# zhangkao/IIP_UAVSal_Saliency

Hardware: AMD Instinct MI355X
Metric: saliency frames/sec at 360x640 (higher is better)
Workload: dtype f32; 1 GPU; 360x640 batch=1 clip(s)/GPU seq=8, UAVSal.forward_clips, prec=f32, launch loop; requests_in_flight=1, clips_per_gpu=1, seq_len=8, height=360, width=640, precision=f32, persistent_state=False, parallelism=single GPU, fused_dw=10

## Files before the change

iip_uavsal_saliency_amd/_lib.py:

```python
from __future__ import annotations

import collections
import ctypes as C
import os

PKG = os.path.dirname(os.path.abspath(__file__))
LIB_PATH = os.environ.get("UAVSAL_HIP_LIB") or os.path.join(PKG, "libuavsal_hip.so")

PREC = {"f32": 0, "bf16x3": 1, "bf16": 2, "f16x3": 3}
ACT_NONE, ACT_RELU6, ACT_SIGMOID = 0, 1, 2
EPI_AFFINE, EPI_TWA, EPI_LSTM = 0, 1, 2
SK_TICKET_BASE = 4096

_ERR = {-1: "UAVSAL_EINVAL (null pointer / non-positive size)",
        -2: "UAVSAL_EALIGN (channel count / ld / pointer not 16-byte aligned)",
        -3: "UAVSAL_ESHAPE (shape not supported by the kernel)",
        -4: "UAVSAL_ESTATE (plan used in the wrong state)",
        -5: "UAVSAL_EDEVICE (a kernel reported a device-side error; the run's outputs are invalid)"}
ERR_STREAMK = 1
DW_KERNEL = {1: "dw3x3_kernel<1, 4, 4>", 2: "dw3x3_kernel<1, 2, 2>", 3: "dw3x3_kernel<2, 2, 2>", 4: "dw3x3_dilated_kernel",
             16: "dw3x3_map_lds_kernel<16, 256>", 32: "dw3x3_map_lds_kernel<32, 256>",
             528: "dw3x3_map_lds_kernel<16, 512>", 544: "dw3x3_map_lds_kernel<32, 512>",
             2048: "dw3x3_rowclass_kernel<256>"}

# ... 418 lines not shown

DESC_TYPES = [ConvDesc, DwDesc, StemDesc, BilinearDesc, TdiffDesc, TsumDesc, LayoutDesc, PostDesc, GuardDesc, CopyDesc,
              FusedIrDesc, WinoDesc, DwDotDesc, FillDesc, ScoreDesc, LetterboxDesc, OverlayDesc, GazeDesc, LossDesc, ConvRoute]

SYMBOLS = [
    ("uavsal_conv_gemm", C.c_int, [C.POINTER(ConvDesc), C.c_void_p]),
    ("uavsal_conv_route_of", C.c_int, [C.POINTER(ConvDesc), C.POINTER(ConvRoute)]),
    ("uavsal_conv_tile", C.c_int, [C.POINTER(ConvDesc)]),
    ("uavsal_conv_uses_split", C.c_int, [C.POINTER(ConvDesc)]),
    ("uavsal_conv_dwproj", C.c_int, [C.POINTER(ConvDesc)]),
    ("uavsal_streamk_workspace_bytes", C.c_longlong, []),
    ("uavsal_conv_streamk_grid", C.c_int, [C.POINTER(ConvDesc)]),
    ("uavsal_dw3x3", C.c_int, [C.POINTER(DwDesc), C.c_void_p]),
    ("uavsal_dw3x3_dot", C.c_int, [C.POINTER(DwDotDesc), C.c_void_p]),
    ("uavsal_dw_variant", C.c_int, [C.POINTER(DwDesc)]),
    ("uavsal_stem_conv", C.c_int, [C.POINTER(StemDesc), C.c_void_p]),
    ("uavsal_bilinear_ac", C.c_int, [C.POINTER(BilinearDesc), C.c_void_p]),
    ("uavsal_tdiff", C.c_int, [C.POINTER(TdiffDesc), C.c_void_p]),
    ("uavsal_tsum", C.c_int, [C.POINTER(TsumDesc), C.c_void_p]),
    ("uavsal_layout", C.c_int, [C.POINTER(LayoutDesc), C.c_void_p]),
    ("uavsal_postprocess", C.c_int, [C.POINTER(PostDesc), C.c_void_p]),
    ("uavsal_letterbox_u8", C.c_int, [C.POINTER(LetterboxDesc), C.c_void_p]),
    ("uavsal_overlay_workspace_bytes", C.c_int64, [C.POINTER(OverlayDesc)]),
    ("uavsal_overlay_u8", C.c_int, [C.POINTER(OverlayDesc), C.c_void_p]),
    ("uavsal_gaze_prepare", C.c_int, [C.POINTER(GazeDesc), C.c_void_p]),
    ("uavsal_loss_fu", C.c_int, [C.POINTER(LossDesc), C.c_void_p]),
    ("uavsal_loss_fu_grad", C.c_int, [C.POINTER(LossDesc), C.c_void_p]),
    ("uavsal_prior_accumulate", C.c_int, [C.POINTER(PriorAccDesc), C.c_void_p]),
    ("uavsal_prior_finish", C.c_int, [C.POINTER(PriorFinishDesc), C.c_void_p]),
    ("uavsal_prior_slab_frames", C.c_int, [C.c_int64, C.c_int32]),
    ("uavsal_prior_sizeof_desc", C.c_int, [C.c_int]),
    ("uavsal_twa_gate_bwd", C.c_int, [C.POINTER(TwaGateDesc), C.c_void_p]),
    ("uavsal_twa_wgrad_workspace_bytes", C.c_int64, [C.POINTER(TwaWgradDesc)]),
    ("uavsal_twa_wgrad_shares", C.c_int, [C.POINTER(TwaWgradDesc)]),
    ("uavsal_twa_wgrad", C.c_int, [C.POINTER(TwaWgradDesc), C.c_void_p]),
    ("uavsal_dec_bwd", C.c_int, [C.POINTER(DecBwdDesc), C.c_void_p]),
    ("uavsal_train_sizeof_desc", C.c_int, [C.c_int]),
    ("uavsal_lstm_scan", C.c_int, [C.POINTER(LstmScanDesc), C.c_void_p]),
    ("uavsal_lstm_gate_bwd", C.c_int, [C.POINTER(LstmGateDesc), C.c_void_p]),
    ("uavsal_lstm_sizeof_desc", C.c_int, [C.c_int]),
    ("uavsal_pix_gemm_workspace_bytes", C.c_int64, [C.POINTER(PixGemmDesc)]),
    ("uavsal_pix_gemm_shares", C.c_int, [C.POINTER(PixGemmDesc)]),
    ("uavsal_pix_gemm", C.c_int, [C.POINTER(PixGemmDesc), C.c_void_p]),
    ("uavsal_dec_sums_workspace_bytes", C.c_int64, [C.POINTER(DecSumsDesc)]),
    ("uavsal_dec_sums_slabs", C.c_int, [C.POINTER(DecSumsDesc)]),
    ("uavsal_dec_sums_slab_rows", C.c_int, [C.POINTER(DecSumsDesc)]),
    ("uavsal_dec_sums", C.c_int, [C.POINTER(DecSumsDesc), C.c_void_p]),
    ("uavsal_dec_finish", C.c_int, [C.POINTER(DecFinishDesc), C.c_void_p]),
    ("uavsal_train_decoder_sizeof_desc", C.c_int, [C.c_int]),
    ("uavsal_ir_bwd", C.c_int, [C.POINTER(IrBwdDesc), C.c_void_p]),
    ("uavsal_ir_sums_workspace_bytes", C.c_int64, [C.POINTER(IrSumsDesc)]),
    ("uavsal_ir_sums_slabs", C.c_int, [C.POINTER(IrSumsDesc)]),
    ("uavsal_ir_sums_slab_rows", C.c_int, [C.POINTER(IrSumsDesc)]),
    ("uavsal_ir_sums", C.c_int, [C.POINTER(IrSumsDesc), C.c_void_p]),
    ("uavsal_ir_finish", C.c_int, [C.POINTER(IrFinishDesc), C.c_void_p]),
    ("uavsal_ir_finish_c16", C.c_int, [C.POINTER(IrFinishDesc), C.c_void_p]),
    ("uavsal_block_sizeof_desc", C.c_int, [C.c_int]),
    ("uavsal_ir_bwd_s2", C.c_int, [C.POINTER(IrBwdS2Desc), C.c_void_p]),
    ("uavsal_bilinear_ac_bwd", C.c_int, [C.POINTER(BilinearBwdDesc), C.c_void_p]),
    ("uavsal_tsum_bwd", C.c_int, [C.POINTER(TsumBwdDesc), C.c_void_p]),
    ("uavsal_ctx_sizeof_desc", C.c_int, [C.c_int]),
    ("uavsal_ir_sums_s2_workspace_bytes", C.c_int64, [C.POINTER(IrSumsS2Desc)]),
    ("uavsal_ir_sums_s2_slabs", C.c_int, [C.POINTER(IrSumsS2Desc)]),
    ("uavsal_ir_sums_s2_slab_rows", C.c_int, [C.POINTER(IrSumsS2Desc)]),
    ("uavsal_ir_sums_s2", C.c_int, [C.POINTER(IrSumsS2Desc), C.c_void_p]),
    ("uavsal_mp_sizeof_desc", C.c_int, [C.c_int]),
    ("uavsal_ir_narrow_workspace_bytes", C.c_int64, [C.POINTER(IrNarrowDesc)]),
    ("uavsal_ir_narrow_slabs", C.c_int, [C.POINTER(IrNarrowDesc)]),
    ("uavsal_ir_narrow_slab_rows", C.c_int, [C.POINTER(IrNarrowDesc)]),
    ("uavsal_ir_narrow_grads", C.c_int, [C.POINTER(IrNarrowDesc), C.c_void_p]),
    ("uavsal_ir_narrow_finish", C.c_int, [C.POINTER(IrNarrowFinishDesc), C.c_void_p]),
    ("uavsal_frame_sum", C.c_int, [C.POINTER(FrameSumDesc), C.c_void_p]),
    ("uavsal_nets_sizeof_desc", C.c_int, [C.c_int]),
    ("uavsal_cbr_sums_workspace_bytes", C.c_int64, [C.POINTER(CbrSumsDesc)]),
    ("uavsal_cbr_sums_slabs", C.c_int, [C.POINTER(CbrSumsDesc)]),
    ("uavsal_cbr_sums_slab_rows", C.c_int, [C.POINTER(CbrSumsDesc)]),
    ("uavsal_cbr_sums", C.c_int, [C.POINTER(CbrSumsDesc), C.c_void_p]),
    ("uavsal_cbr_finish", C.c_int, [C.POINTER(CbrFinishDesc), C.c_void_p]),
    ("uavsal_tdiff_bwd", C.c_int, [C.POINTER(TdiffBwdDesc), C.c_void_p]),
    ("uavsal_st_sizeof_desc", C.c_int, [C.c_int]),
    ("uavsal_conv3_wgrad_workspace_bytes", C.c_int64, [C.POINTER(Conv3WgradDesc)]),
    ("uavsal_conv3_wgrad_shares", C.c_int, [C.POINTER(Conv3WgradDesc)]),
    ("uavsal_conv3_wgrad", C.c_int, [C.POINTER(Conv3WgradDesc), C.c_void_p]),
    ("uavsal_ir_bwd_dil", C.c_int, [C.POINTER(IrBwdDilDesc), C.c_void_p]),
    ("uavsal_ir_sums_dil_workspace_bytes", C.c_int64, [C.POINTER(IrSumsDilDesc)]),
    ("uavsal_ir_sums_dil_slabs", C.c_int, [C.POINTER(IrSumsDilDesc)]),
    ("uavsal_ir_sums_dil_slab_rows", C.c_int, [C.POINTER(IrSumsDilDesc)]),
    ("uavsal_ir_sums_dil", C.c_int, [C.POINTER(IrSumsDilDesc), C.c_void_p]),
    ("uavsal_srf_sizeof_desc", C.c_int, [C.c_int]),
    ("uavsal_skinny_wgrad_workspace_bytes", C.c_int64, [C.POINTER(SkinnyWgradDesc)]),
    ("uavsal_skinny_wgrad_shares", C.c_int, [C.POINTER(SkinnyWgradDesc)]),
    ("uavsal_skinny_wgrad", C.c_int, [C.POINTER(SkinnyWgradDesc), C.c_void_p]),
    ("uavsal_shallow_sizeof_desc", C.c_int, [C.c_int]),
    ("uavsal_bn_slabs", C.c_int, [C.c_int, C.c_int, C.c_int]),
    ("uavsal_bn_slab_rows", C.c_int, [C.c_int, C.c_int, C.c_int]),
    ("uavsal_bn_stats_workspace_bytes", C.c_int64, [C.POINTER(BnStatsDesc)]),
    ("uavsal_bn_stats", C.c_int, [C.POINTER(BnStatsDesc), C.c_void_p]),
    ("uavsal_bn_apply", C.c_int, [C.POINTER(BnApplyDesc), C.c_void_p]),
    ("uavsal_bn_bwd_workspace_bytes", C.c_int64, [C.POINTER(BnBwdDesc)]),
    ("uavsal_bn_bwd_sums", C.c_int, [C.POINTER(BnBwdDesc), C.c_void_p]),
    ("uavsal_bn_bwd_apply", C.c_int, [C.POINTER(BnBwdDesc), C.c_void_p]),
    ("uavsal_dw_wgrad_workspace_bytes", C.c_int64, [C.POINTER(DwWgradDesc)]),
    ("uavsal_dw_wgrad", C.c_int, [C.POINTER(DwWgradDesc), C.c_void_p]),
    ("uavsal_bn_sizeof_desc", C.c_int, [C.c_int]),
    ("uavsal_bn_apply_res", C.c_int, [C.POINTER(BnApplyResDesc), C.c_void_p]),
    ("uavsal_block_bn_sizeof_desc", C.c_int, [C.c_int]),
    ("uavsal_repack", C.c_int, [C.c_void_p, C.c_int, C.c_int, C.c_void_p]),
    ("uavsal_repack_sizeof_desc", C.c_int, []),
    ("uavsal_guard", C.c_int, [C.POINTER(GuardDesc), C.c_void_p]),
    ("uavsal_copy_rows", C.c_int, [C.POINTER(CopyDesc), C.c_void_p]),
    ("uavsal_fill", C.c_int, [C.POINTER(FillDesc), C.c_void_p]),
    ("uavsal_plan_add_fill", C.c_int, [C.c_void_p, C.POINTER(FillDesc)]),
    ("uavsal_fused_ir", C.c_int, [C.POINTER(FusedIrDesc), C.c_void_p]),
    ("uavsal_fused_ir_supported", C.c_int, [C.POINTER(FusedIrDesc)]),
    ("uavsal_plan_add_fused_ir", C.c_int, [C.c_void_p, C.POINTER(FusedIrDesc)]),
    ("uavsal_wino_input", C.c_int, [C.POINTER(WinoDesc), C.c_void_p]),
    ("uavsal_wino_output", C.c_int, [C.POINTER(WinoDesc), C.c_void_p]),
    ("uavsal_wino_output_zero_h", C.c_int, [C.POINTER(WinoDesc), C.c_void_p]),
    ("uavsal_wino_seam", C.c_int, [C.POINTER(WinoDesc), C.POINTER(WinoDesc), C.c_void_p]),
    ("uavsal_wino_seam_zero_h", C.c_int, [C.POINTER(WinoDesc), C.POINTER(WinoDesc), C.c_void_p]),
    ("uavsal_wino_seam_check", C.c_int, [C.POINTER(WinoDesc), C.POINTER(WinoDesc)]),
    ("uavsal_plan_add_wino_input", C.c_int, [C.c_void_p, C.POINTER(WinoDesc)]),
    ("uavsal_plan_add_wino_output", C.c_int, [C.c_void_p, C.POINTER(WinoDesc)]),
    ("uavsal_plan_add_copy", C.c_int, [C.c_void_p, C.POINTER(CopyDesc)]),
    ("uavsal_plan_create", C.c_void_p, []),
    ("uavsal_plan_destroy", None, [C.c_void_p]),
    ("uavsal_plan_add_conv", C.c_int, [C.c_void_p, C.POINTER(ConvDesc)]),
    ("uavsal_plan_add_dw", C.c_int, [C.c_void_p, C.POINTER(DwDesc)]),
    ("uavsal_plan_add_dw_dot", C.c_int, [C.c_void_p, C.POINTER(DwDotDesc)]),
    ("uavsal_plan_add_stem", C.c_int, [C.c_void_p, C.POINTER(StemDesc)]),
    ("uavsal_plan_add_bilinear", C.c_int, [C.c_void_p, C.POINTER(BilinearDesc)]),
    ("uavsal_plan_add_tdiff", C.c_int, [C.c_void_p, C.POINTER(TdiffDesc)]),
    ("uavsal_plan_add_tsum", C.c_int, [C.c_void_p, C.POINTER(TsumDesc)]),
    ("uavsal_plan_add_layout", C.c_int, [C.c_void_p, C.POINTER(LayoutDesc)]),
    ("uavsal_plan_error_word", C.c_void_p, [C.c_void_p]),
    ("uavsal_plan_add_guard", C.c_int, [C.c_void_p, _f, C.c_int64, _f, C.c_int64, _f, C.c_int64]),
    ("uavsal_plan_status", C.c_int, [C.c_void_p, C.c_int]),
    ("uavsal_plan_patch_ptr", C.c_int, [C.c_void_p, C.c_int, C.c_int, C.c_void_p]),
    ("uavsal_plan_set_lane", C.c_int, [C.c_void_p, C.c_int]),
    ("uavsal_plan_add_fork", C.c_int, [C.c_void_p, C.c_int]),
    ("uavsal_plan_add_join", C.c_int, [C.c_void_p, C.c_int]),
    ("uavsal_plan_enable_lanes", C.c_int, [C.c_void_p, C.c_int]),
    ("uavsal_plan_size", C.c_int, [C.c_void_p]),
    ("uavsal_plan_run", C.c_int, [C.c_void_p, C.c_int, C.c_int, C.c_void_p]),
    ("uavsal_plan_group_mark", C.c_int, [C.c_void_p, C.c_int, C.c_int, C.c_int]),
    ("uavsal_plan_group_enable", C.c_int, [C.c_void_p, C.c_int, C.c_int]),
    ("uavsal_plan_group_launches", C.c_int, [C.c_void_p, C.c_int]),
    ("uavsal_plan_last_launches", C.c_int, [C.c_void_p]),
    ("uavsal_plan_frame_repeat", C.c_int, [C.c_void_p, C.c_int, C.c_int, C.c_int, C.c_int, C.c_int]),
    ("uavsal_plan_frame_repeat_workgroups", C.c_int, [C.c_void_p, C.c_int]),
    ("uavsal_plan_seam", C.c_int, [C.c_void_p, C.c_int, C.c_int, C.c_int]),
    ("uavsal_plan_zero_state", C.c_int, [C.c_void_p, C.c_int, C.c_int, C.c_int, C.c_int, C.c_int, C.c_int]),
    ("uavsal_plan_mode_report", C.c_int, [C.c_void_p, C.POINTER(C.c_int * 4)]),
    ("uavsal_plan_graph_build", C.c_int, [C.c_void_p, C.c_void_p]),
    ("uavsal_plan_graph_launch", C.c_int, [C.c_void_p, C.c_void_p]),
    ("uavsal_plan_time", C.c_int, [C.c_void_p, C.c_int, C.c_int, C.c_int, C.c_void_p, C.POINTER(C.c_float)]),
    ("uavsal_score_workspace_bytes", C.c_int64, [C.POINTER(ScoreDesc)]),
    ("uavsal_score_stats", C.c_int, [C.POINTER(ScoreDesc), C.c_void_p]),
    ("uavsal_score_run", C.c_int, [C.POINTER(ScoreDesc), C.c_void_p]),
    ("uavsal_abi_version", C.c_int, []),
    ("uavsal_sizeof_desc", C.c_int, [C.c_int]),
    ("uavsal_build_info", C.c_char_p, []),
]

_lib = None


def load():
    global _lib
    if _lib is not None:
        return _lib
    if not os.path.exists(LIB_PATH):
        raise RuntimeError(
            "libuavsal_hip.so is not built (%s). Run `python -m iip_uavsal_saliency_amd.build` "
            "(needs hipcc). There is no CPU fallback for the UAVSal HIP path." % LIB_PATH)
    lib = C.CDLL(LIB_PATH)
    for name, res, args in SYMBOLS:
        fn = getattr(lib, name)
        fn.restype = res
        fn.argtypes = args
    if lib.uavsal_abi_version() != 20:
        raise RuntimeError("libuavsal_hip.so ABI version mismatch")
    for i, t in enumerate(DESC_TYPES):
        if lib.uavsal_sizeof_desc(i) != C.sizeof(t):
            raise RuntimeError("descriptor %s: ctypes size %d != C size %d" % (
                t.__name__, C.sizeof(t), lib.uavsal_sizeof_desc(i)))
    for sizeof, types in ((lib.uavsal_prior_sizeof_desc, PRIOR_DESC_TYPES), (lib.uavsal_train_sizeof_desc, TRAIN_DESC_TYPES),
                          (lib.uavsal_train_decoder_sizeof_desc, TRAIN_DECODER_DESC_TYPES),
                          (lib.uavsal_block_sizeof_desc, BLOCK_DESC_TYPES), (lib.uavsal_ctx_sizeof_desc, CTX_DESC_TYPES),
                          (lib.uavsal_mp_sizeof_desc, MP_DESC_TYPES), (lib.uavsal_nets_sizeof_desc, NETS_DESC_TYPES),
                          (lib.uavsal_st_sizeof_desc, ST_DESC_TYPES), (lib.uavsal_srf_sizeof_desc, SRF_DESC_TYPES),
                          (lib.uavsal_shallow_sizeof_desc, SHALLOW_DESC_TYPES), (lib.uavsal_lstm_sizeof_desc, LSTM_DESC_TYPES),
                          (lib.uavsal_bn_sizeof_desc, BN_DESC_TYPES), (lib.uavsal_block_bn_sizeof_desc, BLOCK_BN_DESC_TYPES)):
        for i, t in enumerate(types):
            if sizeof(i) != C.sizeof(t):
                raise RuntimeError("descriptor %s: ctypes size %d != C size %d" % (t.__name__, C.sizeof(t), sizeof(i)))
    if lib.uavsal_repack_sizeof_desc() != C.sizeof(RepackEntry):
        raise RuntimeError("descriptor RepackEntry: ctypes size %d != C size %d" % (C.sizeof(RepackEntry), lib.uavsal_repack_sizeof_desc()))
    _lib = lib
    return lib


def check(code: int, what: str = "uavsal call"):
    if code == 0:
        return
    if code == -5:
        raise RuntimeError("%s: %s" % (what, _ERR[-5]))
    if code < 0:
        raise RuntimeError("%s rejected its arguments: %s" % (what, _ERR.get(code, str(code))))
    raise RuntimeError("%s failed with hipError_t %d" % (what, code))
```

iip_uavsal_saliency_amd/csrc/fused_ir.hip:

```cpp
#include "common.h"

namespace {

struct FusedK {
    const float* in; const float* w1; const float* s1; const float* b1;
    const float* wd; const float* sd; const float* bd;
    const float* w2; const float* s2; const float* b2;
    const float* res; float* out;
    int ldi, ldr, ldo, H, W, Ho, Wo, tiles_x, tiles_y;
};

typedef float f32x2 __attribute__((ext_vector_type(2)));

__device__ __forceinline__ f32x4 relu6_4(f32x4 v) {
    return (f32x4){__builtin_amdgcn_fmed3f(v.x, 0.f, 6.f), __builtin_amdgcn_fmed3f(v.y, 0.f, 6.f), __builtin_amdgcn_fmed3f(v.z, 0.f, 6.f),
                   __builtin_amdgcn_fmed3f(v.w, 0.f, 6.f)};
}

#ifndef UAVSAL_FUSED_STAGE_W
#define UAVSAL_FUSED_STAGE_W 1
#endif
#ifndef UAVSAL_FUSED_NBUF2_MAX
#define UAVSAL_FUSED_NBUF2_MAX (80 * 1024)
#endif

template <int S, int TX, int PT>
struct FusedGeom {
    static constexpr int RP = 16 / TX;
    static constexpr int TY = 4 * PT * RP;
    static constexpr int IH = (TY - 1) * S + 3, IW = (TX - 1) * S + 3;
    static constexpr int HALF = (IW + 1) / 2;
    static constexpr int IWP = S == 2 ? 2 * HALF : IW;
    static constexpr int NSLOT = IH * IWP, NRT = (NSLOT + 15) / 16;
};

template <int CIN, int HID, int COUT, int S, bool EXPAND, int HC, int TX, int PT>
struct FusedCfg : FusedGeom<S, TX, PT> {
    using G = FusedGeom<S, TX, PT>;
    static constexpr int PLANE = EXPAND ? G::NRT * 16 * 4 : 4;
    static constexpr int SLOTF = EXPAND ? 4 : HC + 4;
    static constexpr int EBUF = EXPAND ? (HC / 4) * PLANE : G::NRT * 16 * SLOTF;
    static constexpr int NCH = HID / HC;
    static constexpr int CW_S1 = CIN * HC, CW_B1 = CW_S1 + HC, CW_WD = CW_B1 + HC, CW_SD = CW_WD + 9 * HC, CW_BD = CW_SD + HC,
                         CW_W2 = CW_BD + HC, CW_F = CW_W2 + HC * COUT;
    static constexpr bool STAGE_W = EXPAND && UAVSAL_FUSED_STAGE_W;
    static constexpr int NBUF = (EXPAND && NCH > 1 && (2 * EBUF + (STAGE_W ? 2 * CW_F : 0)) * 4 <= UAVSAL_FUSED_NBUF2_MAX) ? 2 : 1;
    static constexpr size_t E_BYTES = (size_t)NBUF * EBUF * 4;
    static constexpr int WBASE = NBUF * EBUF;
    static constexpr size_t SMEM = E_BYTES + (STAGE_W ? (size_t)2 * CW_F * 4 : 0);
};

#ifndef UAVSAL_FUSED_PROBE
#define UAVSAL_FUSED_PROBE 0
#endif

#ifdef UAVSAL_FIR_STAMPS
__device__ unsigned long long g_fir_stamps[128];
#define FIR_STAMP(i) { asm volatile("s_waitcnt vmcnt(0) lgkmcnt(0)" ::: "memory"); \
                       if (blockIdx.x == gridDim.x / 2 && tid == 0) g_fir_stamps[i] = __builtin_amdgcn_s_memtime(); }
#else
#define FIR_STAMP(i)
#endif

template <int CIN, int HID, int COUT, int S, bool EXPAND, int HC, int TX, int PT>
__global__ __launch_bounds__(256, 2) void fused_ir_kernel(const FusedK p) {
    using Cfg = FusedCfg<CIN, HID, COUT, S, EXPAND, HC, TX, PT>;
    constexpr int RP = Cfg::RP, TY = Cfg::TY, IH = Cfg::IH, IW = Cfg::IW, HALF = Cfg::HALF, IWP = Cfg::IWP;
    constexpr int NSLOT = Cfg::NSLOT, NRT = Cfg::NRT, RTW = (NRT + 3) / 4;
    constexpr int CPL = HC / 4, CQ = CPL / 4, PLANE = Cfg::PLANE, SLOTF = Cfg::SLOTF;
    constexpr int NCH = Cfg::NCH, NCTE = HC / 16, NCT = (COUT + 15) / 16, KE = CIN / 4;
    constexpr int EBUF = Cfg::EBUF, NBUF = Cfg::NBUF;
    static_assert(HID % HC == 0 && HC % 16 == 0 && CIN % 8 == 0 && COUT % 4 == 0, "channel blocking");
    static_assert(EXPAND || (HID == CIN && NCH == 1), "without an expand conv the hidden tensor is the input");
    static_assert(KE % 2 == 0, "x fragments are loaded 8 bytes at a time");

    extern __shared__ __attribute__((aligned(16))) float lds[];

    const int tid = threadIdx.x, lane = tid & 63;
    const int wave = __builtin_amdgcn_readfirstlane(tid >> 6);
    const int l15 = lane & 15, lq = lane >> 4;
    int t = blockIdx.x;
    const int tx = t % p.tiles_x; t /= p.tiles_x;
    const int ty = t % p.tiles_y;
    const int n = t / p.tiles_y;
    const int oy0 = ty * TY, ox0 = tx * TX;
    const int iy0 = oy0 * S - 1, ix0 = ox0 * S - 1;
    const float* inb = p.in + (size_t)n * p.H * p.W * p.ldi;
    FIR_STAMP(0)

    auto slot_pixel = [&](int slot, int& gy, int& gx) -> bool {
        const int iy = slot / IWP, rem = slot - iy * IWP;
        int ix = rem;
        if (S == 2) { const int par = rem >= HALF ? 1 : 0; ix = 2 * (rem - par * HALF) + par; }
        gy = iy0 + iy; gx = ix0 + ix;
        return slot < NSLOT && ix < IW && gy >= 0 && gy < p.H && gx >= 0 && gx < p.W;
    };

    auto slot_read = [&](int slot) -> bool {
        const int iy = slot / IWP, rem = slot - iy * IWP;
        return slot < NSLOT && (S == 2 ? rem != IWP - 1 || (IW & 1) == 0 : true);
    };

    float xv[EXPAND ? RTW : 1][EXPAND ? KE : 1];
    unsigned outside = 0;
    unsigned any_outside = 0;
    if (EXPAND) {
#pragma unroll
        for (int j = 0; j < RTW; ++j) {
            const int rt = wave + 4 * j;
            int gy, gx;
            const bool in = rt < NRT && slot_pixel(rt * 16 + l15, gy, gx);
            const bool zero = !in && rt < NRT && slot_read(rt * 16 + l15);
            outside |= (zero ? 1u : 0u) << j;
            any_outside |= (__builtin_amdgcn_ballot_w64(zero) != 0ull ? 1u : 0u) << j;
            const float* src = inb + ((size_t)(in ? gy : 0) * p.W + (in ? gx : 0)) * p.ldi + lq * KE;
            if (KE % 4 == 0) {
#pragma unroll
                for (int s = 0; s < KE; s += 4) {
                    f32x4 v = {0.f, 0.f, 0.f, 0.f};
                    if (in) v = *reinterpret_cast<const f32x4*>(src + s);
                    xv[j][s] = v.x; xv[j][s + 1] = v.y; xv[j][s + 2] = v.z; xv[j][s + 3] = v.w;
                }
            } else {
#pragma unroll
                for (int s = 0; s < KE; s += 2) {
                    f32x2 v = {0.f, 0.f};
                    if (in) v = *reinterpret_cast<const f32x2*>(src + s);
                    xv[j][s] = v.x; xv[j][s + 1] = v.y;
                }
            }
        }
    } else {
        constexpr int NQ = CIN / 4, NST = (NRT * 16 * NQ + 255) / 256;
        f32x4 st[NST];
#pragma unroll
        for (int i = 0; i < NST; ++i) {
            const int idx = tid + 256 * i;
            const int slot = idx / NQ, q = idx - slot * NQ;
            int gy, gx;
            st[i] = (f32x4){0.f, 0.f, 0.f, 0.f};
            if (idx < NRT * 16 * NQ && slot_pixel(slot, gy, gx)) st[i] = *reinterpret_cast<const f32x4*>(inb + ((size_t)gy * p.W + gx) * p.ldi + q * 4);
        }
#pragma unroll
        for (int i = 0; i < NST; ++i) {
            const int idx = tid + 256 * i;
            const int slot = idx / NQ, q = idx - slot * NQ;
            if (idx < NRT * 16 * NQ) *reinterpret_cast<f32x4*>(lds + (size_t)q * PLANE + slot * SLOTF) = st[i];
        }
    }

    FIR_STAMP(1)
    f32x4 acc_o[PT][NCT];
#pragma unroll
    for (int pt = 0; pt < PT; ++pt)
#pragma unroll
        for (int ct = 0; ct < NCT; ++ct) acc_o[pt][ct] = (f32x4){0.f, 0.f, 0.f, 0.f};

    constexpr bool STAGE_W = Cfg::STAGE_W;
    constexpr int HQ = HC / 4, NI_W1 = CIN * HQ, NI_V = HQ, NI_WD = 9 * HQ, NI_W2 = HC * COUT / 4;
    constexpr int NITEM = NI_W1 + 2 * NI_V + NI_WD + 2 * NI_V + NI_W2, WROUNDS = (NITEM + 255) / 256;
    float* const wl = lds + Cfg::WBASE;
    const float* wsrc[STAGE_W ? WROUNDS : 1];
    int wdst[STAGE_W ? WROUNDS : 1], wstep[STAGE_W ? WROUNDS : 1];
    f32x4 wreg[STAGE_W ? WROUNDS : 1];
    if (STAGE_W) {
#pragma unroll
        for (int r = 0; r < WROUNDS; ++r) {
            int it = tid + 256 * r;
            wsrc[r] = nullptr; wdst[r] = 0; wstep[r] = HC;
            if (it < NI_W1) { const int k = it / HQ, q = it - k * HQ; wsrc[r] = p.w1 + (size_t)k * HID + 4 * q; wdst[r] = k * HC + 4 * q; }
            else if ((it -= NI_W1) < NI_V) { wsrc[r] = p.s1 + 4 * it; wdst[r] = Cfg::CW_S1 + 4 * it; }
            else if ((it -= NI_V) < NI_V) { wsrc[r] = p.b1 + 4 * it; wdst[r] = Cfg::CW_B1 + 4 * it; }
            else if ((it -= NI_V) < NI_WD) { const int tp = it / HQ, q = it - tp * HQ; wsrc[r] = p.wd + (size_t)tp * HID + 4 * q; wdst[r] = Cfg::CW_WD + tp * HC + 4 * q; }
            else if ((it -= NI_WD) < NI_V) { wsrc[r] = p.sd + 4 * it; wdst[r] = Cfg::CW_SD + 4 * it; }
            else if ((it -= NI_V) < NI_V) { wsrc[r] = p.bd + 4 * it; wdst[r] = Cfg::CW_BD + 4 * it; }
            else if ((it -= NI_V) < NI_W2) { wsrc[r] = p.w2 + 4 * it; wdst[r] = Cfg::CW_W2 + 4 * it; wstep[r] = HC * COUT; }
        }
#pragma unroll
        for (int r = 0; r < WROUNDS; ++r)
            if (wsrc[r]) *reinterpret_cast<f32x4*>(wl + wdst[r]) = *reinterpret_cast<const f32x4*>(wsrc[r]);
        __syncthreads();
    }
    const float* const g_w1 = p.w1;
    FIR_STAMP(2)

    for (int ch = 0; ch < NCH; ++ch) {
        const int c0 = (UAVSAL_FUSED_PROBE & 8) ? 0 : ch * HC;
        const float* const wc = wl + (ch & 1) * Cfg::CW_F;
        float w1f[EXPAND ? NCTE : 1][EXPAND ? KE : 1];
        f32x4 s1q[EXPAND ? NCTE : 1], b1q[EXPAND ? NCTE : 1];
        if (EXPAND) {
#pragma unroll
            for (int ct = 0; ct < NCTE; ++ct) {
#pragma unroll
                for (int s = 0; s < KE; ++s)
                    w1f[ct][s] = STAGE_W ? wc[(lq * KE + s) * HC + ct * 16 + l15] : g_w1[(size_t)(lq * KE + s) * HID + c0 + ct * 16 + l15];
                s1q[ct] = STAGE_W ? *reinterpret_cast<const f32x4*>(wc + Cfg::CW_S1 + ct * 16 + 4 * lq)
                                  : *reinterpret_cast<const f32x4*>(p.s1 + c0 + ct * 16 + 4 * lq);
                b1q[ct] = STAGE_W ? *reinterpret_cast<const f32x4*>(wc + Cfg::CW_B1 + ct * 16 + 4 * lq)
                                  : *reinterpret_cast<const f32x4*>(p.b1 + c0 + ct * 16 + 4 * lq);
            }
        }
        f32x4 wdq[9][CQ], sdq[CQ], bdq[CQ];
#pragma unroll
        for (int q = 0; q < CQ; ++q) {
#pragma unroll
            for (int tp = 0; tp < 9; ++tp)
                wdq[tp][q] = STAGE_W ? *reinterpret_cast<const f32x4*>(wc + Cfg::CW_WD + tp * HC + lq * CPL + 4 * q)
                                     : *reinterpret_cast<const f32x4*>(p.wd + (size_t)tp * HID + c0 + lq * CPL + 4 * q);
            sdq[q] = STAGE_W ? *reinterpret_cast<const f32x4*>(wc + Cfg::CW_SD + lq * CPL + 4 * q) : *reinterpret_cast<const f32x4*>(p.sd + c0 + lq * CPL + 4 * q);
            bdq[q] = STAGE_W ? *reinterpret_cast<const f32x4*>(wc + Cfg::CW_BD + lq * CPL + 4 * q) : *reinterpret_cast<const f32x4*>(p.bd + c0 + lq * CPL + 4 * q);
        }
        float w2f[NCT][CPL];
#pragma unroll
        for (int ct = 0; ct < NCT; ++ct) {
            const int co = ct * 16 + l15;
#pragma unroll
            for (int s = 0; s < CPL; ++s)
                w2f[ct][s] = co < COUT ? (STAGE_W ? wc[Cfg::CW_W2 + (lq * CPL + s) * COUT + co] : p.w2[(size_t)(c0 + lq * CPL + s) * COUT + co]) : 0.f;
        }
        if (STAGE_W && ch + 1 < NCH) {
#pragma unroll
            for (int r = 0; r < WROUNDS; ++r)
                if (wsrc[r]) wreg[r] = *reinterpret_cast<const f32x4*>(wsrc[r] + (size_t)(ch + 1) * wstep[r]);
        }

        FIR_STAMP(8 + 5 * ch)
        float* eb = lds + (NBUF == 2 ? (ch & 1) * EBUF : 0);
        if (EXPAND) {
            if (NBUF == 1 && ch > 0 && !(UAVSAL_FUSED_PROBE & 16)) __syncthreads();
#pragma unroll
            for (int j = 0; j < RTW; ++j) {
                const int rt = wave + 4 * j;
                if (4 * j + 3 >= NRT && rt >= NRT) continue;
                f32x4 e[NCTE];
#pragma unroll
                for (int ct = 0; ct < NCTE; ++ct) {
                    e[ct] = (f32x4){0.f, 0.f, 0.f, 0.f};
#pragma unroll
                    for (int s = 0; s < KE; ++s) {
                        if (UAVSAL_FUSED_PROBE & 1) e[ct][s & 3] += w1f[ct][s] * xv[j][s];
                        else e[ct] = __builtin_amdgcn_mfma_f32_16x16x4f32(w1f[ct][s], xv[j][s], e[ct], 0, 0, 0);
                    }
                    e[ct] = relu6_4(e[ct] * s1q[ct] + b1q[ct]);
                }
                if ((any_outside >> j) & 1u) {
                    const bool z = (outside >> j) & 1u;
#pragma unroll
                    for (int ct = 0; ct < NCTE; ++ct) if (z) e[ct] = (f32x4){0.f, 0.f, 0.f, 0.f};
                }
#pragma unroll
                for (int ct = 0; ct < NCTE; ++ct)
                    if (!(UAVSAL_FUSED_PROBE & 32) || e[ct].x == 123.f) *reinterpret_cast<f32x4*>(eb + (size_t)(ct * 4 + lq) * PLANE + (rt * 16 + l15) * SLOTF) = e[ct];
            }
        }
        if (STAGE_W && ch + 1 < NCH) {
#pragma unroll
            for (int r = 0; r < WROUNDS; ++r)
                if (wsrc[r]) *reinterpret_cast<f32x4*>(wl + ((ch + 1) & 1) * Cfg::CW_F + wdst[r]) = wreg[r];
        }
        FIR_STAMP(9 + 5 * ch)
        if (!(UAVSAL_FUSED_PROBE & 16)) __syncthreads();
        FIR_STAMP(10 + 5 * ch)
#pragma unroll
        for (int pt = 0; pt < PT; ++pt) {
            const int g = wave * PT + pt;
            const int orow = g * RP + l15 / TX, ocol = l15 % TX;
            f32x4 dq[CQ];
#pragma unroll
            for (int q = 0; q < CQ; ++q) dq[q] = (f32x4){0.f, 0.f, 0.f, 0.f};
#pragma unroll
            for (int ky = 0; ky < ((UAVSAL_FUSED_PROBE & 2) ? 1 : 3); ++ky)
#pragma unroll
                for (int kx = 0; kx < ((UAVSAL_FUSED_PROBE & 2) ? 1 : 3); ++kx) {
                    const int slot = (orow * S + ky) * IWP + (S == 2 ? (kx & 1) * HALF + ocol + (kx >> 1) : ocol + kx);
                    const float* e = eb + (size_t)(lq * CQ) * PLANE + slot * SLOTF;
#pragma unroll
                    for (int q = 0; q < CQ; ++q) dq[q] = *reinterpret_cast<const f32x4*>(e + (size_t)q * PLANE) * wdq[ky * 3 + kx][q] + dq[q];
                }
#pragma unroll
            for (int q = 0; q < CQ; ++q) dq[q] = relu6_4(dq[q] * sdq[q] + bdq[q]);
            if (pt == PT - 1) { FIR_STAMP(11 + 5 * ch) }
#pragma unroll
            for (int s = 0; s < CPL; ++s)
#pragma unroll
                for (int ct = 0; ct < NCT; ++ct)
                    if (UAVSAL_FUSED_PROBE & 4) acc_o[pt][ct][s & 3] += w2f[ct][s] * dq[s >> 2][s & 3];
                    else acc_o[pt][ct] = __builtin_amdgcn_mfma_f32_16x16x4f32(w2f[ct][s], dq[s >> 2][s & 3], acc_o[pt][ct], 0, 0, 0);
        }
        FIR_STAMP(12 + 5 * ch)
    }
    FIR_STAMP(3)

#pragma unroll
    for (int ct = 0; ct < NCT; ++ct) {
        const int co = ct * 16 + 4 * lq;
        if (co >= COUT) continue;
        const f32x4 sc = *reinterpret_cast<const f32x4*>(p.s2 + co), bi = *reinterpret_cast<const f32x4*>(p.b2 + co);
#pragma unroll
        for (int pt = 0; pt < PT; ++pt) {
            const int g = wave * PT + pt;
            const int gy = oy0 + g * RP + l15 / TX, gx = ox0 + l15 % TX;
            if (gy >= p.Ho || gx >= p.Wo) continue;
            const size_t opix = ((size_t)n * p.Ho + gy) * p.Wo + gx;
            f32x4 v = acc_o[pt][ct] * sc + bi;
            if (p.res) v += *reinterpret_cast<const f32x4*>(p.res + opix * p.ldr + co);
            *reinterpret_cast<f32x4*>(p.out + opix * p.ldo + co) = v;
        }
    }
    FIR_STAMP(4)
}

template <int CIN, int HID, int COUT, int S, bool EXPAND, int HC, int TX, int PT>
int launch_fused(const uavsal_fused_ir_desc* d, hipStream_t s) {
    using Cfg = FusedCfg<CIN, HID, COUT, S, EXPAND, HC, TX, PT>;
    FusedK k;
    k.in = d->in; k.w1 = d->w1; k.s1 = d->scale1; k.b1 = d->bias1;
    k.wd = d->wd; k.sd = d->scale_d; k.bd = d->bias_d;
    k.w2 = d->w2; k.s2 = d->scale2; k.b2 = d->bias2;
    k.res = d->res; k.out = d->out;
    k.ldi = d->ldi; k.ldr = d->ldr; k.ldo = d->ldo; k.H = d->H; k.W = d->W;
    k.Ho = (d->H - 1) / S + 1; k.Wo = (d->W - 1) / S + 1;
    k.tiles_x = (k.Wo + TX - 1) / TX; k.tiles_y = (k.Ho + Cfg::TY - 1) / Cfg::TY;
    const long long nblk = (long long)d->n_img * k.tiles_y * k.tiles_x;
    if (nblk > 0x7fffffffLL) return UAVSAL_ESHAPE;
    UAVSAL_LDS_OPTIN((&fused_ir_kernel<CIN, HID, COUT, S, EXPAND, HC, TX, PT>), Cfg::SMEM);
    hipLaunchKernelGGL((fused_ir_kernel<CIN, HID, COUT, S, EXPAND, HC, TX, PT>), dim3((unsigned)nblk), dim3(256), Cfg::SMEM, s, k);
    return uavsal_launch_status();
}

#ifndef UAVSAL_FUSED_BIG_MIN
#define UAVSAL_FUSED_BIG_MIN 400
#endif
template <int CIN, int HID, int COUT, int S, bool EXPAND, int HCS, int HCB>
int launch_fused_shape(const uavsal_fused_ir_desc* d, hipStream_t s) {
    constexpr bool BIG_AUTO = !(CIN == 32 && COUT == 64);
    constexpr int BPT = S == 1 ? 4 : 2;
    constexpr int BTY = 4 * BPT;
    const int Ho = (d->H - 1) / S + 1, Wo = (d->W - 1) / S + 1;
    const long long big = (long long)d->n_img * ((Ho + BTY - 1) / BTY) * ((Wo + 15) / 16);
    const bool use_big = d->tile == 2 || (d->tile == 0 && BIG_AUTO && big >= UAVSAL_FUSED_BIG_MIN);
    return use_big ? launch_fused<CIN, HID, COUT, S, EXPAND, HCB, 16, BPT>(d, s) : launch_fused<CIN, HID, COUT, S, EXPAND, HCS, 16, 1>(d, s);
}

int dispatch(const uavsal_fused_ir_desc* d, hipStream_t s, bool launch) {
#define UAVSAL_FUSED_UNPAREN(...) __VA_ARGS__
#define UAVSAL_FUSED_CASE(CIN, HID, COUT, S, EXP, HCC)                                                   \
    if (d->Cin == CIN && d->hidden == HID && d->Cout == COUT && d->stride == S && (d->w1 != nullptr) == EXP) \
        return launch ? launch_fused_shape<CIN, HID, COUT, S, EXP, UAVSAL_FUSED_UNPAREN HCC>(d, s) : 1;
#ifndef UAVSAL_FUSED_HCS
#define UAVSAL_FUSED_HCS 16
#endif
#ifndef UAVSAL_FUSED_HCS144
#define UAVSAL_FUSED_HCS144 16
#endif
#ifndef UAVSAL_FUSED_HCB
#define UAVSAL_FUSED_HCB 16
#endif
#ifndef UAVSAL_FUSED_HCB144
#define UAVSAL_FUSED_HCB144 16
#endif
    UAVSAL_FUSED_CASE(32, 32, 16, 1, false, (32, 32))
    UAVSAL_FUSED_CASE(16, 96, 24, 2, true, (UAVSAL_FUSED_HCS, UAVSAL_FUSED_HCB))
    UAVSAL_FUSED_CASE(24, 144, 24, 1, true, (UAVSAL_FUSED_HCS144, UAVSAL_FUSED_HCB144))
    UAVSAL_FUSED_CASE(24, 144, 32, 2, true, (UAVSAL_FUSED_HCS144, UAVSAL_FUSED_HCB144))
    UAVSAL_FUSED_CASE(32, 192, 32, 1, true, (UAVSAL_FUSED_HCS, UAVSAL_FUSED_HCB))
    UAVSAL_FUSED_CASE(32, 192, 64, 2, true, (UAVSAL_FUSED_HCS, UAVSAL_FUSED_HCB))
#undef UAVSAL_FUSED_CASE
    return launch ? UAVSAL_ESHAPE : 0;
}

}

int uavsal_fused_mid_dispatch(const uavsal_fused_ir_desc* d, hipStream_t s, bool launch);

#ifdef UAVSAL_FIR_STAMPS
extern "C" int uavsal_fir_stamps(unsigned long long* dst) {
    return (int)hipMemcpyFromSymbol(dst, HIP_SYMBOL(g_fir_stamps), sizeof(unsigned long long) * 128);
}
#endif

extern "C" int uavsal_fused_ir_supported(const uavsal_fused_ir_desc* d) {
    if (!d) return 0;
    const int mid = uavsal_fused_mid_dispatch(d, nullptr, false);
    return mid ? mid : dispatch(d, nullptr, false);
}

extern "C" int uavsal_fused_ir(const uavsal_fused_ir_desc* d, uavsal_stream_t stream) {
    if (!d || !d->in || !d->wd || !d->scale_d || !d->bias_d || !d->w2 || !d->scale2 || !d->bias2 || !d->out) return UAVSAL_EINVAL;
    if (d->w1 && (!d->scale1 || !d->bias1)) return UAVSAL_EINVAL;
    if (d->n_img <= 0 || d->H <= 0 || d->W <= 0) return UAVSAL_EINVAL;
    if ((d->ldi & 3) || d->ldi < d->Cin || (d->ldo & 3) || d->ldo < d->Cout || !uavsal_aligned16(d->in) || !uavsal_aligned16(d->out) ||
        !uavsal_aligned16(d->wd) || !uavsal_aligned16(d->scale_d) || !uavsal_aligned16(d->bias_d) || !uavsal_aligned16(d->scale2) ||
        !uavsal_aligned16(d->bias2) || (d->w1 && (!uavsal_aligned16(d->scale1) || !uavsal_aligned16(d->bias1))) ||
        (d->res && ((d->ldr & 3) || !uavsal_aligned16(d->res))))
        return UAVSAL_EALIGN;
    if ((d->w1 && !uavsal_aligned16(d->w1)) || !uavsal_aligned16(d->w2)) return UAVSAL_EALIGN;
    if (d->tile < 0 || d->tile > 2) return UAVSAL_EINVAL;
    if (d->res && (d->ldr < d->Cout || d->stride != 1 || d->Cin != d->Cout)) return UAVSAL_ESHAPE;
    if (uavsal_fused_mid_dispatch(d, nullptr, false)) return uavsal_fused_mid_dispatch(d, (hipStream_t)stream, true);
    return dispatch(d, (hipStream_t)stream, true);
}
```

iip_uavsal_saliency_amd/csrc/glue.hip:

```cpp
#include "common.h"

namespace {

struct StemK {
    const float* in; const uint8_t* in_u8; const float* w; const float* scale; const float* bias;
    float* out; int ldo, H, W, Ho, Wo, tiles_x, tiles_y;
    float mean[3], stdv[3];
};

constexpr int ST_TY = 4, ST_TX = 64, ST_IH = 2 * ST_TY + 1, ST_IW = 2 * ST_TX + 1, ST_PITCH = 132, ST_ROWS = 3 * ST_IH;
static_assert(ST_PITCH >= ST_IW && ST_PITCH % 4 == 0 && ST_TY * ST_TX == 256, "stem tile");

__global__ __launch_bounds__(256) void stem_kernel(const StemK p) {
    __shared__ __attribute__((aligned(16))) float wsh[27 * 32];
    __shared__ __attribute__((aligned(16))) float ssh[32], bsh[32];
    __shared__ __attribute__((aligned(16))) float xsh[ST_ROWS * ST_PITCH];
    const int tid = threadIdx.x;
    int b = blockIdx.x;
    const int tx = b % p.tiles_x; b /= p.tiles_x;
    const int ty = b % p.tiles_y;
    const int n = b / p.tiles_y;
    const int oy0 = ty * ST_TY, ox0 = tx * ST_TX;
    const int iy0 = 2 * oy0 - 1, ix0 = 2 * ox0 - 1;
    const size_t plane = (size_t)p.H * p.W;
    constexpr int NST = (ST_ROWS * ST_PITCH + 255) / 256;
    float st[NST];
#pragma unroll
    for (int i = 0; i < NST; ++i) {
        const int idx = tid + 256 * i;
        const int r = idx / ST_PITCH, c = idx - r * ST_PITCH;
        const int ci = r / ST_IH, iy = iy0 + (r - ci * ST_IH), ix = ix0 + c;
        float x = 0.f;
        if (r < ST_ROWS && c < ST_IW && iy >= 0 && iy < p.H && ix >= 0 && ix < p.W) {
            const size_t at = ((size_t)n * 3 + ci) * plane + (size_t)iy * p.W + ix;
            if (p.in_u8) x = ((float)p.in_u8[at] / 255.0f - p.mean[ci]) / p.stdv[ci];
            else x = p.in[at];
        }
        st[i] = x;
    }
    for (int i = tid; i < 27 * 32; i += 256) wsh[i] = p.w[i];
    if (tid < 32) { ssh[tid] = p.scale[tid]; bsh[tid] = p.bias[tid]; }
#pragma unroll
    for (int i = 0; i < NST; ++i) {
        const int idx = tid + 256 * i;
        if (idx < ST_ROWS * ST_PITCH) xsh[idx] = st[i];
    }
    __syncthreads();
    const int g = tid & 7, pxg = tid >> 3;
    const int rr = pxg / (ST_TX / 8), xq = pxg - rr * (ST_TX / 8);
    const int oy = oy0 + rr, oxb = ox0 + 8 * xq;
    f32x4 acc[8];
#pragma unroll
    for (int q = 0; q < 8; ++q) acc[q] = (f32x4){0.f, 0.f, 0.f, 0.f};
#pragma unroll 1
    for (int ci = 0; ci < 3; ++ci) {
#pragma unroll
        for (int ky = 0; ky < 3; ++ky) {
            const float* row = xsh + (ci * ST_IH + 2 * rr + ky) * ST_PITCH + 16 * xq;
            float v[17];
#pragma unroll
            for (int c = 0; c < 4; ++c) {
                const f32x4 a = *reinterpret_cast<const f32x4*>(row + 4 * c);
                v[4 * c] = a.x; v[4 * c + 1] = a.y; v[4 * c + 2] = a.z; v[4 * c + 3] = a.w;
            }
            v[16] = row[16];
#pragma unroll
            for (int kx = 0; kx < 3; ++kx) {
                const f32x4 w4 = *reinterpret_cast<const f32x4*>(wsh + (ci * 9 + ky * 3 + kx) * 32 + g * 4);
#pragma unroll
                for (int q = 0; q < 8; ++q) acc[q] = w4 * v[2 * q + kx] + acc[q];
            }
        }
    }
    if (oy >= p.Ho) return;
    const f32x4 sc = *reinterpret_cast<const f32x4*>(ssh + g * 4), bi = *reinterpret_cast<const f32x4*>(bsh + g * 4);
#pragma unroll
    for (int q = 0; q < 8; ++q) {
        const int ox = oxb + q;
        if (ox >= p.Wo) break;
        f32x4 r = acc[q] * sc + bi;
        r.x = fminf(fmaxf(r.x, 0.f), 6.f); r.y = fminf(fmaxf(r.y, 0.f), 6.f); r.z = fminf(fmaxf(r.z, 0.f), 6.f); r.w = fminf(fmaxf(r.w, 0.f), 6.f);
        *reinterpret_cast<f32x4*>(p.out + (((size_t)n * p.Ho + oy) * p.Wo + ox) * p.ldo + g * 4) = r;
    }
}

struct BilK {
    const float* in; float* out;
    int ldi, ldo, Hi, Wi, Ho, Wo, C4, src_mod, src_div;
    float sy, sx; long long total;
    _Float16* out_split; int ldos;
};

__global__ __launch_bounds__(256) void bilinear_kernel(const BilK p) {
    const long long item = (long long)blockIdx.x * 256 + threadIdx.x;
    if (item >= p.total) return;
    const int c = (int)(item % p.C4) * 4;
    long long t = item / p.C4;
    const int ox = (int)(t % p.Wo); t /= p.Wo;
    const int oy = (int)(t % p.Ho);
    const int n = (int)(t / p.Ho);
    const int ns = (n % p.src_mod) / p.src_div;
    const float fy = p.sy * oy, fx = p.sx * ox;
    const int y0 = (int)fy, x0 = (int)fx;
    const int y1 = y0 + (y0 < p.Hi - 1 ? 1 : 0), x1 = x0 + (x0 < p.Wi - 1 ? 1 : 0);
    const float ly = fy - y0, lx = fx - x0;
    const float hy = 1.f - ly, hx = 1.f - lx;
    const float* b = p.in + (size_t)ns * p.Hi * p.Wi * p.ldi + c;
    const f32x4 v00 = *reinterpret_cast<const f32x4*>(b + ((size_t)y0 * p.Wi + x0) * p.ldi);
    const f32x4 v01 = *reinterpret_cast<const f32x4*>(b + ((size_t)y0 * p.Wi + x1) * p.ldi);
    const f32x4 v10 = *reinterpret_cast<const f32x4*>(b + ((size_t)y1 * p.Wi + x0) * p.ldi);
    const f32x4 v11 = *reinterpret_cast<const f32x4*>(b + ((size_t)y1 * p.Wi + x1) * p.ldi);
    const f32x4 r = hy * (hx * v00 + lx * v01) + ly * (hx * v10 + lx * v11);
    const size_t opix = ((size_t)n * p.Ho + oy) * p.Wo + ox;
    *reinterpret_cast<f32x4*>(p.out + opix * p.ldo + c) = r;
    if (p.out_split) uavsal_store_split4(p.out_split + opix * p.ldos, c, r);
}

struct TdK { const float* in; float* out; int ldi, ldo, HW, C4, L; long long total; };

__global__ __launch_bounds__(256) void tdiff_kernel(const TdK p) {
    const long long item = (long long)blockIdx.x * 256 + threadIdx.x;
    if (item >= p.total) return;
    const int c = (int)(item % p.C4) * 4;
    long long t = item / p.C4;
    const int pix = (int)(t % p.HW);
    const int n = (int)(t / p.HW);
    const int tt = n % p.L;
    const size_t img = (size_t)p.HW * p.ldi;
    const float* cur = p.in + (size_t)n * img + (size_t)pix * p.ldi + c;
    const f32x4 x = *reinterpret_cast<const f32x4*>(cur);
    f32x4 dprev, dnext;
    if (tt == 0) {
        const f32x4 nx = *reinterpret_cast<const f32x4*>(cur + img);
        dprev = nx - x; dnext = x - nx;
    } else if (tt == p.L - 1) {
        const f32x4 pv = *reinterpret_cast<const f32x4*>(cur - img);
        dprev = x - pv; dnext = pv - x;
    } else {
        const f32x4 pv = *reinterpret_cast<const f32x4*>(cur - img);
        const f32x4 nx = *reinterpret_cast<const f32x4*>(cur + img);
        dprev = x - pv; dnext = x - nx;
    }
    float* o = p.out + ((size_t)n * p.HW + pix) * p.ldo + c;
    *reinterpret_cast<f32x4*>(o) = dprev;
    *reinterpret_cast<f32x4*>(o + p.C4 * 4) = dnext;
}

struct TsK { const float* in; float* out; int ldi, ldo, HW, C4, T; long long total; };

__global__ __launch_bounds__(256) void tsum_kernel(const TsK p) {
    const long long item = (long long)blockIdx.x * 256 + threadIdx.x;
    if (item >= p.total) return;
    const int c = (int)(item % p.C4) * 4;
    long long t = item / p.C4;
    const int pix = (int)(t % p.HW);
    const int b = (int)(t / p.HW);
    const size_t img = (size_t)p.HW * p.ldi;
    const float* src = p.in + (size_t)b * p.T * img + (size_t)pix * p.ldi + c;
    f32x4 s = *reinterpret_cast<const f32x4*>(src);
    for (int k = 1; k < p.T; ++k) s += *reinterpret_cast<const f32x4*>(src + (size_t)k * img);
    *reinterpret_cast<f32x4*>(p.out + ((size_t)b * p.HW + pix) * p.ldo + c) = s;
}

struct LayK { const float* in; float* out; int C, HW, ld, Cpad, to_nhwc; long long total; };

__global__ __launch_bounds__(256) void layout_kernel(const LayK p) {
    __shared__ float tile[32][33];
    const int tiles_c = (p.Cpad + 31) / 32;
    const int tiles_p = (p.HW + 31) / 32;
    long long b = blockIdx.x;
    const int tc = (int)(b % tiles_c); b /= tiles_c;
    const int tp = (int)(b % tiles_p);
    const int n = (int)(b / tiles_p);
    const int lx = threadIdx.x & 31, ly = threadIdx.x >> 5;
    if (p.to_nhwc) {
        for (int j = ly; j < 32; j += 8) {
            const int c = tc * 32 + j, px = tp * 32 + lx;
            tile[j][lx] = (c < p.C && px < p.HW) ? p.in[((size_t)n * p.C + c) * p.HW + px] : 0.f;
        }
        __syncthreads();
        for (int j = ly; j < 32; j += 8) {
            const int px = tp * 32 + j, c = tc * 32 + lx;
            if (px < p.HW && c < p.Cpad) p.out[((size_t)n * p.HW + px) * p.ld + c] = tile[lx][j];
        }
    } else {
        for (int j = ly; j < 32; j += 8) {
            const int px = tp * 32 + j, c = tc * 32 + lx;
            tile[j][lx] = (px < p.HW && c < p.C) ? p.in[((size_t)n * p.HW + px) * p.ld + c] : 0.f;
        }
        __syncthreads();
        for (int j = ly; j < 32; j += 8) {
            const int c = tc * 32 + j, px = tp * 32 + lx;
            if (c < p.C && px < p.HW) p.out[((size_t)n * p.C + c) * p.HW + px] = tile[lx][j];
        }
    }
}

inline int grid_for(long long total, int* nblk) {
    const long long b = (total + 255) / 256;
    if (b <= 0 || b > 0x7fffffffLL) return UAVSAL_ESHAPE;
    *nblk = (int)b;
    return 0;
}

}

extern "C" int uavsal_stem_conv(const uavsal_stem_desc* d, uavsal_stream_t stream) {
    if (!d || (!d->in && !d->in_u8) || !d->w || !d->scale || !d->bias || !d->out) return UAVSAL_EINVAL;
    if (d->n_img <= 0 || d->H <= 0 || d->W <= 0) return UAVSAL_EINVAL;
    if ((d->ldo & 3) || d->ldo < 32 || !uavsal_aligned16(d->out)) return UAVSAL_EALIGN;
    StemK k;
    k.in = d->in; k.in_u8 = d->in_u8; k.w = d->w; k.scale = d->scale; k.bias = d->bias; k.out = d->out;
    k.ldo = d->ldo; k.H = d->H; k.W = d->W; k.Ho = (d->H - 1) / 2 + 1; k.Wo = (d->W - 1) / 2 + 1;
    for (int i = 0; i < 3; ++i) { k.mean[i] = d->mean[i]; k.stdv[i] = d->stdv[i]; }
    k.tiles_x = (k.Wo + ST_TX - 1) / ST_TX; k.tiles_y = (k.Ho + ST_TY - 1) / ST_TY;
    const long long nblk = (long long)d->n_img * k.tiles_y * k.tiles_x;
    if (nblk > 0x7fffffffLL) return UAVSAL_ESHAPE;
    hipLaunchKernelGGL(stem_kernel, dim3((unsigned)nblk), dim3(256), 0, (hipStream_t)stream, k);
    return uavsal_launch_status();
}

extern "C" int uavsal_bilinear_ac(const uavsal_bilinear_desc* d, uavsal_stream_t stream) {
    if (!d || !d->in || !d->out) return UAVSAL_EINVAL;
    if (d->n_out <= 0 || d->C <= 0 || d->Hi <= 0 || d->Wi <= 0 || d->Ho <= 0 || d->Wo <= 0) return UAVSAL_EINVAL;
    if (d->src_mod <= 0 || d->src_div <= 0) return UAVSAL_EINVAL;
    if ((d->C & 3) || (d->ldi & 3) || (d->ldo & 3) || d->ldi < d->C || d->ldo < d->C) return UAVSAL_EALIGN;
    if (!uavsal_aligned16(d->in) || !uavsal_aligned16(d->out)) return UAVSAL_EALIGN;
    BilK k;
    k.in = d->in; k.out = d->out; k.ldi = d->ldi; k.ldo = d->ldo;
    k.Hi = d->Hi; k.Wi = d->Wi; k.Ho = d->Ho; k.Wo = d->Wo; k.C4 = d->C / 4;
    k.src_mod = d->src_mod; k.src_div = d->src_div;
    k.sy = d->Ho > 1 ? (float)(d->Hi - 1) / (float)(d->Ho - 1) : 0.f;
    k.sx = d->Wo > 1 ? (float)(d->Wi - 1) / (float)(d->Wo - 1) : 0.f;
    if (d->out_split && ((d->ldos & 63) || d->ldos < 2 * d->C || (d->C & 31) || ((uintptr_t)d->out_split & 127)))
// ... 109 lines not shown
```

iip_uavsal_saliency_amd/csrc/plan.hip:

```cpp
#include <vector>
#include <new>
#include "common.h"

namespace {
enum OpKind { OP_CONV = 0, OP_DW, OP_STEM, OP_BILINEAR, OP_TDIFF, OP_TSUM, OP_LAYOUT, OP_GUARD, OP_COPY, OP_FUSED_IR, OP_FORK, OP_JOIN,
              OP_WINO_IN, OP_WINO_OUT, OP_DW_DOT, OP_FILL };
constexpr int MAX_LANES = 8;
constexpr int MAX_GROUPS = 32;

struct Op {
    int kind;
    int lane;
    int group;
    union {
        uavsal_conv_desc conv;
        uavsal_dw_desc dw;
        uavsal_stem_desc stem;
        uavsal_bilinear_desc bil;
        uavsal_tdiff_desc td;
        uavsal_tsum_desc ts;
        uavsal_layout_desc lay;
        uavsal_guard_desc guard;
        uavsal_copy_desc copy;
        uavsal_fused_ir_desc fir;
        uavsal_wino_desc wino;
        uavsal_dw_dot_desc dwdot;
        uavsal_fill_desc fill;
    } u;
};

int run_op(const Op& op, uavsal_stream_t s) {
    switch (op.kind) {
        case OP_CONV: return uavsal_conv_gemm(&op.u.conv, s);
        case OP_DW: return uavsal_dw3x3(&op.u.dw, s);
        case OP_STEM: return uavsal_stem_conv(&op.u.stem, s);
        case OP_BILINEAR: return uavsal_bilinear_ac(&op.u.bil, s);
        case OP_TDIFF: return uavsal_tdiff(&op.u.td, s);
        case OP_TSUM: return uavsal_tsum(&op.u.ts, s);
        case OP_LAYOUT: return uavsal_layout(&op.u.lay, s);
        case OP_GUARD: return uavsal_guard(&op.u.guard, s);
        case OP_COPY: return uavsal_copy_rows(&op.u.copy, s);
        case OP_FUSED_IR: return uavsal_fused_ir(&op.u.fir, s);
        case OP_WINO_IN: return uavsal_wino_input(&op.u.wino, s);
        case OP_WINO_OUT: return uavsal_wino_output(&op.u.wino, s);
        case OP_DW_DOT: return uavsal_dw3x3_dot(&op.u.dwdot, s);
        case OP_FILL: return uavsal_fill(&op.u.fill, s);
    }
    return UAVSAL_EINVAL;
}
}

struct uavsal_plan {
    std::vector<Op> ops;
    hipGraph_t graph = nullptr;
    hipGraphExec_t exec = nullptr;
    int cur_lane = 0;
    bool lanes_on = true;
    hipStream_t side[MAX_LANES] = {};
    std::vector<hipEvent_t> events;
    int32_t* err_dev = nullptr;
    int32_t* err_host = nullptr;
    int32_t* err_host_dev = nullptr;
    hipEvent_t done = nullptr;
    bool ran = false;
    uint32_t groups_off = 0;
    int last_launches = 0;
    int graph_launches = 0;
    int fr_pw = -1, fr_dw = -1, fr_mod = 0, fr_div = 0;
    bool fr_on = false;
    int fr_wg[2] = {0, 0};
    std::vector<int> seam_next;
    int zs_first = -1, zs_last = -1, zs_xin = -1, zs_gemm = -1, zs_xout = -1;
    bool zs_on = false;
    int mode_seams = 0, mode_elided = 0, mode_kernels = 0;
};

extern "C" uavsal_plan* uavsal_plan_create(void) { return new (std::nothrow) uavsal_plan(); }

static bool ensure_error_words(uavsal_plan* p) {
    if (p->err_dev && p->err_host && p->done) return true;
    bool ok = hipMalloc((void**)&p->err_dev, 64) == hipSuccess && hipMemset(p->err_dev, 0, 64) == hipSuccess &&
              hipHostMalloc((void**)&p->err_host, 64, hipHostMallocMapped) == hipSuccess;
    if (ok) {
        p->err_host[0] = 0;
        ok = hipHostGetDevicePointer((void**)&p->err_host_dev, p->err_host, 0) == hipSuccess &&
             hipEventCreateWithFlags(&p->done, hipEventDisableTiming) == hipSuccess;
    }
    if (!ok) (void)hipGetLastError();
    return ok;
}

extern "C" int32_t* uavsal_plan_error_word(uavsal_plan* p) { return (p && ensure_error_words(p)) ? p->err_dev : nullptr; }

extern "C" int uavsal_plan_add_guard(uavsal_plan* p, float* b0, int64_t n0, float* b1, int64_t n1, float* b2, int64_t n2) {
    if (!p) return UAVSAL_EINVAL;
    if (p->exec) return UAVSAL_ESTATE;
    if (!ensure_error_words(p)) return UAVSAL_ESTATE;
    Op op; op.kind = OP_GUARD; op.lane = 0; op.group = -1;
    op.u.guard.err = p->err_dev; op.u.guard.host_err = p->err_host_dev;
    op.u.guard.buf[0] = b0; op.u.guard.n[0] = n0;
    op.u.guard.buf[1] = b1; op.u.guard.n[1] = n1;
    op.u.guard.buf[2] = b2; op.u.guard.n[2] = n2;
    for (int b = 0; b < 3; ++b)
        if ((op.u.guard.buf[b] == nullptr) != (op.u.guard.n[b] == 0) || op.u.guard.n[b] < 0) return UAVSAL_EINVAL;
    p->ops.push_back(op);
    return (int)p->ops.size() - 1;
}

extern "C" int uavsal_plan_status(uavsal_plan* p, int wait) {
    if (!p) return UAVSAL_EINVAL;
    if (!p->ran) return 0;
    if (wait) {
        const hipError_t e = hipEventSynchronize(p->done);
        if (e != hipSuccess) return (int)e;
    } else {
        const hipError_t e = hipEventQuery(p->done);
        if (e == hipErrorNotReady) { (void)hipGetLastError(); return 0; }
        if (e != hipSuccess) return (int)e;
    }
    const int32_t code = *(volatile int32_t*)p->err_host;
    if (code == 0) return 0;
    p->err_host[0] = 0;
    const hipError_t e = hipMemset(p->err_dev, 0, 64);
    if (e != hipSuccess) return (int)e;
    return UAVSAL_EDEVICE;
}

extern "C" void uavsal_plan_destroy(uavsal_plan* p) {
    if (!p) return;
    if (p->exec) hipGraphExecDestroy(p->exec);
    if (p->graph) hipGraphDestroy(p->graph);
    for (hipEvent_t e : p->events) if (e) hipEventDestroy(e);
    for (int i = 1; i < MAX_LANES; ++i) if (p->side[i]) hipStreamDestroy(p->side[i]);
    if (p->done) hipEventDestroy(p->done);
    if (p->err_host) hipHostFree(p->err_host);
    if (p->err_dev) hipFree(p->err_dev);
    delete p;
}

extern "C" int uavsal_plan_set_lane(uavsal_plan* p, int lane) {
    if (!p || lane < 0 || lane >= MAX_LANES) return UAVSAL_EINVAL;
    p->cur_lane = lane;
    return 0;
}

extern "C" int uavsal_plan_enable_lanes(uavsal_plan* p, int on) {
    if (!p) return UAVSAL_EINVAL;
    if (p->exec) return UAVSAL_ESTATE;
    p->lanes_on = on != 0;
    return 0;
}

static int add_sync(uavsal_plan* p, int kind, int lane) {
    if (!p || lane < 1 || lane >= MAX_LANES) return UAVSAL_EINVAL;
    if (p->exec) return UAVSAL_ESTATE;
    Op op; op.kind = kind; op.lane = lane; op.group = -1;
    p->ops.push_back(op);
    return (int)p->ops.size() - 1;
}
extern "C" int uavsal_plan_add_fork(uavsal_plan* p, int lane) { return add_sync(p, OP_FORK, lane); }
extern "C" int uavsal_plan_add_join(uavsal_plan* p, int lane) { return add_sync(p, OP_JOIN, lane); }

#define UAVSAL_ADD(fn, KIND, field, T)                                   \
    extern "C" int fn(uavsal_plan* p, const T* d) {                      \
        if (!p || !d) return UAVSAL_EINVAL;                              \
        if (p->exec) return UAVSAL_ESTATE;                               \
        Op op; op.kind = KIND; op.lane = p->cur_lane; op.group = -1; op.u.field = *d; \
        p->ops.push_back(op);                                            \
        return (int)p->ops.size() - 1;                                   \
    }
UAVSAL_ADD(uavsal_plan_add_conv, OP_CONV, conv, uavsal_conv_desc)
UAVSAL_ADD(uavsal_plan_add_dw, OP_DW, dw, uavsal_dw_desc)
UAVSAL_ADD(uavsal_plan_add_stem, OP_STEM, stem, uavsal_stem_desc)
UAVSAL_ADD(uavsal_plan_add_bilinear, OP_BILINEAR, bil, uavsal_bilinear_desc)
UAVSAL_ADD(uavsal_plan_add_tdiff, OP_TDIFF, td, uavsal_tdiff_desc)
UAVSAL_ADD(uavsal_plan_add_tsum, OP_TSUM, ts, uavsal_tsum_desc)
UAVSAL_ADD(uavsal_plan_add_layout, OP_LAYOUT, lay, uavsal_layout_desc)
UAVSAL_ADD(uavsal_plan_add_copy, OP_COPY, copy, uavsal_copy_desc)
UAVSAL_ADD(uavsal_plan_add_fused_ir, OP_FUSED_IR, fir, uavsal_fused_ir_desc)
UAVSAL_ADD(uavsal_plan_add_wino_input, OP_WINO_IN, wino, uavsal_wino_desc)
UAVSAL_ADD(uavsal_plan_add_wino_output, OP_WINO_OUT, wino, uavsal_wino_desc)
UAVSAL_ADD(uavsal_plan_add_dw_dot, OP_DW_DOT, dwdot, uavsal_dw_dot_desc)
UAVSAL_ADD(uavsal_plan_add_fill, OP_FILL, fill, uavsal_fill_desc)

extern "C" int uavsal_plan_patch_ptr(uavsal_plan* p, int op, int slot, void* ptr) {
    if (!p || op < 0 || op >= (int)p->ops.size() || !ptr) return UAVSAL_EINVAL;
    if (p->exec) return UAVSAL_ESTATE;
    Op& o = p->ops[op];
    switch (o.kind) {
        case OP_CONV:
            if (!uavsal_aligned16(ptr)) return UAVSAL_EALIGN;
            if (slot == 0) o.u.conv.a = (const float*)ptr;
            else if (slot == 1) o.u.conv.out = (float*)ptr;
            else return UAVSAL_EINVAL;
            return 0;
        case OP_DW_DOT:
            if (slot == 0) { if (!uavsal_aligned16(ptr)) return UAVSAL_EALIGN; o.u.dwdot.in = (const float*)ptr; }
            else if (slot == 1) o.u.dwdot.out = (float*)ptr;
            else return UAVSAL_EINVAL;
            return 0;
        case OP_STEM:
            if (slot == 0) { o.u.stem.in = (const float*)ptr; o.u.stem.in_u8 = nullptr; }
            else if (slot == 1) { o.u.stem.in_u8 = (const uint8_t*)ptr; o.u.stem.in = nullptr; }
            else return UAVSAL_EINVAL;
            return 0;
        case OP_LAYOUT:
            if (slot == 0) o.u.lay.in = (const float*)ptr;
            else if (slot == 1) o.u.lay.out = (float*)ptr;
            else return UAVSAL_EINVAL;
            return 0;
        case OP_GUARD:
            if (slot < 0 || slot > 2 || !o.u.guard.buf[slot]) return UAVSAL_EINVAL;
            o.u.guard.buf[slot] = (float*)ptr;
            return 0;
    }
    return UAVSAL_ESHAPE;
}

extern "C" int uavsal_plan_size(const uavsal_plan* p) { return p ? (int)p->ops.size() : UAVSAL_EINVAL; }

extern "C" int uavsal_plan_group_mark(uavsal_plan* p, int group, int first, int last) {
    if (!p || group < 0 || group >= MAX_GROUPS || first < 0 || last > (int)p->ops.size() || first >= last) return UAVSAL_EINVAL;
    if (p->exec) return UAVSAL_ESTATE;
    for (int i = first; i < last; ++i)
        if (p->ops[i].group >= 0 && p->ops[i].group != group) return UAVSAL_EINVAL;
    for (int i = first; i < last; ++i) p->ops[i].group = group;
    return 0;
}

extern "C" int uavsal_plan_group_enable(uavsal_plan* p, int group, int on) {
    if (!p || group < 0 || group >= MAX_GROUPS) return UAVSAL_EINVAL;
    const uint32_t bit = 1u << group;
    if (((p->groups_off & bit) == 0) == (on != 0)) return 0;
    if (p->exec) return UAVSAL_ESTATE;
    if (on) p->groups_off &= ~bit; else p->groups_off |= bit;
    return 0;
}

extern "C" int uavsal_plan_group_launches(const uavsal_plan* p, int group) {
    if (!p || group < 0 || group >= MAX_GROUPS) return UAVSAL_EINVAL;
    int n = 0;
    for (const Op& op : p->ops) n += op.group == group && op.kind != OP_FORK && op.kind != OP_JOIN;
    return n;
}

extern "C" int uavsal_plan_last_launches(const uavsal_plan* p) { return p ? p->last_launches : UAVSAL_EINVAL; }

static int run_range(uavsal_plan* p, int first, int last, uavsal_stream_t stream, bool masked, int* launched, bool repeat = false) {
    const int n = (int)p->ops.size();
    if (last < 0 || last > n) last = n;
    if (first < 0 || first > last) return UAVSAL_EINVAL;
    bool fr = repeat && p->fr_on && p->fr_pw >= 0 && first == 0 && last > p->fr_dw;
    if (fr) {
        const Op& a = p->ops[p->fr_pw];
        const Op& b = p->ops[p->fr_dw];
        const uint32_t goff = masked ? p->groups_off : 0u;
        hipStreamCaptureStatus cs = hipStreamCaptureStatusNone;
        if (hipStreamIsCapturing((hipStream_t)stream, &cs) != hipSuccess) { (void)hipGetLastError(); cs = hipStreamCaptureStatusActive; }
        fr = cs == hipStreamCaptureStatusNone && !(a.group >= 0 && ((goff >> a.group) & 1u)) && !(b.group >= 0 && ((goff >> b.group) & 1u)) &&
             uavsal_conv_repeat_pair(&a.u.conv, &b.u.conv, p->fr_mod, p->fr_div) == 1;
    }
    bool modes = repeat && (p->zs_on || !p->seam_next.empty());
    if (modes) {
        hipStreamCaptureStatus cs = hipStreamCaptureStatusNone;
        if (hipStreamIsCapturing((hipStream_t)stream, &cs) != hipSuccess) { (void)hipGetLastError(); cs = hipStreamCaptureStatusActive; }
        modes = cs == hipStreamCaptureStatusNone;
    }
    const uint32_t moff = masked ? p->groups_off : 0u;
    auto masked_out = [&](int i) { return p->ops[i].group >= 0 && ((moff >> p->ops[i].group) & 1u); };
    bool zs = modes && p->zs_on && p->zs_xin >= first && p->zs_xout < last && (p->zs_first < 0 || (p->zs_first >= first && p->zs_last < last)) &&
              !masked_out(p->zs_xin) && !masked_out(p->zs_gemm) && !masked_out(p->zs_xout);
    for (int i = p->zs_first; zs && i >= 0 && i <= p->zs_last; ++i) zs = !masked_out(i);
    if (repeat && first == 0) p->mode_seams = p->mode_elided = p->mode_kernels = 0;
    const bool lanes = p->lanes_on && first == 0 && last == n;
    const uint32_t off = masked ? p->groups_off : 0u;
    hipStream_t main_s = (hipStream_t)stream;
    if (p->events.size() < p->ops.size()) p->events.resize(p->ops.size(), nullptr);
    for (int i = first; i < last; ++i) {
        const Op& op = p->ops[i];
        if (op.group >= 0 && ((off >> op.group) & 1u)) continue;
        if (op.kind == OP_FORK || op.kind == OP_JOIN) {
            if (!lanes) continue;
            if (!p->side[op.lane] &&
                hipStreamCreateWithFlags(&p->side[op.lane], hipStreamNonBlocking) != hipSuccess) return (int)hipGetLastError();
            if (!p->events[i] &&
                hipEventCreateWithFlags(&p->events[i], hipEventDisableTiming) != hipSuccess) return (int)hipGetLastError();
            hipStream_t from = op.kind == OP_FORK ? main_s : p->side[op.lane];
            hipStream_t to = op.kind == OP_FORK ? p->side[op.lane] : main_s;
            hipError_t e = hipEventRecord(p->events[i], from);
            if (e == hipSuccess) e = hipStreamWaitEvent(to, p->events[i], 0);
            if (e != hipSuccess) return (int)e;
            continue;
        }
        uavsal_stream_t s = (lanes && op.lane > 0) ? (uavsal_stream_t)p->side[op.lane] : stream;
        if (lanes && op.lane > 0 && !p->side[op.lane]) return UAVSAL_ESTATE;
        int e;
        if (zs && ((p->zs_first >= 0 && i >= p->zs_first && i <= p->zs_last) || i == p->zs_xin || i == p->zs_gemm)) {
            ++p->mode_elided;
            ++*launched;
            continue;
        }
        const bool seam = modes && i < (int)p->seam_next.size() && p->seam_next[i] == i + 1 && i + 1 < last && !masked_out(i + 1) &&
                          p->ops[i + 1].lane == op.lane;
        if (seam) {
            const bool zh = zs && i == p->zs_xout;
            e = zh ? uavsal_wino_seam_zero_h(&op.u.wino, &p->ops[i + 1].u.wino, s) : uavsal_wino_seam(&op.u.wino, &p->ops[i + 1].u.wino, s);
            if (e) return e;
            ++p->mode_seams; ++p->mode_kernels;
            *launched += 2;
            ++i;
            continue;
        }
        if (repeat && (i == p->fr_pw || i == p->fr_dw))
            e = uavsal_conv_gemm_mapped(&op.u.conv, s, fr ? p->fr_mod : 0, fr ? p->fr_div : 0, &p->fr_wg[i == p->fr_dw]);
        else if (zs && i == p->zs_xout)
            e = uavsal_wino_output_zero_h(&op.u.wino, s);
        else
            e = run_op(op, s);
        if (e) return e;
        ++*launched;
        if (repeat) ++p->mode_kernels;
    }
    if (last == n) {
        hipStreamCaptureStatus cs = hipStreamCaptureStatusNone;
        if (hipStreamIsCapturing(main_s, &cs) != hipSuccess) { (void)hipGetLastError(); cs = hipStreamCaptureStatusNone; }
        if (cs == hipStreamCaptureStatusNone && p->done) {
            const hipError_t e = hipEventRecord(p->done, main_s);
            if (e != hipSuccess) return (int)e;
            p->ran = true;
        }
    }
    return 0;
}

extern "C" int uavsal_plan_run(uavsal_plan* p, int first, int last, uavsal_stream_t stream) {
    if (!p) return UAVSAL_EINVAL;
    if (first == 0) p->last_launches = 0;
    return run_range(p, first, last, stream, true, &p->last_launches, true);
}

extern "C" int uavsal_plan_frame_repeat(uavsal_plan* p, int op_pw, int op_dwpl, int src_mod, int src_div, int on) {
    const int n = p ? (int)p->ops.size() : 0;
    if (!p || op_pw < 0 || op_dwpl <= op_pw || op_dwpl >= n || src_mod <= 0 || src_div <= 0) return UAVSAL_EINVAL;
    if (p->ops[op_pw].kind != OP_CONV || p->ops[op_dwpl].kind != OP_CONV) return UAVSAL_EINVAL;
    p->fr_pw = op_pw; p->fr_dw = op_dwpl; p->fr_mod = src_mod; p->fr_div = src_div;
    p->fr_on = on != 0 && !p->exec &&
               uavsal_conv_repeat_pair(&p->ops[op_pw].u.conv, &p->ops[op_dwpl].u.conv, src_mod, src_div) == 1;
    return p->fr_on ? 1 : 0;
}

extern "C" int uavsal_plan_seam(uavsal_plan* p, int op_xout, int op_xin, int on) {
    const int n = p ? (int)p->ops.size() : 0;
    if (!p || op_xout < 0 || op_xin < 0 || op_xout >= n || op_xin >= n) return UAVSAL_EINVAL;
    if (p->ops[op_xout].kind != OP_WINO_OUT || p->ops[op_xin].kind != OP_WINO_IN) return UAVSAL_EINVAL;
    if ((int)p->seam_next.size() < n) p->seam_next.resize(n, -1);
    p->seam_next[op_xout] = -1;
    if (!on || p->exec || op_xin != op_xout + 1 || p->ops[op_xin].lane != p->ops[op_xout].lane ||
        uavsal_wino_seam_check(&p->ops[op_xout].u.wino, &p->ops[op_xin].u.wino) != 0)
        return 0;
    p->seam_next[op_xout] = op_xin;
    return 1;
}

extern "C" int uavsal_plan_zero_state(uavsal_plan* p, int op_state_in_first, int op_state_in_last, int op_xin0, int op_gemm0,
                                      int op_xout0, int on) {
    const int n = p ? (int)p->ops.size() : 0;
    if (!p || op_xin0 < 0 || op_gemm0 != op_xin0 + 1 || op_xout0 != op_gemm0 + 1 || op_xout0 >= n) return UAVSAL_EINVAL;
    if ((op_state_in_first < 0) != (op_state_in_last < 0) || op_state_in_last < op_state_in_first || op_state_in_last >= op_xin0)
        return UAVSAL_EINVAL;
    const Op& xi = p->ops[op_xin0];
    const Op& g = p->ops[op_gemm0];
    const Op& xo = p->ops[op_xout0];
    if (xi.kind != OP_WINO_IN || g.kind != OP_CONV || xo.kind != OP_WINO_OUT) return UAVSAL_EINVAL;
    for (int i = op_state_in_first; i >= 0 && i <= op_state_in_last; ++i)
        if (p->ops[i].kind != OP_LAYOUT) return UAVSAL_EINVAL;
    p->zs_first = op_state_in_first; p->zs_last = op_state_in_last;
    p->zs_xin = op_xin0; p->zs_gemm = op_gemm0; p->zs_xout = op_xout0;
    p->zs_on = on != 0 && !p->exec && xi.u.wino.R == 2 && xo.u.wino.R == 2 && xo.u.wino.epi == UAVSAL_EPI_TWA &&
               xi.u.wino.n_seg == 0 && xi.u.wino.in == xo.u.wino.hprev && g.u.conv.a == xi.u.wino.out && g.u.conv.out == xo.u.wino.in &&
               xi.lane == xo.lane && g.lane == xo.lane;
    return p->zs_on ? 1 : 0;
}

extern "C" int uavsal_plan_mode_report(const uavsal_plan* p, int out[4]) {
    if (!p || !out) return UAVSAL_EINVAL;
    out[0] = p->mode_seams; out[1] = p->mode_elided; out[2] = p->mode_kernels; out[3] = 0;
    return 0;
}

extern "C" int uavsal_plan_frame_repeat_workgroups(const uavsal_plan* p, int which) {
    return p && (which == 0 || which == 1) ? p->fr_wg[which] : UAVSAL_EINVAL;
}

extern "C" int uavsal_plan_graph_build(uavsal_plan* p, uavsal_stream_t stream) {
    if (!p) return UAVSAL_EINVAL;
    if (p->exec) return 0;
    p->fr_on = false;
    p->zs_on = false;
    p->seam_next.clear();
    hipStream_t s = (hipStream_t)stream;
    hipError_t e = hipStreamBeginCapture(s, hipStreamCaptureModeThreadLocal);
    if (e != hipSuccess) return (int)e;
    const int r = uavsal_plan_run(p, 0, -1, stream);
    hipGraph_t g = nullptr;
    e = hipStreamEndCapture(s, &g);
    if (r) { if (g) hipGraphDestroy(g); return r; }
    if (e != hipSuccess) return (int)e;
    hipGraphExec_t ex = nullptr;
    e = hipGraphInstantiate(&ex, g, nullptr, nullptr, 0);
    if (e != hipSuccess) { hipGraphDestroy(g); return (int)e; }
    p->graph = g; p->exec = ex;
    p->graph_launches = p->last_launches;
    return 0;
}

extern "C" int uavsal_plan_graph_launch(uavsal_plan* p, uavsal_stream_t stream) {
    if (!p) return UAVSAL_EINVAL;
    if (!p->exec) return UAVSAL_ESTATE;
    hipError_t e = hipGraphLaunch(p->exec, (hipStream_t)stream);
    if (e == hipSuccess && p->done) {
        e = hipEventRecord(p->done, (hipStream_t)stream);
        if (e == hipSuccess) p->ran = true;
    }
    if (e == hipSuccess) p->last_launches = p->graph_launches;
    return e == hipSuccess ? 0 : (int)e;
}

extern "C" int uavsal_plan_time(uavsal_plan* p, int first, int last, int iters, uavsal_stream_t stream, float* ms) {
    if (!p || !ms || iters <= 0) return UAVSAL_EINVAL;
    hipStream_t s = (hipStream_t)stream;
    hipEvent_t e0, e1;
    if (hipEventCreate(&e0) != hipSuccess) return (int)hipGetLastError();
    if (hipEventCreate(&e1) != hipSuccess) { hipEventDestroy(e0); return (int)hipGetLastError(); }
    int r = 0, launched = 0;
    hipEventRecord(e0, s);
    for (int i = 0; i < iters && !r; ++i) r = run_range(p, first, last, stream, false, &launched);
    hipEventRecord(e1, s);
    hipError_t e = hipEventSynchronize(e1);
    float t = 0.f;
    if (e == hipSuccess) e = hipEventElapsedTime(&t, e0, e1);
    hipEventDestroy(e0); hipEventDestroy(e1);
    if (r) return r;
    if (e != hipSuccess) return (int)e;
    *ms = t / iters;
    return 0;
}

extern "C" int uavsal_abi_version(void) { return UAVSAL_ABI_VERSION; }

extern "C" int uavsal_sizeof_desc(int which) {
    switch (which) {
        case 0: return (int)sizeof(uavsal_conv_desc);
        case 1: return (int)sizeof(uavsal_dw_desc);
        case 2: return (int)sizeof(uavsal_stem_desc);
        case 3: return (int)sizeof(uavsal_bilinear_desc);
        case 4: return (int)sizeof(uavsal_tdiff_desc);
        case 5: return (int)sizeof(uavsal_tsum_desc);
        case 6: return (int)sizeof(uavsal_layout_desc);
        case 7: return (int)sizeof(uavsal_post_desc);
        case 8: return (int)sizeof(uavsal_guard_desc);
        case 9: return (int)sizeof(uavsal_copy_desc);
        case 10: return (int)sizeof(uavsal_fused_ir_desc);
        case 11: return (int)sizeof(uavsal_wino_desc);
        case 12: return (int)sizeof(uavsal_dw_dot_desc);
        case 13: return (int)sizeof(uavsal_fill_desc);
        case 14: return (int)sizeof(uavsal_score_desc);
        case 15: return (int)sizeof(uavsal_letterbox_desc);
        case 16: return (int)sizeof(uavsal_overlay_desc);
        case 17: return (int)sizeof(uavsal_gaze_desc);
        case 18: return (int)sizeof(uavsal_loss_desc);
        case 19: return (int)sizeof(uavsal_conv_route);
    }
    return UAVSAL_EINVAL;
}

extern "C" const char* uavsal_build_info(void) {
#define UAVSAL_STR2(x) #x
#define UAVSAL_STR(x) UAVSAL_STR2(x)
    return "libuavsal_hip gfx950 abi " UAVSAL_STR(UAVSAL_ABI_VERSION) " (" __DATE__ " " __TIME__ ")";
}
```

iip_uavsal_saliency_amd/engine.py:

```python
from __future__ import annotations

import contextlib
import ctypes as C
from typing import Dict, Optional

import torch

from . import _lib as L
from .arena import ARENA_ALIGN, Arena, _ArenaRef, arena_conflict, plan_arena
from .views import OpView, V, _down, read_view
from .recorder import PRIOR_GROUP, Recorder
from .topology import record_forward
from .weights import WeightCache


class PriorCache:

    def __init__(self, lib, plan, ops):
        self.lib, self.plan, self.ops = lib, plan, sorted(ops)
        self.marked = self.off = False
        self.rec = self.new = None
        self.group_launches = 0

    def mark(self):
# ... 55 lines not shown
        s = self.rec.get("same") if self.rec is not None else None
        if isinstance(s, tuple):
            ev, word = s
            if not ev.query():
                return False
            s = self.rec["same"] = bool(word[0])
        return s is True

    def bound(self):
        return self.rec["bound"]

    @contextlib.contextmanager
    def launches(self):
        try:
            yield
        except Exception:
            self.rec = self.new = None
            raise
        if self.new is not None:
            self.rec = dict(self.new, confirmed=False)
            self.new = None

    def confirm(self):
        if self.rec is not None:
            self.rec["confirmed"] = True

    def drop(self):
        self.rec = None


class Engine:
    def __init__(self, model, device, n_seq, seq_len, H, W, ctx_T, ctx_mode="tile",
                 precision="f32", taps=False, in_dtype=torch.float32, use_graph=False, fuse_dw=None,
                 use_lanes=True, stream_k=True, sync_errors=True, persistent=False,
                 wcache=None, static_priors=False, plan_only=False):
        if precision not in L.PREC:
            raise ValueError("precision must be one of %s" % list(L.PREC))
        self.lib = L.load()
        self.device = torch.device(device)
        self.plan_only = bool(plan_only)
        if self.device.type != "cuda" and not self.plan_only:
            raise RuntimeError("Engine needs a cuda (ROCm) device; there is no CPU fallback")
        self.model, self.n_seq, self.seq_len = model, n_seq, seq_len
        self.N = n_seq * seq_len
        self.H, self.W = H, W
        self.ctx_T, self.ctx_mode = ctx_T, ctx_mode
        self.prec_name, self.prec = precision, L.PREC[precision]
        self.keep_taps = taps
        self.in_dtype = in_dtype
        self.static_priors = bool(static_priors)
        self.use_graph = use_graph
        self.stream_k = bool(stream_k)
        self.sync_errors = bool(sync_errors)
        self._first_run_verified = False
        self._sk_debug = tuple(getattr(model, "_sk_debug", (0, 0)))
        self.fuse_dw = fuse_dw if fuse_dw is None else bool(fuse_dw)
        if self.N % ctx_T:
            raise RuntimeError("frame count %d is not a multiple of time_dims %d" % (self.N, ctx_T))
        self.h = _down(_down(_down(H)))
        self.w = _down(_down(_down(W)))
        self.weights = WeightCache(self.device, wcache if wcache is not None else {})
        self.lstm = getattr(model, "rnn_type", "twa") == "lstm"
        self.persistent = bool(persistent)
        presplit = getattr(model, "presplit", None)
        self.prec_overrides = dict(getattr(model, "prec_overrides", None) or {})
        for v in self.prec_overrides.values():
            if v not in L.PREC:
                raise ValueError("prec_overrides: unknown precision %r" % (v,))
        self.split_mode = (precision == "f16x3" and not self.prec_overrides
                           and (bool(presplit) if presplit is not None else n_seq >= 4))
        self.winograd = (precision == "f32" or bool(getattr(model, "prec_overrides", None))) and bool(getattr(model, "winograd", True))
        self.winograd_r = int(getattr(model, "winograd_r", None) or 4)
        self.winograd_step_r = int(getattr(model, "winograd_step_r", None)
                                   or (2 if getattr(model, "winograd_r", None) == 2 else 0))
        self.fuse_blocks = bool(getattr(model, "fuse_blocks", True))
        self.use_priors = tuple(bool(getattr(model, a, 1)) for a in ("use_gauss_prior", "use_ob_prior", "use_context_prior"))
        self.inplace = not use_graph
        self._bound_t: Dict[str, torch.Tensor] = {}
        self.priors = None
        self.use_arena = bool(getattr(model, "arena", True))
        self.arena_debug = bool(getattr(model, "arena_debug", False))
        self.rec = Recorder(torch, self.lib, self.device, self.weights, precision, self.prec_overrides, self.split_mode, self.stream_k,
                            self._sk_debug, self.fuse_dw, self.fuse_blocks, self.use_arena, self.arena_debug)
        if self.plan_only:
            self._size()
            return
        with torch.cuda.device(self.device):
            self._init_on_device(use_lanes)

    plan = property(lambda self: self.rec.plan)
    ops_meta = property(lambda self: self.rec.ops_meta)
    op_args = property(lambda self: self.rec.op_args)
    _op_idx = property(lambda self: self.rec.op_idx)
    named = property(lambda self: self.rec.named)
    stage_ranges = property(lambda self: self.rec.stage_ranges)
    arena = property(lambda self: self.rec.arena)
    _scratch = property(lambda self: self.rec.scratch)
    _sk_ws = property(lambda self: self.rec.sk_ws)
    x_in = property(lambda self: self.rec.callers["x"])
    cb0_in = property(lambda self: self.rec.callers["cb0"])
    cb1_in = property(lambda self: self.rec.callers["cb1"])
    state_in = property(lambda self: self.rec.callers["state_in"])
    state_out = property(lambda self: self.rec.callers["state_out"])
    cstate_in = property(lambda self: self.rec.callers["cstate_in"])
    cstate_out = property(lambda self: self.rec.callers["cstate_out"])
    zero_state = property(lambda self: self.rec.callers["zero_state"])
    out = property(lambda self: self.rec.callers["out"])
    logits = property(lambda self: self.rec.callers.get("logits"))
    _prior_rec = property(lambda self: self.priors.rec)
    prior_group_launches = property(lambda self: self.priors.group_launches if self.priors else 0)
    _arena = property(lambda self: self.arena.buf)
    arena_stats = property(lambda self: self.arena.stats)
    TAP_NAMES = ("c3", "c4", "c5", "sfnet", "st0", "st1", "fust_in_cb", "prefuse", "rnn")
    TAPS_ON_REQUEST = ("fu320", "cb192")

    def _size(self):
        self.rec.begin(dry=True)
        record_forward(self.rec, self)
        self.rec.place(self.TAP_NAMES + self.TAPS_ON_REQUEST if self.keep_taps else ())

    def arena_layout(self):
        return self.arena.layout()

    def _init_on_device(self, use_lanes, resume=False):
        if not resume:
            self._size()
        N, h, w = self.N, self.h, self.w
        f32, state = torch.float32, (self.n_seq, 256, h, w)
        stage = "shape" if self.inplace else "empty"
        np_ = 1 if self.static_priors else N
        callers = {"x": ((N, 3, self.H, self.W), self.in_dtype, stage), "cb0": ((np_, 8, h, w), f32, stage),
                   "cb1": ((np_, 20, h, w), f32, stage), "state_in": (state, f32, "zeros"),
                   "zero_state": (state, f32, "zeros"),
                   "state_out": (state, f32, "empty"), "cstate_in": (state, f32, "zeros"), "cstate_out": (state, f32, "empty"),
                   "out": ((N, h * w), f32, "empty")}
        if self.keep_taps:
            callers["logits"] = ((N, h * w), f32, "empty")
        rec = self.rec
        rec.allocate(callers)
        rec.begin(dry=False)
        record_forward(rec, self)
        rec.end()
        if self.persistent:
            self.h_view, self.c_view = (rec.named[k].t.view(self.n_seq, h, w, 256).permute(0, 3, 1, 2) if k in rec.named else None
                                        for k in ("h0", "c0"))
        self.priors = PriorCache(self.lib, rec.plan, rec.prior_ops)
        pw, dwpl = rec.op_idx.get("fucb.pw"), rec.op_idx.get("fucb.dwpl")
        self._fr = None
        if pw is not None and dwpl is not None and rec.ops_meta[pw]["kind"] == "conv1" and rec.ops_meta[dwpl]["kind"] == "conv1":
            self._fr = (pw, dwpl) + ((N // self.ctx_T, 1) if self.ctx_mode == "tile" else (N, self.ctx_T))
        self._fr_idx = None
        self.repeat_armed = False
        self._plan_recurrence_modes()
        self.use_lanes = bool(use_lanes)
        L.check(self.lib.uavsal_plan_enable_lanes(self.plan, 1 if self.use_lanes else 0), "plan_enable_lanes")
        self._graph_ready = False

    @staticmethod
    def _extent(v):
        t = v.t
        if isinstance(t, _ArenaRef):
            lo = t.arena.buf.data_ptr() + 4 * t.off
            return lo, lo + 4 * t.numel_
        if isinstance(t, torch.Tensor):
            return t.data_ptr(), t.data_ptr() + t.numel() * t.element_size()
        return None

    def seam_conflicts(self, prev, nxt):
        v = self._extent(nxt["v"])
        bad = []
        for k in ("m", "out", "a", "x", "pre"):
            e = self._extent(prev[k])
            if v is None or (e is not None and e[0] < v[1] and v[0] < e[1]):
                bad.append(k)
        return bad

    def _plan_recurrence_modes(self):
        self._seams, self._zs = [], None
        self._seams_on = None
        self._zs_rec = None
        self.zero_armed = False
        steps = self.rec.twa_steps
        if self.lstm or not self.inplace or self.arena_debug or not steps or any(s["r"] != 2 for s in steps):
            return
        for a, b in zip(steps, steps[1:]):
            if b["xin"] == a["xout"] + 1 and not self.seam_conflicts(a, b):
                self._seams.append((a["xout"], b["xin"]))
        lay = [i for i, m in enumerate(self.ops_meta) if m.get("name") == "state.in"]
        s0 = steps[0]
        if s0["gemm"] == s0["xin"] + 1 and s0["xout"] == s0["gemm"] + 1:
            self._zs = ((lay[0], lay[-1]) if lay else (-1, -1)) + (s0["xin"], s0["gemm"], s0["xout"])

    def _state_is_zero(self, state) -> bool:
        if state is None:
            return True
        try:
            base = state._base if state._base is not None else state
            sig = (state.data_ptr(), tuple(state.shape), tuple(state.stride()), state._version)
        except RuntimeError:
            return False
        if state.dtype != torch.float32 or state.device != self.device:
            return False
        r = self._zs_rec
        if r is not None and r["base"] is base and r["sig"] == sig:
            if isinstance(r["zero"], tuple):
                ev, word = r["zero"]
                if not ev.query():
                    return False
                r["zero"] = bool(word[0])
            return r["zero"]
        src = state if state.is_contiguous() else state.contiguous()
        ok = (src.view(torch.int32) == 0).all()
        word = torch.zeros(1, dtype=torch.bool).pin_memory()
        word.copy_(ok.reshape(1), non_blocking=True)
        ev = torch.cuda.Event()
        ev.record()
        self._zs_rec = dict(base=base, sig=sig, zero=(ev, word))
        return False

    def invalidate_zero_state(self):
        self._zs_rec = None

    def _arm_modes(self, zero):
        self.zero_armed = False
        want = bool(getattr(self.model, "fuse_seams", True))
        if self._seams and want != self._seams_on:
            for xo, xi in self._seams:
                r = self.lib.uavsal_plan_seam(self.plan, xo, xi, 1 if want else 0)
                if r < 0:
                    L.check(r, "plan_seam")
            self._seams_on = want
        if zero and self._zs is not None and bool(getattr(self.model, "skip_zero_state", True)):
            r = self.lib.uavsal_plan_zero_state(self.plan, *self._zs, 1)
            if r < 0:
                L.check(r, "plan_zero_state")
            self.zero_armed = r == 1

    def _disarm_modes(self):
        if self.zero_armed:
            self.lib.uavsal_plan_zero_state(self.plan, *self._zs, 0)

    def mode_report(self):
        out = (C.c_int * 4)()
        L.check(self.lib.uavsal_plan_mode_report(self.plan, C.byref(out)), "plan_mode_report")
        return int(out[0]), int(out[1]), int(out[2])

    def __del__(self):
        try:
            if getattr(self, "plan", None) and not getattr(self, "plan_only", False):
                self.lib.uavsal_plan_destroy(self.plan)
                self.rec.plan = None
        except Exception:
            pass

    def bound(self, name) -> torch.Tensor:
        return self._bound_t[name] if self.inplace else self.rec.callers[name]

    def _stream(self):
        return C.c_void_p(torch.cuda.current_stream(self.device).cuda_stream)

    def _prior_sig(self, srcs):
        sig = []
        for t, on in zip(srcs, self.use_priors[:2]):
            if not on:
                continue
            try:
                base = t._base if t._base is not None else t
                sig.append((base, t.data_ptr(), tuple(t.shape), tuple(t.stride()), t._version))
            except RuntimeError:
                return None
        return sig

    def drop_prior_record(self):
        self.priors.drop()

    def _prior_gate(self, srcs) -> bool:
        sig = self._prior_sig(srcs) if (self.inplace and bool(getattr(self.model, "cache_priors", True))) else None
        return self.priors.gate(sig, lambda: self.check(wait=True))

    def _arm_repeat(self, skip):
        self.repeat_armed = False
        if self._fr is None or not self.inplace:
            return
        pw, dwpl, mod, div = self._fr
        if not skip:
            if self._fr_idx is None:
                self._fr_idx = torch.tensor([(f // div * div) % mod for f in range(self.N)], dtype=torch.int64, device=self.device)
            self.priors.compare_frames(self._fr_idx)
        on = (skip and bool(getattr(self.model, "dedupe_priors", True)) and bool(getattr(self.model, "cache_priors", True))
              and self.priors.frames_repeat())
        r = self.lib.uavsal_plan_frame_repeat(self.plan, pw, dwpl, mod, div, 1 if on else 0)
        if r < 0:
            L.check(r, "plan_frame_repeat")
        self.repeat_armed = r == 1

    def _disarm_repeat(self):
        if self.repeat_armed:
            pw, dwpl, mod, div = self._fr
            self.lib.uavsal_plan_frame_repeat(self.plan, pw, dwpl, mod, div, 0)

    def repeat_workgroups(self):
        return tuple(int(self.lib.uavsal_plan_frame_repeat_workgroups(self.plan, i)) for i in (0, 1))

    def last_launches(self) -> int:
        return int(self.lib.uavsal_plan_last_launches(self.plan))

    def launch(self):
        self.priors.mark()
        if self.use_graph:
            cur = torch.cuda.current_stream(self.device)
            if not self._graph_ready:
                self._gstream = torch.cuda.Stream(self.device)
                self._gstream.wait_stream(cur)
                gs = C.c_void_p(self._gstream.cuda_stream)
                L.check(self.lib.uavsal_plan_run(self.plan, 0, -1, gs), "plan_run (warm-up)")
                self._gstream.synchronize()
                L.check(self.lib.uavsal_plan_graph_build(self.plan, gs), "plan_graph_build")
                self._graph_ready = True
            self._gstream.wait_stream(cur)
            L.check(self.lib.uavsal_plan_graph_launch(self.plan, C.c_void_p(self._gstream.cuda_stream)),
                    "plan_graph_launch")
            cur.wait_stream(self._gstream)
        else:
            if self.inplace and not self._bound_t:
                raise RuntimeError("launch-loop plan was never bound to the caller's tensors (Engine.run does that)")
            L.check(self.lib.uavsal_plan_run(self.plan, 0, -1, self._stream()), "plan_run")

    def _is_resident(self, t, view) -> bool:
        return (t is not None and view is not None and t.data_ptr() == view.data_ptr()
                and t.numel() == view.numel() and t.reshape(view.shape).stride() == view.stride())

    def _stage_state_persistent(self, state, cstate):
        pairs = [(state, self.h_view, self.state_in, "h0")]
        if self.c_view is not None:
            pairs.append((cstate, self.c_view, self.cstate_in, "c0"))
        self._resident_zero = False
        for t, view, stage, name in pairs:
            if self._is_resident(t, view):
                continue
            buf = self.named[name]
            if t is None:
                buf.t.zero_()
                if name == "h0":
                    self._resident_zero = True
                continue
            stage.copy_(t.reshape(stage.shape))
            d = L.LayoutDesc()
            d.inp, d.out, d.n_img, d.C, d.HW, d.ld, d.to_nhwc, d.Cpad = (
                stage.data_ptr(), buf.ptr, self.n_seq, 256, self.h * self.w, 256, 1, 0)
            L.check(self.lib.uavsal_layout(C.byref(d), self._stream()), "uavsal_layout(state)")

    def _bind_in_place(self, x, cb0, cb1, state, cstate, lstm, skip_priors=False):
        dev, callers = self.device, self.rec.callers
        bound = {"x": x.reshape(callers["x"].shape).contiguous()}
        if not skip_priors:
            for name, t, on in (("cb0", cb0, self.use_priors[0]), ("cb1", cb1, self.use_priors[1])):
                if not on:
                    continue
                if self.static_priors:
                    t = t[:1]
                bound[name] = t.reshape(callers[name].shape).contiguous()
            self.priors.note({k: bound[k] for k in ("cb0", "cb1") if k in bound})
        out = bound["out"] = torch.empty((self.N, self.h * self.w), dtype=torch.float32, device=dev)
        st = None
        if self.persistent:
            self._stage_state_persistent(state, cstate)
        else:
            shape = callers["state_in"].shape
            for nm, t in [("state", state)] + ([("cstate", cstate)] if lstm else []):
                bound[nm + "_in"] = callers["zero_state"] if t is None else t.reshape(shape).contiguous()
                bound[nm + "_out"] = torch.empty(shape, dtype=torch.float32, device=dev)
            st = (bound["state_out"], bound["cstate_out"]) if lstm else bound["state_out"]
        for name, op, slot, off in self.rec.binds:
            if name in bound:
                L.check(self.lib.uavsal_plan_patch_ptr(self.plan, op, slot, bound[name].data_ptr() + off), "plan_patch_ptr(%s)" % name)
        if skip_priors:
            bound.update(self.priors.bound())
        self._bound_t = bound
        return out, st

    def stage_inputs(self, x, cb0, cb1, state, cstate=None):
        self.x_in.copy_(x.reshape(self.x_in.shape))
        for t, stage, on in ((cb0, self.cb0_in, self.use_priors[0]), (cb1, self.cb1_in, self.use_priors[1])):
            if on:
                stage.copy_((t[:1] if self.static_priors else t).reshape(stage.shape))
        if self.persistent:
            return self._stage_state_persistent(state, cstate)
        if state is None:
            self.state_in.zero_()
        else:
            self.state_in.copy_(state.reshape(self.state_in.shape))
        if cstate is None:
            self.cstate_in.zero_()
        else:
            self.cstate_in.copy_(cstate.reshape(self.cstate_in.shape))

    def run(self, x, cb0, cb1, state=None, taps: Optional[dict] = None, cstate=None, prior_src=None):
        if x.dtype != self.in_dtype:
            raise RuntimeError("engine built for %s frames, got %s" % (self.in_dtype, x.dtype))
        lstm = self.lstm
        with torch.cuda.device(self.device):
            self.check(wait=False)
            skip = self._prior_gate(prior_src if prior_src is not None else (cb0, cb1))
            if self.inplace:
                out, st = self._bind_in_place(x, cb0, cb1, state, cstate, lstm, skip)
            else:
                self.stage_inputs(x, cb0, cb1, state, cstate)
            self._arm_repeat(skip)
            modes = self.inplace and bool(self._seams or self._zs)
            if modes:
                self._arm_modes(self._resident_zero if self.persistent else self._state_is_zero(state))
            with self.priors.launches():
                try:
                    self.launch()
                finally:
                    self._disarm_repeat()
                    if modes:
                        self._disarm_modes()
            if self.sync_errors:
                self.check(wait=True)
            if not self._first_run_verified and self.split_mode:
                self._first_run_verified = True
                self.check(wait=True)
                res = out if self.inplace else self.out
                if bool(torch.isnan(res).any().item()) and not bool(torch.isnan(x.float()).any().item()):
                    raise RuntimeError("the first run of this plan produced NaN maps from finite frames: a split shadow "
                                       "was read that no producer wrote (Recorder.no_shadow is missing a buffer)")
            if not self.inplace:
                out = self.out.clone()
                if self.persistent:
                    st = None
                else:
                    st = self.state_out.clone()
                    if lstm:
                        st = (st, self.cstate_out.clone())
            if self.persistent:
                st = (self.h_view, self.c_view) if lstm else self.h_view
            if taps is not None:
                if not self.keep_taps:
                    raise RuntimeError("engine was built without taps")
                for k in self.TAPS_ON_REQUEST:
                    if k in taps:
                        if k not in self.named:
                            raise RuntimeError("this plan has no buffer %r to tap (a model without priors)" % k)
                        taps[k] = self.tap(k, channels_last=True)
                for k in self.TAP_NAMES:
                    if k in self.named:
                        taps[k] = self.tap(k)
                taps["logits"] = self.logits.clone().view(self.N, 1, self.h, self.w)
        return out, st

    def state_split(self) -> int:
        for i, m in enumerate(self.ops_meta):
            if m.get("name", "").startswith(("twa.step0", "lstm.step0")):
                return i
        raise RuntimeError("plan has no recurrence step")

    def run_streamed(self, x, cb0, cb1, prev: Optional["Engine"] = None, prev_done: Optional[torch.cuda.Event] = None, reset=False):
        if not (self.persistent and self.inplace):
            raise RuntimeError("run_streamed needs the resident-state launch-loop plan (model.persistent_state = True, no graph)")
        lstm = self.lstm
        with torch.cuda.device(self.device):
            self.check(wait=False)
            skip = self._prior_gate((cb0, cb1))
            out, _ = self._bind_in_place(x, cb0, cb1, self.h_view, self.c_view, lstm, skip)
            split = self.state_split()
            self._arm_repeat(skip)
            with self.priors.launches():
                try:
                    L.check(self.lib.uavsal_plan_run(self.plan, 0, split, self._stream()), "plan_run(head)")
                finally:
                    self._disarm_repeat()
                cur = torch.cuda.current_stream(self.device)
                if prev_done is not None:
                    cur.wait_event(prev_done)
                for name in ("h0", "c0") if lstm else ("h0",):
                    mine = self.named[name].t
                    if reset:
                        mine.zero_()
                    elif prev is not None and prev is not self:
                        mine.copy_(prev.named[name].t)
                self._arm_modes(bool(reset))
                try:
                    L.check(self.lib.uavsal_plan_run(self.plan, split, -1, self._stream()), "plan_run(tail)")
                finally:
                    self._disarm_modes()
        return out

    def check(self, wait=True):
        code = self.lib.uavsal_plan_status(self.plan, 1 if wait else 0)
        if code == 0:
            if wait:
                self.priors.confirm()
            return
        self.priors.drop()
        if code == -5:
            torch.cuda.synchronize(self.device)
            for ws in self._sk_ws.values():
                ws[:65536].zero_()
            raise RuntimeError("UAVSal HIP path: a stream-K hand-off timed out on the device "
                               "(UAVSAL_ERR_STREAMK); the maps and state of that call are invalid (NaN-filled)")
        L.check(code, "uavsal_plan_status")

    def streamk_clean(self) -> bool:
        torch.cuda.synchronize(self.device)
        return all(int(ws[:65536].view(torch.int32).abs().sum().item()) == 0 for ws in self._sk_ws.values())

    def tap(self, name, channels_last=False) -> torch.Tensor:
        v = self.named[name]
        base = v.t.tensor() if isinstance(v.t, _ArenaRef) else v.t
        t = base.view(v.n, v.h, v.w, v.ld) if base.numel() == v.n * v.h * v.w * v.ld else None
        if t is None:
            raise RuntimeError("tap %s is not a dense buffer" % name)
        t = t[..., v.coff:v.coff + v.c]
        return t.contiguous().permute(0, 3, 1, 2) if channels_last else t.permute(0, 3, 1, 2).contiguous()

    def run_ops(self, first, last):
        if last > first:
            L.check(self.lib.uavsal_plan_run(self.plan, first, last, self._stream()), "plan_run")

    def time_ops(self, first, last, iters=10) -> float:
        ms = C.c_float(0.0)
        L.check(self.lib.uavsal_plan_time(self.plan, first, last, iters, self._stream(), C.byref(ms)), "plan_time")
        return float(ms.value)
```

iip_uavsal_saliency_amd/model.py:

```python
from __future__ import annotations

import os
from collections import OrderedDict
from typing import Dict, List, Optional, Sequence, Tuple

import numpy as np
import torch
import torch.nn as nn

from .model_convlstm import ConvLSTM, ConvTWA
from .model_feature import ReMobileNetV2, _no_eager

feature_inplanes = {"mobilenet_v2": [24, 32, 96, 320]}


def init_weights(model, funcname="kaiming_normal", **kwargs):
    fn = {"kaiming_normal": nn.init.kaiming_normal_, "kaiming_uniform": nn.init.kaiming_uniform_,
          "xavier_uniform": nn.init.xavier_uniform_, "xavier_normal": nn.init.xavier_normal_,
          "normal": nn.init.normal_, "uniform": nn.init.uniform_}[funcname]
    for m in model.modules():
        if isinstance(m, nn.Conv2d):
            fn(m.weight, **kwargs)
            if m.bias is not None:
                nn.init.zeros_(m.bias)
        elif isinstance(m, nn.BatchNorm2d):
            nn.init.ones_(m.weight)
            nn.init.zeros_(m.bias)


class BasicConv2d(nn.Sequential):

    def __init__(self, in_planes, out_planes, kernel_size=3, stride=1, dilation=1, groups=1):
        padding = dilation * (kernel_size - 1) // 2
        super().__init__(
            nn.Conv2d(in_planes, out_planes, kernel_size, stride, padding, dilation=dilation, groups=groups, bias=False),
            nn.BatchNorm2d(out_planes), nn.ReLU6(inplace=True))

    def forward(self, x):
        _no_eager("BasicConv2d")


class dwBlock(nn.Module):

    def __init__(self, inp, oup, kernel_size=3, stride=1, expand_ratio=6, dilation=1, res_connect=None):
        super().__init__()
        assert stride in (1, 2) and kernel_size == 3
        hidden = int(round(inp * expand_ratio))
        self.stride, self.dilation, self.expand_ratio = stride, dilation, expand_ratio
        self.cin, self.cout, self.hidden = inp, oup, hidden
        self.use_res_connect = stride == 1 and inp == oup
        if res_connect is not None:
            self.use_res_connect = bool(res_connect) and self.use_res_connect
        layers = []
        if expand_ratio != 1:
            layers.append(BasicConv2d(inp, hidden, kernel_size=1))
        layers += [BasicConv2d(hidden, hidden, kernel_size, stride=stride, dilation=dilation, groups=hidden),
                   nn.Conv2d(hidden, oup, 1, 1, 0, bias=False), nn.BatchNorm2d(oup)]
        self.conv = nn.Sequential(*layers)

    def forward(self, x):
        _no_eager("dwBlock")


class uavsal_srfnet_aspp(nn.Module):

    def __init__(self, cnn_type="mobilenet_v2", planes=(64, 64, 128, 256), last_channel=256):
        super().__init__()
        if cnn_type.lower() != "mobilenet_v2":
            raise NotImplementedError("the HIP path covers the mobilenet_v2 backbone (Demo_Test.py:33)")
        planes = list(planes)
        if last_channel == 128:
            planes = [32, 32, 64, 128]
        inpl = feature_inplanes["mobilenet_v2"]
        self.conv_lv3 = BasicConv2d(inpl[1], planes[1], 1)
        self.conv_lv4 = BasicConv2d(inpl[2], planes[2], 1)
        self.lv5_aspp1 = BasicConv2d(inpl[3], planes[3], 1)
        self.lv5_aspp2 = dwBlock(inpl[3], planes[3], 3, dilation=6)
        self.lv5_aspp3 = dwBlock(inpl[3], planes[3], 3, dilation=12)
        self.lv5_aspp4 = dwBlock(inpl[3], planes[3], 3, dilation=18)
        self.conv_lv5 = BasicConv2d(planes[3] * 4, planes[3], 1)
        self.conv_last = BasicConv2d(planes[1] + planes[2] + planes[3], last_channel, 3)
        init_weights(self, "kaiming_normal", mode="fan_out")
        self.features = ReMobileNetV2(name="mobilenet_v2")

    def forward(self, x):
        _no_eager("uavsal_srfnet_aspp")


class spConv(nn.Module):
    def __init__(self, inplanes, planes=256, kernel_size=3, stride=1, expand_ratio=6, dilation=1, res_connect=False):
        super().__init__()
        self.spconv = dwBlock(inplanes, planes, kernel_size, stride, expand_ratio, dilation, res_connect)
        init_weights(self, "kaiming_normal", mode="fan_out")

    def forward(self, x):
        _no_eager("spConv")


class teConv_sub(nn.Module):
    def __init__(self, inplanes, planes=256, time_dims=8, reduction=8, res_connect=False):
        super().__init__()
        self.time_dims = time_dims
        self.res_connect = res_connect and inplanes == planes
        width = planes // reduction
        self.reduce_conv = BasicConv2d(inplanes, width, 1)
        self.sub_conv = dwBlock(2 * width, width, 3, res_connect=False)
        self.last_conv = BasicConv2d(width, planes, 1)
        init_weights(self, "kaiming_normal", mode="fan_out")

    def forward(self, x):
        _no_eager("teConv_sub")


class STBlock(nn.Module):
    def __init__(self, inplanes, planes=256, time_dims=8, fu_type="sum", res_connect=True, **kwargs):
        super().__init__()
        if fu_type.lower() != "sum":
            raise NotImplementedError("UAVSal builds STBlock with fu_type='sum' (model.py:274)")
        self.res_connect = res_connect and inplanes == planes
        self.time_dims, self.fu_type, self.inplanes, self.planes = time_dims, "sum", inplanes, planes
        self.stconv_sp = spConv(inplanes, planes, res_connect=False)
        self.stconv_te = teConv_sub(inplanes, planes, time_dims, res_connect=False, **kwargs)
        self.stconv_last = BasicConv2d(planes, planes, 1)
        init_weights(self, "kaiming_normal", mode="fan_out")

    def forward(self, x):
        _no_eager("STBlock")


class UAVSal(nn.Module):
    rnn_type = "twa"

    def __init__(self, cnn_type="mobilenet_v2", time_dims=5, num_stblock=2, bias_type=[1, 1, 1],
                 iosize=[360, 640, 45, 80], planes=256, pre_model_path="", precision="f32"):
        super().__init__()
        bias_type = [int(b) for b in bias_type]
        if len(bias_type) != 3 or any(b not in (0, 1) for b in bias_type):
            raise ValueError("bias_type must be three 0/1 flags [gauss, observed, context] (reference model.py:281-284)")
        if planes != 256:
            raise NotImplementedError("planes=256 is the only configuration on the Demo_Test path")
        self.time_dims = time_dims
        self.precision = precision
        self.use_graph = False
        self.fuse_dw = None
        self.use_lanes = True
        self.stream_k = True
        self.presplit = None
        self.fuse_blocks = True
        self.winograd = True
        self.prec_overrides = None
        self.winograd_r = None
        self.sync_errors = None
        self.persistent_state = False
        self.dedupe_priors = True
        self.cache_priors = True
        self.fuse_seams = True
        self.skip_zero_state = True
        self.arena = True
        self.arena_debug = False
        self.max_engines = 4
        self.check_weight_versions = True
        self.sfnet = uavsal_srfnet_aspp(cnn_type, last_channel=planes)
        self.num_stblock = num_stblock
        self.st_layer = nn.Sequential(*[
            STBlock(planes, planes, time_dims=time_dims, reduction=planes // 32, res_connect=True)
            for _ in range(num_stblock)])
        self.fust_layer = nn.Sequential(dwBlock(planes, planes, kernel_size=3))
        self.use_gauss_prior, self.use_ob_prior, self.use_context_prior = bias_type
        self.num_cb = int(np.sum(np.array(bias_type) > 0))
        if self.use_gauss_prior:
            self.gauss_cb_layer = nn.Sequential(dwBlock(8, 64, kernel_size=3), dwBlock(64, 64, kernel_size=3))
            init_weights(self.gauss_cb_layer)
        if self.use_ob_prior:
            self.ob_cb_layer = nn.Sequential(dwBlock(20, 64, kernel_size=3), dwBlock(64, 64, kernel_size=3))
            init_weights(self.ob_cb_layer)
        if self.use_context_prior:
            self.cxt_cb_prior = nn.Sequential(dwBlock(planes, 64, kernel_size=3, stride=2),
                                              dwBlock(64, 64, kernel_size=3, stride=2))
            init_weights(self.cxt_cb_prior)
        if self.num_cb:
            self.fucb_layer = nn.Sequential(dwBlock(64 * self.num_cb, planes // 4, kernel_size=3))
            self.fucbst_layer = nn.Sequential(dwBlock(planes + planes // 4, planes, kernel_size=3))
        _, _, shape_r_out, shape_c_out = iosize
        rnn_cls = ConvLSTM if self.rnn_type == "lstm" else ConvTWA
        self.rnn = rnn_cls((shape_r_out, shape_c_out), planes, planes, kernel_size=(3, 3), num_layers=1,
                           batch_first=True, bias=False, return_all_layers=False)
        self.conv_out_st = dwBlock(planes, 1, kernel_size=3)
        init_weights(self.st_layer, "kaiming_normal", mode="fan_out")
        init_weights(self.fust_layer, "kaiming_normal", mode="fan_out")
        init_weights(self.conv_out_st, "kaiming_normal", mode="fan_out")
        self._engines: "OrderedDict[tuple, object]" = OrderedDict()
        self._wshared: Dict[str, dict] = {}
        self._wversion = None
        if pre_model_path and os.path.exists(pre_model_path):
            from .checkpoint import load_reference_state_dict
            self.load_state_dict(load_reference_state_dict(pre_model_path), strict=False)

    def replica(self):
        import copy
        r = copy.copy(self)
        r._wshared, r._wversion = self._wshared, self._wversion
        for k in ("_wtensors", "_wvers"):
            if k in self.__dict__:
                setattr(r, k, self.__dict__[k])
        return r

    _RUNTIME_STATE = ("_engines", "_wshared", "_wversion", "_wtensors", "_wvers", "_stream_replicas", "_stream_streams")

    def __getstate__(self):
        return {k: v for k, v in self.__dict__.items() if k not in self._RUNTIME_STATE}

    def __setstate__(self, state):
        super().__setstate__(state)
        self._engines = OrderedDict()
        self._wshared = {}
        self._wversion = None

    def _drop_engines(self):
        self._engines = OrderedDict()
        self._wshared = {}
        self._wversion = None

    invalidate_engines = _drop_engines

    def refresh_weights(self, *modules, device=False, fused_t=False):
        from .weights import WeightCache
        if self._wversion is None or "_wtensors" not in self.__dict__:
            return 0
        mods = {id(s): s for m in modules for s in m.modules()}
        mine = {id(t) for m in modules for t in list(m.parameters()) + list(m.buffers())}
        then = self.__dict__.get("_wvers")
        if then is None or any(t._version != v for t, v in zip(self._wtensors, then) if id(t) not in mine):
            self._drop_engines()
            return 0
        caches = [WeightCache(dev, store) for dev, store in self._wshared.items()]
        if device and any(c.device.type == "cpu" for c in caches):
            raise ValueError("refresh_weights(device=True) needs packed weights on a GPU: this model holds a CPU store")
        kw = {"fused_t": True} if fused_t else {}
        for c in caches:
            (c.refresh_device if device else c.refresh)(mods, dry=True, **kw)
        n = sum(c.refresh_device(mods, **kw) if device else c.refresh(mods, **kw) for c in caches)
        for m in [self] + list(self.__dict__.get("_stream_replicas") or []):
            if m._wversion is not None and "_wtensors" in m.__dict__:
                m._wversion = m._weights_version()
                m._wvers = [t._version for t in m._wtensors]
        nets = [getattr(self, a, None) for a in ("gauss_cb_layer", "ob_cb_layer")]
        if any(id(s) in mods for net in nets if net is not None for s in net.modules()):
            self.invalidate_priors()
        return n

    def invalidate_priors(self):
        for m in [self] + list(self.__dict__.get("_stream_replicas") or []):
            for eng in list(m._engines.values()):
                eng.drop_prior_record()

    def invalidate_state(self):
        for m in [self] + list(self.__dict__.get("_stream_replicas") or []):
            for eng in list(m._engines.values()):
                eng.invalidate_zero_state()

    def _weights_version(self):
        return sum(t._version for t in self._wtensors)

    def check_errors(self):
        for eng in list(self._engines.values()):
            eng.check(wait=True)

    def load_state_dict(self, *args, **kwargs):
        out = super().load_state_dict(*args, **kwargs)
        self._drop_engines()
        return out

    def _apply(self, fn, *args, **kwargs):
        out = super()._apply(fn, *args, **kwargs)
        self._drop_engines()
        return out

    def train(self, mode: bool = True):
        if mode:
            self._drop_engines()
        return super().train(mode)

    @staticmethod
    def frame_invariant(cb, frame_dims=1):
        return all(all(t.shape[d] == 1 or t.stride(d) == 0 for d in range(frame_dims)) for t in cb)

    def _check_weights(self):
        if not self.check_weight_versions:
            return
        if self._wversion is not None and self._weights_version() != self._wversion:
            self._drop_engines()
        if self._wversion is None:
            self._wtensors = [t for k, t in self.state_dict(keep_vars=True).items()
                              if not k.endswith("num_batches_tracked")]
            self._wversion = self._weights_version()
            self._wvers = [t._version for t in self._wtensors]

    def _engine(self, device, n_seq, seq_len, H, W, ctx_mode, taps=False, in_dtype=torch.float32, sync_default=True, static_priors=False):
        from .engine import Engine
        self._check_weights()
        key = (str(device), n_seq, seq_len, H, W, self.time_dims if ctx_mode == "tile" else seq_len,
               ctx_mode, self.precision, bool(taps), in_dtype, bool(self.use_graph), self.rnn_type, self.fuse_dw, bool(self.use_lanes),
               bool(self.stream_k), bool(self.persistent_state), tuple(getattr(self, "_sk_debug", (0, 0))),
               self.presplit, bool(self.fuse_blocks), bool(getattr(self, "winograd", True)), getattr(self, "winograd_r", None),
               tuple(sorted((getattr(self, "prec_overrides", None) or {}).items())), bool(static_priors),
               bool(getattr(self, "arena", True)), bool(getattr(self, "arena_debug", False)))
        eng = self._engines.get(key)
        if eng is None:
            while len(self._engines) >= max(1, int(self.max_engines)):
                _, old = self._engines.popitem(last=False)
# ... 104 lines not shown
```

iip_uavsal_saliency_amd/ops.py:

```python
from __future__ import annotations

import ctypes as C
from typing import Optional

import torch

from . import _lib as L
from . import packing as P


def _stream(t):
    return C.c_void_p(torch.cuda.current_stream(t.device).cuda_stream)


def _nhwc_view(t: torch.Tensor):
    if t.dim() != 4 or t.dtype != torch.float32 or not t.is_cuda:
        raise RuntimeError("expected a float32 cuda NHWC tensor [n,h,w,c]")
    n, h, w, c = t.shape
    ld = t.stride(2) if w > 1 else (t.stride(1) if h > 1 else (t.stride(0) if n > 1 else c))
    ok = (c == 1 or t.stride(3) == 1) and (w == 1 or t.stride(2) == ld) \
        and (h == 1 or t.stride(1) == w * ld) and (n == 1 or t.stride(0) == h * w * ld)
    if not ok:
        raise RuntimeError("tensor is not an NHWC buffer (or channel slice of one)")
    return t.data_ptr(), ld, n, h, w, c
# ... 138 lines not shown
    wo.n_img, wo.H, wo.W, wo.C, wo.Mp, wo.R = n, h, w, cout, mp, r
    keep = [v, m, wp]
    if scale is not None:
        npad = P.roundup(cout, 32)
        s_ = P.pad_vec(scale, npad, 1.0).to(dev)
        b_ = P.pad_vec(bias, npad, 0.0).to(dev)
        keep += [s_, b_]
        wo.scale, wo.bias = s_.data_ptr(), b_.data_ptr()
    wo.act, wo.epi = act, L.EPI_AFFINE
    if res is not None:
        rp, ldr, *_ = _nhwc_view(res)
        wo.res, wo.ldr = rp, ldr
    if twa is not None:
        xp, ldr, *_ = _nhwc_view(twa[0])
        pp, ldx, *_ = _nhwc_view(twa[1])
        wo.epi, wo.res, wo.ldr, wo.aux, wo.ldx, wo.hprev, wo.ldh = L.EPI_TWA, xp, ldr, pp, ldx, ip, ldi
    L.check(lib.uavsal_wino_output(C.byref(wo), st), "uavsal_wino_output")
    torch.cuda.current_stream(dev).synchronize()
    return out


def twa_step(x_t, h_prev, pre_t, w_h, prec="f32", tile=0, stream_k=False, route=None):
    lib = L.load()
    ap, lda, n, h, w, c = _nhwc_view(h_prev)
    xp, ldr, *_ = _nhwc_view(x_t)
    pp, ldx, *_ = _nhwc_view(pre_t)
    out = torch.empty((n, h, w, c), dtype=torch.float32, device=x_t.device)
    d = L.ConvDesc()
    d.a, d.lda, d.a_img_stride = ap, lda, h * w
    d.w = 1 << 20
    d.out, d.ldc, d.o_img_stride = out.data_ptr(), c, h * w
    d.res, d.ldr, d.r_img_stride = xp, ldr, h * w
    d.aux, d.ldx, d.x_img_stride = pp, ldx, h * w
    d.n_img, d.H, d.W, d.Cin, d.Cout, d.taps = n, h, w, c, c, 9
    d.prec, d.act, d.epi, d.tile = L.PREC[prec], L.ACT_NONE, L.EPI_TWA, tile
    if stream_k:
        ws = torch.zeros(int(lib.uavsal_streamk_workspace_bytes()), dtype=torch.uint8, device=x_t.device)
        d.sk_ws, d.sk_ws_bytes = ws.data_ptr(), ws.numel()
    rt = L.conv_route(lib, d)
    if route is not None:
        route.update(rt._asdict())
    wp = P.pack_conv_weight(w_h, P.conv_weight_layout(prec, False, False, rt.tile, w_h.shape[-1])).to(x_t.device)
    d.w = wp.data_ptr()
    L.check(lib.uavsal_conv_gemm(C.byref(d), _stream(x_t)), "uavsal_conv_gemm(TWA)")
    torch.cuda.current_stream(x_t.device).synchronize()
    if stream_k:
        _streamk_outcome(ws, "uavsal_conv_gemm(TWA)")
    return out


def dw3x3(x, weight, scale, bias, stride=1, dilation=1, act=L.ACT_RELU6, out=None, split_out=False, dil_groups=None):
    lib = L.load()
    ip, ldi, n, h, w, c = _nhwc_view(x)
    ho, wo = (h - 1) // stride + 1, (w - 1) // stride + 1
    if split_out:
        sp = _empty_shadow(n, ho, wo, c, x.device)
        op, ldo = None, c
    else:
        if out is None:
            out = torch.empty((n, ho, wo, c), dtype=torch.float32, device=x.device)
        op, ldo, *_ = _nhwc_view(out)
    w9 = P.pack_dw_weight(weight).to(x.device)
    s, b = scale.float().contiguous().to(x.device), bias.float().contiguous().to(x.device)
    d = L.DwDesc()
    d.inp, d.ldi, d.w9c, d.scale, d.bias = ip, ldi, w9.data_ptr(), s.data_ptr(), b.data_ptr()
    d.out, d.ldo = op, ldo
    d.n_img, d.H, d.W, d.C, d.stride, d.dilation, d.act = n, h, w, c, stride, dilation, act
    if split_out:
        d.out_split, d.ldos = sp.data_ptr(), 2 * c
    if dil_groups:
        d.dil_group_c = c // len(dil_groups)
        for i, dl in enumerate(dil_groups):
            d.dil_groups[i] = dl
    L.check(lib.uavsal_dw3x3(C.byref(d), _stream(x)), "uavsal_dw3x3")
    torch.cuda.current_stream(x.device).synchronize()
    return sp if split_out else out


def dw3x3_dot(x, weight, scale, bias, w2, scale2, bias2, act=L.ACT_NONE):
    lib = L.load()
    ip, ldi, n, h, w, c = _nhwc_view(x)
    dev = x.device
    out = torch.empty((n, h, w, 1), dtype=torch.float32, device=dev)
    keep = [P.pack_dw_weight(weight).to(dev), scale.float().contiguous().to(dev), bias.float().contiguous().to(dev),
            w2.detach().float().reshape(-1).contiguous().to(dev), torch.as_tensor(scale2, dtype=torch.float32).reshape(1).to(dev),
            torch.as_tensor(bias2, dtype=torch.float32).reshape(1).to(dev)]
    d = L.DwDotDesc()
    d.inp, d.ldi = ip, ldi
    d.w9c, d.scale, d.bias, d.w2, d.scale2, d.bias2 = (t.data_ptr() for t in keep)
    d.out, d.ldo = out.data_ptr(), 1
    d.n_img, d.H, d.W, d.C, d.act = n, h, w, c, act
    L.check(lib.uavsal_dw3x3_dot(C.byref(d), _stream(x)), "uavsal_dw3x3_dot")
    torch.cuda.current_stream(dev).synchronize()
    return out


def fused_ir(x, w1, bn1, wd, bnd, w2, bn2, stride=1, residual=False, tile=0):
    lib = L.load()
    ip, ldi, n, h, w, cin = _nhwc_view(x)
    hid, cout = wd.shape[0], w2.shape[0]
    ho, wo = (h - 1) // stride + 1, (w - 1) // stride + 1
    out = torch.empty((n, ho, wo, cout), dtype=torch.float32, device=x.device)
    dev = x.device
    keep = []

    def up(t):
        t = t.detach().float().contiguous().to(dev)
        keep.append(t)
        return t.data_ptr()
    d = L.FusedIrDesc()
    d.inp, d.ldi = ip, ldi
    d.n_img, d.H, d.W, d.Cin, d.hidden, d.Cout, d.stride, d.tile = n, h, w, cin, hid, cout, stride, tile
    d.w1 = (1 << 20) if w1 is not None else None
    kind = int(lib.uavsal_fused_ir_supported(C.byref(d)))
    if not kind:
        raise RuntimeError("no fused inverted-residual instance for (Cin, hidden, Cout, stride) = %s" % ((cin, hid, cout, stride),))
    natural = kind == 2
    if w1 is not None:
        d.w1 = up(w1.reshape(hid, cin) if natural else w1.reshape(hid, cin).t())
        d.scale1, d.bias1 = up(bn1[0]), up(bn1[1])
    d.wd, d.scale_d, d.bias_d = up(P.pack_dw_weight(wd)), up(bnd[0]), up(bnd[1])
    d.w2, d.scale2, d.bias2 = up(w2.reshape(cout, hid) if natural else w2.reshape(cout, hid).t()), up(bn2[0]), up(bn2[1])
    if residual:
        d.res, d.ldr = ip, ldi
    d.out, d.ldo = out.data_ptr(), cout
    L.check(lib.uavsal_fused_ir(C.byref(d), _stream(x)), "uavsal_fused_ir")
    torch.cuda.current_stream(dev).synchronize()
    return out


def stem_conv(x_nchw, weight, scale, bias):
    lib = L.load()
    n, _, H, W = x_nchw.shape
    ho, wo = (H - 1) // 2 + 1, (W - 1) // 2 + 1
    out = torch.empty((n, ho, wo, 32), dtype=torch.float32, device=x_nchw.device)
    ws = P.pack_stem_weight(weight).to(x_nchw.device)
    s, b = scale.float().contiguous().to(x_nchw.device), bias.float().contiguous().to(x_nchw.device)
    x_nchw = x_nchw.contiguous()
    d = L.StemDesc()
    if x_nchw.dtype == torch.uint8:
        d.inp, d.in_u8 = None, x_nchw.data_ptr()
    else:
        d.inp, d.in_u8 = x_nchw.data_ptr(), None
    d.w, d.scale, d.bias, d.out, d.ldo = ws.data_ptr(), s.data_ptr(), b.data_ptr(), out.data_ptr(), 32
    d.n_img, d.H, d.W = n, H, W
    from .synth import IMAGENET_MEAN, IMAGENET_STD
    for i in range(3):
        d.mean[i], d.stdv[i] = IMAGENET_MEAN[i], IMAGENET_STD[i]
    L.check(lib.uavsal_stem_conv(C.byref(d), _stream(out)), "uavsal_stem_conv")
    torch.cuda.current_stream(out.device).synchronize()
    return out


def bilinear_ac(x, ho, wo, out=None, n_out=None, src_mod=None, src_div=1, split_out=False):
    lib = L.load()
    ip, ldi, n, h, w, c = _nhwc_view(x)
    n_out = n if n_out is None else n_out
    if out is None:
        out = torch.empty((n_out, ho, wo, c), dtype=torch.float32, device=x.device)
    op, ldo, *_ = _nhwc_view(out)
    d = L.BilinearDesc()
    d.inp, d.ldi, d.Hi, d.Wi, d.out, d.ldo, d.Ho, d.Wo = ip, ldi, h, w, op, ldo, ho, wo
    d.n_out, d.C, d.src_mod, d.src_div = n_out, c, (n_out if src_mod is None else src_mod), src_div
    if split_out:
        sp = _empty_shadow(n_out, ho, wo, c, x.device)
        d.out_split, d.ldos = sp.data_ptr(), 2 * c
    L.check(lib.uavsal_bilinear_ac(C.byref(d), _stream(x)), "uavsal_bilinear_ac")
    torch.cuda.current_stream(x.device).synchronize()
    return (out, sp) if split_out else out


def tdiff(x, seq_len):
    lib = L.load()
    ip, ldi, n, h, w, c = _nhwc_view(x)
    out = torch.empty((n, h, w, 2 * c), dtype=torch.float32, device=x.device)
    d = L.TdiffDesc()
    d.inp, d.ldi, d.out, d.ldo, d.n_img, d.HW, d.C, d.seq_len = ip, ldi, out.data_ptr(), 2 * c, n, h * w, c, seq_len
    L.check(lib.uavsal_tdiff(C.byref(d), _stream(x)), "uavsal_tdiff")
    return out


def tsum(x, T):
    lib = L.load()
    ip, ldi, n, h, w, c = _nhwc_view(x)
    out = torch.empty((n // T, h, w, c), dtype=torch.float32, device=x.device)
    d = L.TsumDesc()
    d.inp, d.ldi, d.out, d.ldo, d.n_groups, d.T, d.HW, d.C = ip, ldi, out.data_ptr(), c, n // T, T, h * w, c
    L.check(lib.uavsal_tsum(C.byref(d), _stream(x)), "uavsal_tsum")
    return out


def to_nhwc(x_nchw, cpad=0):
    lib = L.load()
    x_nchw = x_nchw.contiguous()
    n, c, h, w = x_nchw.shape
    ld = max(c, cpad)
    out = torch.empty((n, h, w, ld), dtype=torch.float32, device=x_nchw.device)
    d = L.LayoutDesc()
    d.inp, d.out, d.n_img, d.C, d.HW, d.ld, d.to_nhwc, d.Cpad = x_nchw.data_ptr(), out.data_ptr(), n, c, h * w, ld, 1, cpad
    L.check(lib.uavsal_layout(C.byref(d), _stream(out)), "uavsal_layout")
    return out


def to_nchw(x_nhwc):
    lib = L.load()
    ip, ld, n, h, w, c = _nhwc_view(x_nhwc)
    out = torch.empty((n, c, h, w), dtype=torch.float32, device=x_nhwc.device)
    d = L.LayoutDesc()
    d.inp, d.out, d.n_img, d.C, d.HW, d.ld, d.to_nhwc, d.Cpad = ip, out.data_ptr(), n, c, h * w, ld, 0, 0
    L.check(lib.uavsal_layout(C.byref(d), _stream(out)), "uavsal_layout")
    return out


def postprocess_predictions(maps, H, W):
    lib = L.load()
    if maps.dim() == 4:
        maps = maps[:, 0]
    maps = maps.contiguous()
    if maps.dtype != torch.float32 or not maps.is_cuda:
        raise RuntimeError("expected float32 cuda maps")
    n, h, w = maps.shape
    out = torch.empty((n, H, W), dtype=torch.uint8, device=maps.device)
    scratch = torch.empty((n,), dtype=torch.int32, device=maps.device)
    d = L.PostDesc()
    d.inp, d.out, d.scratch = maps.data_ptr(), out.data_ptr(), scratch.data_ptr()
    d.n_img, d.h, d.w, d.H, d.W = n, h, w, H, W
    L.check(lib.uavsal_postprocess(C.byref(d), _stream(maps)), "uavsal_postprocess")
    torch.cuda.current_stream(maps.device).synchronize()
    return out


def letterbox_geometry(h0: int, w0: int, R: int, C: int):
    h0, w0, R, C = int(h0), int(w0), int(R), int(C)
    if min(h0, w0, R, C) <= 0:
        raise RuntimeError("letterbox_geometry: sizes must be positive, got %r" % ((h0, w0, R, C),))
    if h0 / R > w0 / C:
        new_r, new_c, branch = R, (w0 * R) // h0, "cols"
    else:
        new_r, new_c, branch = (h0 * C) // w0, C, "rows"
    if new_r <= 0 or new_c <= 0:
        raise RuntimeError("letterbox_geometry: a %dx%d frame has no picture inside %dx%d (%dx%d)" % (h0, w0, R, C, new_r, new_c))
    return new_r, new_c, (R - new_r) // 2, (C - new_c) // 2, branch


def letterbox_frames(frames, H, W, layout="HWC", bgr=False):
    lib = L.load()
    if not torch.is_tensor(frames) or not frames.is_cuda or frames.dtype != torch.uint8 or frames.dim() != 4:
        raise RuntimeError("expected uint8 cuda frames [F,H0,W0,3] (layout='HWC') or [F,3,H0,W0] (layout='CHW')")
    if layout not in ("HWC", "CHW"):
        raise RuntimeError("layout must be 'HWC' or 'CHW', got %r" % (layout,))
    F = frames.shape[0]
    if layout == "HWC":
        _, h0, w0, c = frames.shape
        st = frames.stride()
        dense = (st[3] == 1 or c == 1) and (st[2] == 3 or w0 == 1)
        row, plane, img = (st[1] if h0 > 1 else 3 * w0), 0, st[0]
    else:
        _, c, h0, w0 = frames.shape
        st = frames.stride()
        dense = st[3] == 1 or w0 == 1
        row = st[2] if h0 > 1 else w0
        plane, img = st[1], st[0]
    if c != 3:
        raise RuntimeError("expected 3 channels in dimension %d of %s frames, got shape %r" % (
            3 if layout == "HWC" else 1, layout, tuple(frames.shape)))
    letterbox_geometry(h0, w0, H, W)
    if F == 0:
        return torch.empty((0, 3, H, W), dtype=torch.uint8, device=frames.device)
    if not dense or row < (3 * w0 if layout == "HWC" else w0):
        raise RuntimeError("frames are not a %s buffer (or a slice of one): strides %r" % (layout, tuple(st)))
    out = torch.empty((F, 3, H, W), dtype=torch.uint8, device=frames.device)
    d = L.LetterboxDesc()
    d.src, d.dst = frames.data_ptr(), out.data_ptr()
    d.row_pitch, d.plane_pitch, d.img_pitch = row, plane, (img if F > 1 else 0)
    d.n_img, d.h0, d.w0, d.R, d.C = F, h0, w0, H, W
    d.layout, d.swap_rb = (L.LETTERBOX_HWC if layout == "HWC" else L.LETTERBOX_CHW), int(bool(bgr))
    L.check(lib.uavsal_letterbox_u8(C.byref(d), _stream(frames)), "uavsal_letterbox_u8")
    return out


def _gaze_view(t, name, layout):
    if not torch.is_tensor(t) or not t.is_cuda or t.dtype != torch.uint8:
        raise RuntimeError("prepare_gaze: %s must be a uint8 cuda tensor" % name)
    if t.dim() == 4:
        if t.shape[2] != 1:
            raise RuntimeError("prepare_gaze: a 4-d %s is the .mat layout [H0,W0,1,F], got %r" % (name, tuple(t.shape)))
        return t[:, :, 0, :].permute(2, 0, 1)
    if t.dim() != 3 or layout not in (None, "FHW", "HWF"):
        raise RuntimeError("prepare_gaze: %s must be [F,H0,W0], [H0,W0,F] (layout='HWF') or [H0,W0,1,F]" % name)
    return t.permute(2, 0, 1) if layout == "HWF" else t


def prepare_gaze(fix_map_u8, fix_loc_u8, h, w, layout=None):
    lib = L.load()
    m, l = _gaze_view(fix_map_u8, "fix_map", layout), _gaze_view(fix_loc_u8, "fix_loc", layout)
    if m.shape != l.shape or m.device != l.device:
        raise RuntimeError("prepare_gaze: fix_map %r and fix_loc %r differ" % (tuple(m.shape), tuple(l.shape)))
    F, h0, w0 = m.shape
    h, w = int(h), int(w)
    letterbox_geometry(h0, w0, h, w)
    nbytes = F * 2 * h * w * 4
    buf = torch.zeros(nbytes + 2 * F, dtype=torch.uint8, device=m.device)
    y = buf[:nbytes].view(torch.float32).view(F, 2, h, w)
    flags = buf[nbytes:].view(F, 2)
    if F == 0:
        return y, flags.view(torch.bool)
# ... 90 lines not shown
```

include/uavsal_hip.h:

```cpp
#ifndef UAVSAL_HIP_H
#define UAVSAL_HIP_H

#include <stdint.h>

#ifdef __cplusplus
extern "C" {
#endif

#define UAVSAL_ABI_VERSION 20

#define UAVSAL_EINVAL   (-1)
#define UAVSAL_EALIGN   (-2)
#define UAVSAL_ESHAPE   (-3)
#define UAVSAL_ESTATE   (-4)
#define UAVSAL_EDEVICE  (-5)

#define UAVSAL_ERR_STREAMK  1

#define UAVSAL_PREC_F32     0
#define UAVSAL_PREC_BF16X3  1
#define UAVSAL_PREC_BF16    2
#define UAVSAL_PREC_F16X3   3

#define UAVSAL_ACT_NONE     0
#define UAVSAL_ACT_RELU6    1
#define UAVSAL_ACT_SIGMOID  2

#define UAVSAL_EPI_AFFINE   0
#define UAVSAL_EPI_TWA      1
#define UAVSAL_EPI_LSTM     2

typedef void* uavsal_stream_t;

typedef struct uavsal_conv_desc {
    const float* a;      int32_t lda;  int64_t a_img_stride;
    const void*  w;
    const float* scale;  const float* bias;
    float*       out;    int32_t ldc;  int64_t o_img_stride;
    const float* res;    int32_t ldr;  int64_t r_img_stride;
    const float* aux;    int32_t ldx;  int64_t x_img_stride;
    int32_t n_img, H, W;
    int32_t Cin, Cout, taps;
    int32_t prec, act, epi;
    int32_t tile;
    float*       out2;   int32_t ld2;
    const float* dw_w9c; const float* dw_scale; const float* dw_bias;
    int32_t dw_stride, dw_Hin, dw_Win;
    void* sk_ws; int64_t sk_ws_bytes;
    const void* a_split;  int32_t ldas;
    void* out_split;      int32_t ldos;
    int32_t* err;
    int32_t sk_spin_limit;
    int32_t sk_debug_drop;
    int64_t w_group_stride;
    int32_t n_group, a_group_off;
} uavsal_conv_desc;

int uavsal_conv_gemm(const uavsal_conv_desc* d, uavsal_stream_t stream);
long long uavsal_streamk_workspace_bytes(void);

enum { UAVSAL_ROUTE_PRESPLIT = 1, UAVSAL_ROUTE_DWPROJ, UAVSAL_ROUTE_STREAMK, UAVSAL_ROUTE_K32, UAVSAL_ROUTE_F32_DMA,
       UAVSAL_ROUTE_STAGED };
enum { UAVSAL_REDUCE_NONE = 0, UAVSAL_REDUCE_LAUNCH, UAVSAL_REDUCE_IN_LAUNCH };
typedef struct uavsal_conv_route {
    int32_t family;
    int32_t tile;
    int32_t dwproj;
    int32_t streamk;
    int32_t ksplit;
    int32_t reduce;
} uavsal_conv_route;
int uavsal_conv_route_of(const uavsal_conv_desc* d, uavsal_conv_route* r);
int uavsal_conv_tile(const uavsal_conv_desc* d);
int uavsal_conv_uses_split(const uavsal_conv_desc* d);
int uavsal_conv_dwproj(const uavsal_conv_desc* d);
int uavsal_conv_streamk_grid(const uavsal_conv_desc* d);

typedef struct uavsal_dw_desc {
    const float* in;   int32_t ldi;
    const float* w9c;  const float* scale;  const float* bias;
    float*       out;  int32_t ldo;
    int32_t n_img, H, W, C, stride, dilation, act;
    void* out_split;  int32_t ldos;
    int32_t dil_group_c;  int32_t dil_groups[4];
} uavsal_dw_desc;

int uavsal_dw3x3(const uavsal_dw_desc* d, uavsal_stream_t stream);
int uavsal_dw_variant(const uavsal_dw_desc* d);

typedef struct uavsal_dw_dot_desc {
    const float* in;   int32_t ldi;
    const float* w9c;  const float* scale;  const float* bias;
    const float* w2;   const float* scale2; const float* bias2;
    float*       out;  int32_t ldo;
    int32_t n_img, H, W, C, act;
} uavsal_dw_dot_desc;

int uavsal_dw3x3_dot(const uavsal_dw_dot_desc* d, uavsal_stream_t stream);

typedef struct uavsal_fused_ir_desc {
    const float* in;   int32_t ldi;
    const float* w1;   const float* scale1;  const float* bias1;
    const float* wd;   const float* scale_d; const float* bias_d;
    const float* w2;   const float* scale2;  const float* bias2;
    const float* res;  int32_t ldr;
    float*       out;  int32_t ldo;
    int32_t n_img, H, W, Cin, hidden, Cout, stride;
    int32_t tile;
} uavsal_fused_ir_desc;

int uavsal_fused_ir(const uavsal_fused_ir_desc* d, uavsal_stream_t stream);
int uavsal_fused_ir_supported(const uavsal_fused_ir_desc* d);

typedef struct uavsal_stem_desc {
    const float*   in;
    const uint8_t* in_u8;
    const float* w;  const float* scale;  const float* bias;
    float* out;  int32_t ldo;
    int32_t n_img, H, W;
    float mean[3], stdv[3];
} uavsal_stem_desc;

int uavsal_stem_conv(const uavsal_stem_desc* d, uavsal_stream_t stream);

typedef struct uavsal_bilinear_desc {
    const float* in;  int32_t ldi;  int32_t Hi, Wi;
    float* out;       int32_t ldo;  int32_t Ho, Wo;
    int32_t n_out, C, src_mod, src_div;
    void* out_split;  int32_t ldos;
} uavsal_bilinear_desc;

int uavsal_bilinear_ac(const uavsal_bilinear_desc* d, uavsal_stream_t stream);

typedef struct uavsal_tdiff_desc {
    const float* in;  int32_t ldi;
    float* out;       int32_t ldo;
    int32_t n_img, HW, C, seq_len;
} uavsal_tdiff_desc;

int uavsal_tdiff(const uavsal_tdiff_desc* d, uavsal_stream_t stream);

typedef struct uavsal_wino_desc {
    const float* in;   int32_t ldi;  int64_t in_img_stride;
    float* out;        int32_t ldo;  int64_t out_img_stride;
    int32_t n_img, H, W, C;
    int64_t Mp;
    int32_t R;
    const float* scale; const float* bias;
    int32_t act, epi;
    const float* res;   int32_t ldr;  int64_t res_img_stride;
    const float* aux;   int32_t ldx;  int64_t aux_img_stride;
    const float* hprev; int32_t ldh;  int64_t h_img_stride;
    int32_t n_seg;
    const float* seg_in[3];  int32_t seg_ld[3], seg_c[3], seg_H[3], seg_W[3];
} uavsal_wino_desc;

int uavsal_wino_input(const uavsal_wino_desc* d, uavsal_stream_t stream);
int uavsal_wino_output(const uavsal_wino_desc* d, uavsal_stream_t stream);
int uavsal_wino_output_zero_h(const uavsal_wino_desc* d, uavsal_stream_t stream);
int uavsal_wino_seam(const uavsal_wino_desc* xout, const uavsal_wino_desc* xin, uavsal_stream_t stream);
int uavsal_wino_seam_zero_h(const uavsal_wino_desc* xout, const uavsal_wino_desc* xin, uavsal_stream_t stream);
int uavsal_wino_seam_check(const uavsal_wino_desc* xout, const uavsal_wino_desc* xin);

typedef struct uavsal_tsum_desc {
    const float* in;  int32_t ldi;
    float* out;       int32_t ldo;
    int32_t n_groups, T, HW, C;
} uavsal_tsum_desc;

int uavsal_tsum(const uavsal_tsum_desc* d, uavsal_stream_t stream);

typedef struct uavsal_layout_desc {
    const float* in;  float* out;
    int32_t n_img, C, HW, ld, to_nhwc, Cpad;
} uavsal_layout_desc;

int uavsal_layout(const uavsal_layout_desc* d, uavsal_stream_t stream);

typedef struct uavsal_post_desc {
    const float* in;  uint8_t* out;  void* scratch;
    int32_t n_img, h, w, H, W;
} uavsal_post_desc;

int uavsal_postprocess(const uavsal_post_desc* d, uavsal_stream_t stream);

#define UAVSAL_LETTERBOX_HWC 0
#define UAVSAL_LETTERBOX_CHW 1

typedef struct uavsal_letterbox_desc {
    const uint8_t* src;  uint8_t* dst;
    int64_t row_pitch, plane_pitch, img_pitch;
    int32_t n_img, h0, w0, R, C;
    int32_t layout, swap_rb;
} uavsal_letterbox_desc;

int uavsal_letterbox_u8(const uavsal_letterbox_desc* d, uavsal_stream_t stream);

typedef struct uavsal_overlay_desc {
    const uint8_t* frames;  int64_t row_pitch, plane_pitch, img_pitch;
    const uint8_t* map;  int64_t map_img_pitch;
    const uint8_t* fix;  const uint8_t* lut;
    uint8_t* out;  void* ws;  int64_t ws_bytes;
    int32_t n_img, layout, h0, w0, map_h, map_w, fix_h, fix_w;
    int32_t mid_h, mid_w, out_h, out_w;
} uavsal_overlay_desc;

int64_t uavsal_overlay_workspace_bytes(const uavsal_overlay_desc* d);
int uavsal_overlay_u8(const uavsal_overlay_desc* d, uavsal_stream_t stream);

typedef struct uavsal_copy_desc {
    const float* in;  float* out;
    int64_t in_pitch, out_pitch, row_floats;  int32_t rows;
} uavsal_copy_desc;

int uavsal_copy_rows(const uavsal_copy_desc* d, uavsal_stream_t stream);

typedef struct uavsal_fill_desc {
    uint32_t* out;  int64_t n;  uint32_t bits;
} uavsal_fill_desc;

int uavsal_fill(const uavsal_fill_desc* d, uavsal_stream_t stream);

typedef struct uavsal_guard_desc {
    const int32_t* err;  int32_t* host_err;
    float* buf[3];  int64_t n[3];
} uavsal_guard_desc;

int uavsal_guard(const uavsal_guard_desc* d, uavsal_stream_t stream);

#define UAVSAL_SCORE_NSTAT 16
#define UAVSAL_SCORE_REPS  100
#define UAVSAL_SCORE_RUN   4096
#define UAVSAL_SCORE_NKEY  7

typedef struct uavsal_score_desc {
    const void* sal;  const void* fix_loc;  const float* fix_map;
    const float* jitter;
    int32_t sal_u8, loc_u8, n_frames, n_pix;
    double* stats;
    const int64_t* fix_off;  const int64_t* run_off;  int64_t total_fix;  int32_t total_runs;
    int32_t nan_rows;
    const int32_t* samp[2];  const int64_t* samp_off[2];  int64_t n_samp[2];
    void* ws;  int64_t ws_bytes;
    float* out;  int32_t n_keys;  int32_t keys[UAVSAL_SCORE_NKEY];
} uavsal_score_desc;

int64_t uavsal_score_workspace_bytes(const uavsal_score_desc* d);
int uavsal_score_stats(const uavsal_score_desc* d, uavsal_stream_t stream);
int uavsal_score_run(const uavsal_score_desc* d, uavsal_stream_t stream);

typedef struct uavsal_gaze_desc {
    const uint8_t* fix_map;  int64_t map_row_pitch, map_col_pitch, map_img_pitch;
    const uint8_t* fix_loc;  int64_t loc_row_pitch, loc_col_pitch, loc_img_pitch;
    float* out;  uint8_t* flags;
    int32_t n_img, h0, w0, h, w;
} uavsal_gaze_desc;

int uavsal_gaze_prepare(const uavsal_gaze_desc* d, uavsal_stream_t stream);

#define UAVSAL_LOSS_NSTAT 16

typedef struct uavsal_loss_desc {
    const float* pred;  const float* truth;
    double* stats;
    float* out;
    const float* grad_out;  float* grad;
    int32_t n_img, n_pix;
    double w_kl, w_cc, w_nss;
} uavsal_loss_desc;

int uavsal_loss_fu(const uavsal_loss_desc* d, uavsal_stream_t stream);
int uavsal_loss_fu_grad(const uavsal_loss_desc* d, uavsal_stream_t stream);

#define UAVSAL_PRIOR_MIN_SLAB 32

typedef struct uavsal_prior_acc_desc {
// ... 291 lines not shown
int uavsal_ir_sums_dil_slabs(const uavsal_ir_sums_dil_desc* d);
int uavsal_ir_sums_dil_slab_rows(const uavsal_ir_sums_dil_desc* d);
int uavsal_ir_sums_dil(const uavsal_ir_sums_dil_desc* d, uavsal_stream_t stream);
int uavsal_srf_sizeof_desc(int which);

#define UAVSAL_SKINNY_UNIT 128
#define UAVSAL_SKINNY_SHARES 1024
#define UAVSAL_SKINNY_MAX_NARROW 32
#define UAVSAL_SKINNY_MAX_WIDE 192

typedef struct uavsal_skinny_wgrad_desc {
    const float* a;  int32_t lda;
    const float* b;  int32_t ldb;
    const float* row_scale;
    const float* w;  int32_t ldw;
    double* rowdot;
    float* ws;  int64_t ws_bytes;
    float* out;  int32_t ldo;
    int64_t K;  int32_t M, N, accumulate;
} uavsal_skinny_wgrad_desc;

int64_t uavsal_skinny_wgrad_workspace_bytes(const uavsal_skinny_wgrad_desc* d);
int uavsal_skinny_wgrad_shares(const uavsal_skinny_wgrad_desc* d);
int uavsal_skinny_wgrad(const uavsal_skinny_wgrad_desc* d, uavsal_stream_t stream);
int uavsal_shallow_sizeof_desc(int which);

typedef struct uavsal_bn_stats_desc {
    const float* u;  int32_t ld;
    const float* gamma;  const float* beta;
    float* running_mean;  float* running_var;
    double eps, momentum;
    double* ws;  int64_t ws_bytes;
    float* mu;  float* var;  float* r;  float* s;  float* b;
    int32_t n_img, H, W, C;
} uavsal_bn_stats_desc;

typedef struct uavsal_bn_apply_desc {
    const float* u;  int32_t ld;
    const float* s;  const float* b;
    const float* dot_w;
    float* out;
    int64_t n_pix;  int32_t C, act;
} uavsal_bn_apply_desc;

typedef struct uavsal_bn_bwd_desc {
    const float* g;  int32_t ldg;
    const float* g_pix;  const float* g_chan;
    const float* u;  int32_t ld;
    const float* s;  const float* b;  const float* mu;  const float* r;
    double* ws;  int64_t ws_bytes;
    double* sums;
    float* g_gamma;  float* g_beta;  float* g_w;
    float* gu;
    int32_t n_img, H, W, C, act, accumulate;
} uavsal_bn_bwd_desc;

typedef struct uavsal_dw_wgrad_desc {
    const float* g;  int32_t ldg;
    const float* e;  int32_t lde;
    double* ws;  int64_t ws_bytes;
    float* out;
    int32_t n_img, H, W, C, accumulate;
} uavsal_dw_wgrad_desc;

int uavsal_bn_slabs(int n_img, int H, int W);
int uavsal_bn_slab_rows(int n_img, int H, int W);
int64_t uavsal_bn_stats_workspace_bytes(const uavsal_bn_stats_desc* d);
int uavsal_bn_stats(const uavsal_bn_stats_desc* d, uavsal_stream_t stream);
int uavsal_bn_apply(const uavsal_bn_apply_desc* d, uavsal_stream_t stream);
int64_t uavsal_bn_bwd_workspace_bytes(const uavsal_bn_bwd_desc* d);
int uavsal_bn_bwd_sums(const uavsal_bn_bwd_desc* d, uavsal_stream_t stream);
int uavsal_bn_bwd_apply(const uavsal_bn_bwd_desc* d, uavsal_stream_t stream);
int64_t uavsal_dw_wgrad_workspace_bytes(const uavsal_dw_wgrad_desc* d);
int uavsal_dw_wgrad(const uavsal_dw_wgrad_desc* d, uavsal_stream_t stream);
int uavsal_bn_sizeof_desc(int which);

typedef struct uavsal_bn_apply_res_desc {
    const float* u;  int32_t ld;
    const float* s;  const float* b;
    const float* res;  int32_t ldr;
    float* out;
    int64_t n_pix;  int32_t C, act;
} uavsal_bn_apply_res_desc;

int uavsal_bn_apply_res(const uavsal_bn_apply_res_desc* d, uavsal_stream_t stream);
int uavsal_block_bn_sizeof_desc(int which);

#define UAVSAL_REPACK_MAX_SRC 4
#define UAVSAL_REPACK_MAX_BLOCKS (1 << 24)
enum { UAVSAL_REPACK_CONV = 0, UAVSAL_REPACK_WINO = 1, UAVSAL_REPACK_FOLD = 2, UAVSAL_REPACK_DW = 3, UAVSAL_REPACK_COPY = 4,
       UAVSAL_REPACK_COPY_T = 5 };
enum { UAVSAL_REPACK_F32 = 0, UAVSAL_REPACK_F16X3 = 1, UAVSAL_REPACK_F16X3I = 2, UAVSAL_REPACK_F16X3J = 3, UAVSAL_REPACK_BF16 = 4,
       UAVSAL_REPACK_BF16X3 = 5 };
enum { UAVSAL_REPACK_SCALE = 0, UAVSAL_REPACK_BIAS = 1, UAVSAL_REPACK_RSTD = 2, UAVSAL_REPACK_MEAN = 3 };

typedef struct uavsal_repack_entry {
    int32_t kind, layout;
    void* dst;
    int64_t units;
    const float* src[UAVSAL_REPACK_MAX_SRC];
    const float* beta[UAVSAL_REPACK_MAX_SRC];
    const float* mean[UAVSAL_REPACK_MAX_SRC];
    const float* var[UAVSAL_REPACK_MAX_SRC];
    double eps[UAVSAL_REPACK_MAX_SRC];
    int32_t rows[UAVSAL_REPACK_MAX_SRC];
    int32_t n_src;
    int32_t N, C, taps, Npad, Kpad, kt, flip, gi;
    int32_t P;
    int64_t sN, sC, off;
    const float* sg;  const float* sv;  double seps;
    float pad;  int32_t reserved;
    double G[18];
} uavsal_repack_entry;

int uavsal_repack(const void* table, int n_entries, int n_blocks, uavsal_stream_t stream);
int uavsal_repack_sizeof_desc(void);

typedef struct uavsal_plan uavsal_plan;

uavsal_plan* uavsal_plan_create(void);
void uavsal_plan_destroy(uavsal_plan* p);
int uavsal_plan_add_conv(uavsal_plan* p, const uavsal_conv_desc* d);
int uavsal_plan_add_dw(uavsal_plan* p, const uavsal_dw_desc* d);
int uavsal_plan_add_dw_dot(uavsal_plan* p, const uavsal_dw_dot_desc* d);
int uavsal_plan_add_stem(uavsal_plan* p, const uavsal_stem_desc* d);
int uavsal_plan_add_bilinear(uavsal_plan* p, const uavsal_bilinear_desc* d);
int uavsal_plan_add_tdiff(uavsal_plan* p, const uavsal_tdiff_desc* d);
int uavsal_plan_add_wino_input(uavsal_plan* p, const uavsal_wino_desc* d);
int uavsal_plan_add_wino_output(uavsal_plan* p, const uavsal_wino_desc* d);
int uavsal_plan_add_tsum(uavsal_plan* p, const uavsal_tsum_desc* d);
int uavsal_plan_add_layout(uavsal_plan* p, const uavsal_layout_desc* d);
int uavsal_plan_add_copy(uavsal_plan* p, const uavsal_copy_desc* d);
int uavsal_plan_add_fused_ir(uavsal_plan* p, const uavsal_fused_ir_desc* d);
int uavsal_plan_add_fill(uavsal_plan* p, const uavsal_fill_desc* d);
int32_t* uavsal_plan_error_word(uavsal_plan* p);
int uavsal_plan_add_guard(uavsal_plan* p, float* b0, int64_t n0, float* b1, int64_t n1, float* b2, int64_t n2);
int uavsal_plan_status(uavsal_plan* p, int wait);
int uavsal_plan_patch_ptr(uavsal_plan* p, int op, int slot, void* ptr);
int uavsal_plan_set_lane(uavsal_plan* p, int lane);
int uavsal_plan_add_fork(uavsal_plan* p, int lane);
int uavsal_plan_add_join(uavsal_plan* p, int lane);
int uavsal_plan_enable_lanes(uavsal_plan* p, int on);
int uavsal_plan_size(const uavsal_plan* p);
int uavsal_plan_run(uavsal_plan* p, int first, int last, uavsal_stream_t stream);
int uavsal_plan_group_mark(uavsal_plan* p, int group, int first, int last);
int uavsal_plan_group_enable(uavsal_plan* p, int group, int on);
int uavsal_plan_group_launches(const uavsal_plan* p, int group);
int uavsal_plan_last_launches(const uavsal_plan* p);
int uavsal_plan_frame_repeat(uavsal_plan* p, int op_pw, int op_dwpl, int src_mod, int src_div, int on);
int uavsal_plan_frame_repeat_workgroups(const uavsal_plan* p, int which);
int uavsal_plan_seam(uavsal_plan* p, int op_xout, int op_xin, int on);
int uavsal_plan_zero_state(uavsal_plan* p, int op_state_in_first, int op_state_in_last, int op_xin0, int op_gemm0, int op_xout0, int on);
int uavsal_plan_mode_report(const uavsal_plan* p, int out[4]);
int uavsal_plan_graph_build(uavsal_plan* p, uavsal_stream_t stream);
int uavsal_plan_graph_launch(uavsal_plan* p, uavsal_stream_t stream);

int uavsal_plan_time(uavsal_plan* p, int first, int last, int iters, uavsal_stream_t stream, float* ms);

int uavsal_abi_version(void);
int uavsal_sizeof_desc(int which);
const char* uavsal_build_info(void);

#ifdef __cplusplus
}
#endif
#endif
```

Before: 1997 frames/s.

## Fuse stem conv into features.1 inverted-residual kernel with recomputed halo

```diff
diff --git a/iip_uavsal_saliency_amd/_lib.py b/iip_uavsal_saliency_amd/_lib.py
--- a/iip_uavsal_saliency_amd/_lib.py
+++ b/iip_uavsal_saliency_amd/_lib.py
@@ -594,6 +594,10 @@
     ("uavsal_plan_seam", C.c_int, [C.c_void_p, C.c_int, C.c_int, C.c_int]),
     ("uavsal_plan_zero_state", C.c_int, [C.c_void_p, C.c_int, C.c_int, C.c_int, C.c_int, C.c_int, C.c_int]),
     ("uavsal_plan_mode_report", C.c_int, [C.c_void_p, C.POINTER(C.c_int * 4)]),
+    ("uavsal_stem_fused_ir", C.c_int, [C.POINTER(StemDesc), C.POINTER(FusedIrDesc), C.c_void_p]),
+    ("uavsal_stem_fused_ir_check", C.c_int, [C.POINTER(StemDesc), C.POINTER(FusedIrDesc)]),
+    ("uavsal_plan_stem_pair", C.c_int, [C.c_void_p, C.c_int, C.c_int, C.c_int]),
+    ("uavsal_plan_stem_pair_report", C.c_int, [C.c_void_p]),
     ("uavsal_plan_graph_build", C.c_int, [C.c_void_p, C.c_void_p]),
     ("uavsal_plan_graph_launch", C.c_int, [C.c_void_p, C.c_void_p]),
     ("uavsal_plan_time", C.c_int, [C.c_void_p, C.c_int, C.c_int, C.c_int, C.c_void_p, C.POINTER(C.c_float)]),
diff --git a/iip_uavsal_saliency_amd/csrc/fused_ir.hip b/iip_uavsal_saliency_amd/csrc/fused_ir.hip
--- a/iip_uavsal_saliency_amd/csrc/fused_ir.hip
+++ b/iip_uavsal_saliency_amd/csrc/fused_ir.hip
@@ -1,4 +1,5 @@
 #include "common.h"
+#include "stem_px.h"
 
 namespace {
 
@@ -62,9 +63,22 @@
 #define FIR_STAMP(i)
 #endif
 
-template <int CIN, int HID, int COUT, int S, bool EXPAND, int HC, int TX, int PT>
-__global__ __launch_bounds__(256, 2) void fused_ir_kernel(const FusedK p) {
+struct StemSrc {
+    const float* in; const uint8_t* in_u8; const float* w; const float* scale; const float* bias;
+    int H, W;
+    float mean[3], stdv[3];
+};
+
+constexpr int STEM_XP = 40;
+template <int IH> constexpr int stem_lds_floats() { return 3 * (2 * IH + 1) * STEM_XP + 27 * 32 + 64; }
+
+template <bool STEM> struct FusedArgs : FusedK {};
+template <> struct FusedArgs<true> : FusedK { StemSrc stem; };
+
+template <int CIN, int HID, int COUT, int S, bool EXPAND, int HC, int TX, int PT, bool STEM = false>
+__global__ __launch_bounds__(256, 2) void fused_ir_kernel(const FusedArgs<STEM> p) {
     using Cfg = FusedCfg<CIN, HID, COUT, S, EXPAND, HC, TX, PT>;
+    static_assert(!STEM || (!EXPAND && S == 1 && CIN == 32), "the stem feeds features.1");
     constexpr int RP = Cfg::RP, TY = Cfg::TY, IH = Cfg::IH, IW = Cfg::IW, HALF = Cfg::HALF, IWP = Cfg::IWP;
     constexpr int NSLOT = Cfg::NSLOT, NRT = Cfg::NRT, RTW = (NRT + 3) / 4;
     constexpr int CPL = HC / 4, CQ = CPL / 4, PLANE = Cfg::PLANE, SLOTF = Cfg::SLOTF;
@@ -130,6 +144,78 @@
                 }
             }
         }
+    } else if constexpr (STEM) {
+        constexpr int XR = 2 * IH + 1, XW = 2 * IW + 1, XP = STEM_XP, XROWS = 3 * XR;
+        constexpr int GP = 6, GPR = IW / GP, NIT = IH * GPR * 8, NRND = (NIT + 255) / 256;
+        static_assert(XP >= XW && XP % 4 == 0 && IW % GP == 0 && (2 * GP) % 4 == 0 && IWP == IW && EBUF % 4 == 0, "stem patch");
+        float* const xsh = lds + EBUF;
+        float* const wsh = xsh + XROWS * XP;
+        float* const ssh = wsh + 27 * 32;
+        float* const bsh = ssh + 32;
+        const int sy0 = oy0 - 1, sx0 = ox0 - 1;
+        const int xy0 = 2 * sy0 - 1, xx0 = 2 * sx0 - 1;
+        const size_t plane = (size_t)p.stem.H * p.stem.W;
+        constexpr int NXL = (XROWS * XP + 255) / 256;
+        float st[NXL];
+#pragma unroll
+        for (int i = 0; i < NXL; ++i) {
+            const int idx = tid + 256 * i;
+            const int r = idx / XP, c = idx - r * XP;
+            const int ci = r / XR, iy = xy0 + (r - ci * XR), ix = xx0 + c;
+            float x = 0.f;
+            if (r < XROWS && c < XW && iy >= 0 && iy < p.stem.H && ix >= 0 && ix < p.stem.W)
+                x = stem_sample(p.stem.in, p.stem.in_u8, ((size_t)n * 3 + ci) * plane + (size_t)iy * p.stem.W + ix, p.stem.mean[ci], p.stem.stdv[ci]);
+            st[i] = x;
+        }
+        for (int i = tid; i < 27 * 32; i += 256) wsh[i] = p.stem.w[i];
+        if (tid < 32) { ssh[tid] = p.stem.scale[tid]; bsh[tid] = p.stem.bias[tid]; }
+#pragma unroll
+        for (int i = 0; i < NXL; ++i) {
+            const int idx = tid + 256 * i;
+            if (idx < XROWS * XP) xsh[idx] = st[i];
+        }
+        for (int idx = NSLOT * 8 + tid; idx < NRT * 16 * 8; idx += 256)
+            *reinterpret_cast<f32x4*>(lds + (size_t)(idx & 7) * PLANE + (idx >> 3) * SLOTF) = (f32x4){0.f, 0.f, 0.f, 0.f};
+        __syncthreads();
+#pragma unroll 1
+        for (int rnd = 0; rnd < NRND; ++rnd) {
+            const int item = tid + 256 * rnd;
+            if (item >= NIT) break;
+            const int g = item & 7, grp = item >> 3;
+            const int r = grp / GPR, c0 = (grp - r * GPR) * GP;
+            f32x4 acc[GP];
+#pragma unroll
+            for (int q = 0; q < GP; ++q) acc[q] = (f32x4){0.f, 0.f, 0.f, 0.f};
+#pragma unroll 1
+            for (int ci = 0; ci < 3; ++ci) {
+#pragma unroll
+                for (int ky = 0; ky < 3; ++ky) {
+                    const float* row = xsh + (ci * XR + 2 * r + ky) * XP + 2 * c0;
+                    float v[2 * GP + 1];
+#pragma unroll
+                    for (int c = 0; c < 2 * GP / 4; ++c) {
+                        const f32x4 a = *reinterpret_cast<const f32x4*>(row + 4 * c);
+                        v[4 * c] = a.x; v[4 * c + 1] = a.y; v[4 * c + 2] = a.z; v[4 * c + 3] = a.w;
+                    }
+                    v[2 * GP] = row[2 * GP];
+#pragma unroll
+                    for (int kx = 0; kx < 3; ++kx) {
+                        const f32x4 w4 = *reinterpret_cast<const f32x4*>(wsh + (ci * 9 + ky * 3 + kx) * 32 + g * 4);
+#pragma unroll
+                        for (int q = 0; q < GP; ++q) acc[q] = stem_tap(w4, v[2 * q + kx], acc[q]);
+                    }
+                }
+            }
+            const f32x4 sc = *reinterpret_cast<const f32x4*>(ssh + g * 4), bi = *reinterpret_cast<const f32x4*>(bsh + g * 4);
+            const int sy = sy0 + r;
+#pragma unroll
+            for (int q = 0; q < GP; ++q) {
+                const int sx = sx0 + c0 + q;
+                f32x4 e = stem_bn_relu6(acc[q], sc, bi);
+                if (sy < 0 || sy >= p.H || sx < 0 || sx >= p.W) e = (f32x4){0.f, 0.f, 0.f, 0.f};
+                *reinterpret_cast<f32x4*>(lds + (size_t)g * PLANE + (r * IWP + c0 + q) * SLOTF) = e;
+            }
+        }
     } else {
         constexpr int NQ = CIN / 4, NST = (NRT * 16 * NQ + 255) / 256;
         f32x4 st[NST];
@@ -311,10 +397,33 @@
     FIR_STAMP(4)
 }
 
+template <int PT>
+int launch_stem_fused(const uavsal_stem_desc* sd, const uavsal_fused_ir_desc* d, hipStream_t s) {
+    using Cfg = FusedCfg<32, 32, 16, 1, false, 32, 16, PT>;
+    constexpr size_t SMEM = Cfg::SMEM + (size_t)stem_lds_floats<Cfg::IH>() * 4;
+    static_assert(Cfg::SMEM == (size_t)Cfg::EBUF * 4 && 2 * SMEM <= 160 * 1024, "the frame patch lies behind the one E buffer; two workgroups per CU");
+    FusedArgs<true> k;
+    StemSrc& sk = k.stem;
+    k.in = d->in; k.w1 = nullptr; k.s1 = nullptr; k.b1 = nullptr;
+    k.wd = d->wd; k.sd = d->scale_d; k.bd = d->bias_d;
+    k.w2 = d->w2; k.s2 = d->scale2; k.b2 = d->bias2;
+    k.res = nullptr; k.out = d->out;
+    k.ldi = d->ldi; k.ldr = 0; k.ldo = d->ldo; k.H = d->H; k.W = d->W;
+    k.Ho = d->H; k.Wo = d->W;
+    k.tiles_x = (k.Wo + 15) / 16; k.tiles_y = (k.Ho + Cfg::TY - 1) / Cfg::TY;
+    sk.in = sd->in; sk.in_u8 = sd->in_u8; sk.w = sd->w; sk.scale = sd->scale; sk.bias = sd->bias; sk.H = sd->H; sk.W = sd->W;
+    for (int i = 0; i < 3; ++i) { sk.mean[i] = sd->mean[i]; sk.stdv[i] = sd->stdv[i]; }
+    const long long nblk = (long long)d->n_img * k.tiles_y * k.tiles_x;
+    if (nblk > 0x7fffffffLL) return UAVSAL_ESHAPE;
+    UAVSAL_LDS_OPTIN((&fused_ir_kernel<32, 32, 16, 1, false, 32, 16, PT, true>), SMEM);
+    hipLaunchKernelGGL((fused_ir_kernel<32, 32, 16, 1, false, 32, 16, PT, true>), dim3((unsigned)nblk), dim3(256), SMEM, s, k);
+    return uavsal_launch_status();
+}
+
 template <int CIN, int HID, int COUT, int S, bool EXPAND, int HC, int TX, int PT>
 int launch_fused(const uavsal_fused_ir_desc* d, hipStream_t s) {
     using Cfg = FusedCfg<CIN, HID, COUT, S, EXPAND, HC, TX, PT>;
-    FusedK k;
+    FusedArgs<false> k;
     k.in = d->in; k.w1 = d->w1; k.s1 = d->scale1; k.b1 = d->bias1;
     k.wd = d->wd; k.sd = d->scale_d; k.bd = d->bias_d;
     k.w2 = d->w2; k.s2 = d->scale2; k.b2 = d->bias2;
@@ -386,7 +495,35 @@
     return mid ? mid : dispatch(d, nullptr, false);
 }
 
+static int fused_ir_args(const uavsal_fused_ir_desc* d);
+
+extern "C" int uavsal_stem_fused_ir_check(const uavsal_stem_desc* sd, const uavsal_fused_ir_desc* d) {
+    if (!sd || (!sd->in && !sd->in_u8) || !sd->w || !sd->scale || !sd->bias || !sd->out) return UAVSAL_EINVAL;
+    if (sd->n_img <= 0 || sd->H <= 0 || sd->W <= 0) return UAVSAL_EINVAL;
+    if ((sd->ldo & 3) || sd->ldo < 32 || !uavsal_aligned16(sd->out)) return UAVSAL_EALIGN;
+    if (!d) return UAVSAL_EINVAL;
+    if (const int e = fused_ir_args(d)) return e;
+    if (d->Cin != 32 || d->hidden != 32 || d->Cout != 16 || d->stride != 1 || d->w1) return UAVSAL_ESHAPE;
+    if (d->res) return UAVSAL_ESHAPE;
+    if (d->in != sd->out || d->ldi != sd->ldo) return UAVSAL_ESHAPE;
+    if (d->n_img != sd->n_img || d->H != (sd->H - 1) / 2 + 1 || d->W != (sd->W - 1) / 2 + 1) return UAVSAL_ESHAPE;
+    return 0;
+}
+
+extern "C" int uavsal_stem_fused_ir(const uavsal_stem_desc* sd, const uavsal_fused_ir_desc* d, uavsal_stream_t stream) {
+    if (const int e = uavsal_stem_fused_ir_check(sd, d)) return e;
+    const long long big = (long long)d->n_img * ((d->H + 15) / 16) * ((d->W + 15) / 16);
+    const bool use_big = d->tile == 2 || (d->tile == 0 && big >= UAVSAL_FUSED_BIG_MIN);
+    return use_big ? launch_stem_fused<4>(sd, d, (hipStream_t)stream) : launch_stem_fused<1>(sd, d, (hipStream_t)stream);
+}
+
 extern "C" int uavsal_fused_ir(const uavsal_fused_ir_desc* d, uavsal_stream_t stream) {
+    if (const int e = fused_ir_args(d)) return e;
+    if (uavsal_fused_mid_dispatch(d, nullptr, false)) return uavsal_fused_mid_dispatch(d, (hipStream_t)stream, true);
+    return dispatch(d, (hipStream_t)stream, true);
+}
+
+static int fused_ir_args(const uavsal_fused_ir_desc* d) {
     if (!d || !d->in || !d->wd || !d->scale_d || !d->bias_d || !d->w2 || !d->scale2 || !d->bias2 || !d->out) return UAVSAL_EINVAL;
     if (d->w1 && (!d->scale1 || !d->bias1)) return UAVSAL_EINVAL;
     if (d->n_img <= 0 || d->H <= 0 || d->W <= 0) return UAVSAL_EINVAL;
@@ -398,6 +535,5 @@
     if ((d->w1 && !uavsal_aligned16(d->w1)) || !uavsal_aligned16(d->w2)) return UAVSAL_EALIGN;
     if (d->tile < 0 || d->tile > 2) return UAVSAL_EINVAL;
     if (d->res && (d->ldr < d->Cout || d->stride != 1 || d->Cin != d->Cout)) return UAVSAL_ESHAPE;
-    if (uavsal_fused_mid_dispatch(d, nullptr, false)) return uavsal_fused_mid_dispatch(d, (hipStream_t)stream, true);
-    return dispatch(d, (hipStream_t)stream, true);
-}
+    return 0;
+}
diff --git a/iip_uavsal_saliency_amd/csrc/glue.hip b/iip_uavsal_saliency_amd/csrc/glue.hip
--- a/iip_uavsal_saliency_amd/csrc/glue.hip
+++ b/iip_uavsal_saliency_amd/csrc/glue.hip
@@ -1,4 +1,5 @@
 #include "common.h"
+#include "stem_px.h"
 
 namespace {
 
@@ -32,9 +33,7 @@
         const int ci = r / ST_IH, iy = iy0 + (r - ci * ST_IH), ix = ix0 + c;
         float x = 0.f;
         if (r < ST_ROWS && c < ST_IW && iy >= 0 && iy < p.H && ix >= 0 && ix < p.W) {
-            const size_t at = ((size_t)n * 3 + ci) * plane + (size_t)iy * p.W + ix;
-            if (p.in_u8) x = ((float)p.in_u8[at] / 255.0f - p.mean[ci]) / p.stdv[ci];
-            else x = p.in[at];
+            x = stem_sample(p.in, p.in_u8, ((size_t)n * 3 + ci) * plane + (size_t)iy * p.W + ix, p.mean[ci], p.stdv[ci]);
         }
         st[i] = x;
     }
@@ -68,7 +67,7 @@
             for (int kx = 0; kx < 3; ++kx) {
                 const f32x4 w4 = *reinterpret_cast<const f32x4*>(wsh + (ci * 9 + ky * 3 + kx) * 32 + g * 4);
 #pragma unroll
-                for (int q = 0; q < 8; ++q) acc[q] = w4 * v[2 * q + kx] + acc[q];
+                for (int q = 0; q < 8; ++q) acc[q] = stem_tap(w4, v[2 * q + kx], acc[q]);
             }
         }
     }
@@ -78,8 +77,7 @@
     for (int q = 0; q < 8; ++q) {
         const int ox = oxb + q;
         if (ox >= p.Wo) break;
-        f32x4 r = acc[q] * sc + bi;
-        r.x = fminf(fmaxf(r.x, 0.f), 6.f); r.y = fminf(fmaxf(r.y, 0.f), 6.f); r.z = fminf(fmaxf(r.z, 0.f), 6.f); r.w = fminf(fmaxf(r.w, 0.f), 6.f);
+        const f32x4 r = stem_bn_relu6(acc[q], sc, bi);
         *reinterpret_cast<f32x4*>(p.out + (((size_t)n * p.Ho + oy) * p.Wo + ox) * p.ldo + g * 4) = r;
     }
 }
diff --git a/iip_uavsal_saliency_amd/csrc/plan.hip b/iip_uavsal_saliency_amd/csrc/plan.hip
--- a/iip_uavsal_saliency_amd/csrc/plan.hip
+++ b/iip_uavsal_saliency_amd/csrc/plan.hip
@@ -73,6 +73,8 @@
     int zs_first = -1, zs_last = -1, zs_xin = -1, zs_gemm = -1, zs_xout = -1;
     bool zs_on = false;
     int mode_seams = 0, mode_elided = 0, mode_kernels = 0;
+    int sp_stem = -1;
+    int mode_stem_pair = 0;
 };
 
 extern "C" uavsal_plan* uavsal_plan_create(void) { return new (std::nothrow) uavsal_plan(); }
@@ -260,7 +262,7 @@
         fr = cs == hipStreamCaptureStatusNone && !(a.group >= 0 && ((goff >> a.group) & 1u)) && !(b.group >= 0 && ((goff >> b.group) & 1u)) &&
              uavsal_conv_repeat_pair(&a.u.conv, &b.u.conv, p->fr_mod, p->fr_div) == 1;
     }
-    bool modes = repeat && (p->zs_on || !p->seam_next.empty());
+    bool modes = repeat && (p->zs_on || !p->seam_next.empty() || p->sp_stem >= 0);
     if (modes) {
         hipStreamCaptureStatus cs = hipStreamCaptureStatusNone;
         if (hipStreamIsCapturing((hipStream_t)stream, &cs) != hipSuccess) { (void)hipGetLastError(); cs = hipStreamCaptureStatusActive; }
@@ -271,7 +273,9 @@
     bool zs = modes && p->zs_on && p->zs_xin >= first && p->zs_xout < last && (p->zs_first < 0 || (p->zs_first >= first && p->zs_last < last)) &&
               !masked_out(p->zs_xin) && !masked_out(p->zs_gemm) && !masked_out(p->zs_xout);
     for (int i = p->zs_first; zs && i >= 0 && i <= p->zs_last; ++i) zs = !masked_out(i);
-    if (repeat && first == 0) p->mode_seams = p->mode_elided = p->mode_kernels = 0;
+    const bool sp = modes && p->sp_stem >= first && p->sp_stem + 1 < last && !masked_out(p->sp_stem) && !masked_out(p->sp_stem + 1) &&
+                    p->ops[p->sp_stem].lane == p->ops[p->sp_stem + 1].lane;
+    if (repeat && first == 0) p->mode_seams = p->mode_elided = p->mode_kernels = p->mode_stem_pair = 0;
     const bool lanes = p->lanes_on && first == 0 && last == n;
     const uint32_t off = masked ? p->groups_off : 0u;
     hipStream_t main_s = (hipStream_t)stream;
@@ -300,6 +304,14 @@
             ++*launched;
             continue;
         }
+        if (sp && i == p->sp_stem) {
+            e = uavsal_stem_fused_ir(&op.u.stem, &p->ops[i + 1].u.fir, s);
+            if (e) return e;
+            p->mode_stem_pair = 1; ++p->mode_kernels;
+            *launched += 2;
+            ++i;
+            continue;
+        }
         const bool seam = modes && i < (int)p->seam_next.size() && p->seam_next[i] == i + 1 && i + 1 < last && !masked_out(i + 1) &&
                           p->ops[i + 1].lane == op.lane;
         if (seam) {
@@ -362,6 +374,20 @@
     return 1;
 }
 
+extern "C" int uavsal_plan_stem_pair(uavsal_plan* p, int op_stem, int op_f1, int on) {
+    const int n = p ? (int)p->ops.size() : 0;
+    if (!p || op_stem < 0 || op_f1 < 0 || op_stem >= n || op_f1 >= n) return UAVSAL_EINVAL;
+    if (p->ops[op_stem].kind != OP_STEM || p->ops[op_f1].kind != OP_FUSED_IR) return UAVSAL_EINVAL;
+    if (p->sp_stem == op_stem) p->sp_stem = -1;
+    if (!on || p->exec || op_f1 != op_stem + 1 || p->ops[op_f1].lane != p->ops[op_stem].lane ||
+        uavsal_stem_fused_ir_check(&p->ops[op_stem].u.stem, &p->ops[op_f1].u.fir) != 0)
+        return 0;
+    p->sp_stem = op_stem;
+    return 1;
+}
+
+extern "C" int uavsal_plan_stem_pair_report(const uavsal_plan* p) { return p ? p->mode_stem_pair : UAVSAL_EINVAL; }
+
 extern "C" int uavsal_plan_zero_state(uavsal_plan* p, int op_state_in_first, int op_state_in_last, int op_xin0, int op_gemm0,
                                       int op_xout0, int on) {
     const int n = p ? (int)p->ops.size() : 0;
@@ -398,6 +424,7 @@
     p->fr_on = false;
     p->zs_on = false;
     p->seam_next.clear();
+    p->sp_stem = -1;
     hipStream_t s = (hipStream_t)stream;
     hipError_t e = hipStreamBeginCapture(s, hipStreamCaptureModeThreadLocal);
     if (e != hipSuccess) return (int)e;
diff --git a/iip_uavsal_saliency_amd/csrc/stem_px.h b/iip_uavsal_saliency_amd/csrc/stem_px.h
--- /dev/null
+++ b/iip_uavsal_saliency_amd/csrc/stem_px.h
@@ -0,0 +1,17 @@
+#pragma once
+#include "common.h"
+
+__device__ __forceinline__ float stem_sample(const float* in, const uint8_t* in_u8, size_t at, float mean, float stdv) {
+    if (in_u8) return ((float)in_u8[at] / 255.0f - mean) / stdv;
+    return in[at];
+}
+
+__device__ __forceinline__ f32x4 stem_tap(f32x4 w, float x, f32x4 acc) {
+    return (f32x4){fmaf(w.x, x, acc.x), fmaf(w.y, x, acc.y), fmaf(w.z, x, acc.z), fmaf(w.w, x, acc.w)};
+}
+
+__device__ __forceinline__ f32x4 stem_bn_relu6(f32x4 acc, f32x4 sc, f32x4 bi) {
+    f32x4 r = {fmaf(acc.x, sc.x, bi.x), fmaf(acc.y, sc.y, bi.y), fmaf(acc.z, sc.z, bi.z), fmaf(acc.w, sc.w, bi.w)};
+    r.x = fminf(fmaxf(r.x, 0.f), 6.f); r.y = fminf(fmaxf(r.y, 0.f), 6.f); r.z = fminf(fmaxf(r.z, 0.f), 6.f); r.w = fminf(fmaxf(r.w, 0.f), 6.f);
+    return r;
+}
diff --git a/iip_uavsal_saliency_amd/engine.py b/iip_uavsal_saliency_amd/engine.py
--- a/iip_uavsal_saliency_amd/engine.py
+++ b/iip_uavsal_saliency_amd/engine.py
@@ -231,6 +231,7 @@
         self._fr_idx = None
         self.repeat_armed = False
         self._plan_recurrence_modes()
+        self._plan_stem_pair()
         self.use_lanes = bool(use_lanes)
         L.check(self.lib.uavsal_plan_enable_lanes(self.plan, 1 if self.use_lanes else 0), "plan_enable_lanes")
         self._graph_ready = False
@@ -269,6 +270,44 @@
         s0 = steps[0]
         if s0["gemm"] == s0["xin"] + 1 and s0["xout"] == s0["gemm"] + 1:
             self._zs = ((lay[0], lay[-1]) if lay else (-1, -1)) + (s0["xin"], s0["gemm"], s0["xout"])
+
+    def stem_pair_conflicts(self, stem_op, f1):
+        r = f1.t
+        if not isinstance(r, _ArenaRef):
+            return []
+        return [q.aid for q in self.arena.refs.values()
+                if q is not r and q.first is not None and q.first <= stem_op <= q.last
+                and q.off < r.off + r.numel_ and r.off < q.off + q.numel_]
+
+    def _plan_stem_pair(self):
+        self._stem_pair, self._stem_on = None, None
+        rec = self.rec
+        s, f = rec.op_idx.get("features.0"), rec.op_idx.get("features.1")
+        if not self.inplace or self.arena_debug or s is None or f != s + 1:
+            return
+        if rec.ops_meta[s]["kind"] != "stem" or rec.ops_meta[f]["kind"] != "fused_ir" or "f0" not in rec.named or "f1" not in rec.named:
+            return
+        f0, f1 = rec.named["f0"], rec.named["f1"]
+        users = [i for i, a in enumerate(rec.op_args)
+                 if any(isinstance(v, OpView) and v.buf is f0.t for v in a.values())]
+        if users != [s, f] or rec.op_args[s]["out"].buf is not f0.t or rec.op_args[f]["a"].buf is not f0.t:
+            return
+        if isinstance(f0.t, _ArenaRef) and (f0.t.first, f0.t.last) != (s, f):
+            return
+        if self.stem_pair_conflicts(s, f1):
+            return
+        self._stem_pair = (s, f)
+
+    def _arm_stem_pair(self):
+        want = bool(getattr(self.model, "fuse_stem", True))
+        if self._stem_pair is not None and want != self._stem_on:
+            r = self.lib.uavsal_plan_stem_pair(self.plan, self._stem_pair[0], self._stem_pair[1], 1 if want else 0)
+            if r < 0:
+                L.check(r, "plan_stem_pair")
+            self._stem_on = want
+
+    def stem_pair_fused(self) -> int:
+        return int(self.lib.uavsal_plan_stem_pair_report(self.plan))
 
     def _state_is_zero(self, state) -> bool:
         if state is None:
@@ -486,6 +525,7 @@
             else:
                 self.stage_inputs(x, cb0, cb1, state, cstate)
             self._arm_repeat(skip)
+            self._arm_stem_pair()
             modes = self.inplace and bool(self._seams or self._zs)
             if modes:
                 self._arm_modes(self._resident_zero if self.persistent else self._state_is_zero(state))
@@ -545,6 +585,7 @@
             out, _ = self._bind_in_place(x, cb0, cb1, self.h_view, self.c_view, lstm, skip)
             split = self.state_split()
             self._arm_repeat(skip)
+            self._arm_stem_pair()
             with self.priors.launches():
                 try:
                     L.check(self.lib.uavsal_plan_run(self.plan, 0, split, self._stream()), "plan_run(head)")
diff --git a/iip_uavsal_saliency_amd/model.py b/iip_uavsal_saliency_amd/model.py
--- a/iip_uavsal_saliency_amd/model.py
+++ b/iip_uavsal_saliency_amd/model.py
@@ -156,6 +156,7 @@
         self.cache_priors = True
         self.fuse_seams = True
         self.skip_zero_state = True
+        self.fuse_stem = True
         self.arena = True
         self.arena_debug = False
         self.max_engines = 4
diff --git a/iip_uavsal_saliency_amd/ops.py b/iip_uavsal_saliency_amd/ops.py
--- a/iip_uavsal_saliency_amd/ops.py
+++ b/iip_uavsal_saliency_amd/ops.py
@@ -314,6 +314,46 @@
     return out
 
 
+def stem_pair_descs(x_nchw, weight, scale, bias, wd, bnd, w2, bn2, tile=0):
+    from .synth import IMAGENET_MEAN, IMAGENET_STD
+    dev = x_nchw.device
+    n, _, H, W = x_nchw.shape
+    ho, wo = (H - 1) // 2 + 1, (W - 1) // 2 + 1
+    f0 = torch.empty((n, ho, wo, 32), dtype=torch.float32, device=dev)
+    f1 = torch.empty((n, ho, wo, 16), dtype=torch.float32, device=dev)
+    keep = [x_nchw.contiguous()]
+
+    def up(t):
+        t = t.detach().float().contiguous().to(dev)
+        keep.append(t)
+        return t.data_ptr()
+    sd = L.StemDesc()
+    sd.inp, sd.in_u8 = (None, keep[0].data_ptr()) if x_nchw.dtype == torch.uint8 else (keep[0].data_ptr(), None)
+    sd.w, sd.scale, sd.bias = up(P.pack_stem_weight(weight)), up(scale), up(bias)
+    sd.out, sd.ldo, sd.n_img, sd.H, sd.W = f0.data_ptr(), 32, n, H, W
+    for i in range(3):
+        sd.mean[i], sd.stdv[i] = IMAGENET_MEAN[i], IMAGENET_STD[i]
+    fd = L.FusedIrDesc()
+    fd.inp, fd.ldi = f0.data_ptr(), 32
+    fd.n_img, fd.H, fd.W, fd.Cin, fd.hidden, fd.Cout, fd.stride, fd.tile = n, ho, wo, 32, 32, 16, 1, tile
+    fd.wd, fd.scale_d, fd.bias_d = up(P.pack_dw_weight(wd)), up(bnd[0]), up(bnd[1])
+    fd.w2, fd.scale2, fd.bias2 = up(w2.reshape(16, 32).t()), up(bn2[0]), up(bn2[1])
+    fd.out, fd.ldo = f1.data_ptr(), 16
+    return sd, fd, f0, f1, keep
+
+
+def stem_fused_ir(x_nchw, weight, scale, bias, wd, bnd, w2, bn2, tile=0, fused=True):
+    lib = L.load()
+    sd, fd, f0, f1, keep = stem_pair_descs(x_nchw, weight, scale, bias, wd, bnd, w2, bn2, tile)
+    if fused:
+        L.check(lib.uavsal_stem_fused_ir(C.byref(sd), C.byref(fd), _stream(f1)), "uavsal_stem_fused_ir")
+    else:
+        L.check(lib.uavsal_stem_conv(C.byref(sd), _stream(f1)), "uavsal_stem_conv")
+        L.check(lib.uavsal_fused_ir(C.byref(fd), _stream(f1)), "uavsal_fused_ir")
+    torch.cuda.current_stream(f1.device).synchronize()
+    return f1
+
+
 def bilinear_ac(x, ho, wo, out=None, n_out=None, src_mod=None, src_div=1, split_out=False):
     lib = L.load()
     ip, ldi, n, h, w, c = _nhwc_view(x)
diff --git a/include/uavsal_hip.h b/include/uavsal_hip.h
--- a/include/uavsal_hip.h
+++ b/include/uavsal_hip.h
@@ -122,6 +122,9 @@
 } uavsal_stem_desc;
 
 int uavsal_stem_conv(const uavsal_stem_desc* d, uavsal_stream_t stream);
+
+int uavsal_stem_fused_ir(const uavsal_stem_desc* stem, const uavsal_fused_ir_desc* f1, uavsal_stream_t stream);
+int uavsal_stem_fused_ir_check(const uavsal_stem_desc* stem, const uavsal_fused_ir_desc* f1);
 
 typedef struct uavsal_bilinear_desc {
     const float* in;  int32_t ldi;  int32_t Hi, Wi;
@@ -719,6 +722,8 @@
 int uavsal_plan_seam(uavsal_plan* p, int op_xout, int op_xin, int on);
 int uavsal_plan_zero_state(uavsal_plan* p, int op_state_in_first, int op_state_in_last, int op_xin0, int op_gemm0, int op_xout0, int on);
 int uavsal_plan_mode_report(const uavsal_plan* p, int out[4]);
+int uavsal_plan_stem_pair(uavsal_plan* p, int op_stem, int op_f1, int on);
+int uavsal_plan_stem_pair_report(const uavsal_plan* p);
 int uavsal_plan_graph_build(uavsal_plan* p, uavsal_stream_t stream);
 int uavsal_plan_graph_launch(uavsal_plan* p, uavsal_stream_t stream);
 
```

Result: no change. 1998 frames/s (median of 2 runs) (+0.1%).
